# shanjiayao/PTT

Measured on AMD Instinct MI355X. Metric: tracklet frames/sec (hot path: PointNet++ SA stack + Point-Track-Transformer blocks), higher is better.
Workload: dtype f32

## Files before the change

include/ptt_hip.h:

```cpp
#ifndef PTT_HIP_H
#define PTT_HIP_H

#include <stddef.h>
#include <stdint.h>

#ifdef __cplusplus
extern "C" {
#endif

#define PTT_ABI_VERSION 28

enum {
    PTT_OK = 0,
    PTT_EINVAL = -1,
    PTT_EUNSUPPORTED = -2,
    PTT_ELAUNCH = -3,
    PTT_EWORKSPACE = -4
};

typedef void* ptt_stream_t;

int ptt_version(void);
const char* ptt_error_name(int code);
const char* ptt_last_error_string(void);

int ptt_fps_f32(const float* xyz, int B, int N, int npoint, int32_t* idx_out,
                ptt_stream_t stream);
int ptt_fps_ws_f32(const float* xyz, int B, int N, int npoint, int32_t* idx_out, float* workspace,
                   size_t workspace_elems, ptt_stream_t stream);

int ptt_gather_f32(const float* feat, const int32_t* idx, int B, int C, int N, int M,
                   float* out, ptt_stream_t stream);
int ptt_gather_grad_f32(const float* grad_out, const int32_t* idx, int B, int C, int N,
                        int M, float* grad_feat, ptt_stream_t stream);

int ptt_select_centres_f32(const float* xyz, const int32_t* idx, int B, int N, int M, float* new_xyz,
                           int64_t* idx64_out, ptt_stream_t stream);

int ptt_ball_query_f32(const float* new_xyz, const float* xyz, int B, int M, int N,
                       float radius, int nsample, int32_t* idx_out, ptt_stream_t stream);

int ptt_centres_ball_query_f32(const float* xyz, const int32_t* sel, int B, int N, int M, float radius, int nsample,
                               float* new_xyz, int64_t* idx64_out, int32_t* idx_out, ptt_stream_t stream);

int ptt_group_f32(const float* feat, const int32_t* idx, int B, int C, int N, int M,
                  int ns, float* out, ptt_stream_t stream);
int ptt_group_grad_f32(const float* grad_out, const int32_t* idx, int B, int C, int N,
                       int M, int ns, float* grad_feat, ptt_stream_t stream);

size_t ptt_scatter_add_det_workspace(int B, int N, int E);
int ptt_scatter_add_det_f32(const float* src, const int32_t* idx, int B, int C, int N, int E, float* out,
                            void* workspace, size_t workspace_bytes, ptt_stream_t stream);

int ptt_knn_f32(const float* xyz, int B, int N, int k, int32_t* idx_out,
                ptt_stream_t stream);
int ptt_knn_rel_f32(const float* xyz, int B, int N, int k, int32_t* idx_out, float* rel_out,
                    ptt_stream_t stream);

size_t ptt_packed_weight_elems(int Cout, int K);
int ptt_pack_weight_f32(const float* W, int Cout, int K, float* packed,
                        ptt_stream_t stream);
int ptt_pack_weight_rot_f32(const float* W, int Cout, int K, int rot, float* packed,
                            ptt_stream_t stream);

int ptt_linear_f32(const float* X, int rows, int K, int ldx, const float* Wpacked, int Cout,
                   const float* scale, const float* shift, int relu, const float* residual,
                   int ldr, float* out, int ldo, ptt_stream_t stream);

#define PTT_SA_MAX_LAYERS 4

typedef struct ptt_sa_layer {
    const float* Wpacked;
    const float* scale;
    const float* shift;
    int Cin;
    int Cout;
    int relu;
} ptt_sa_layer;

int ptt_rows_mlp_f32(const float* X, int rows, int K, int ldx, const ptt_sa_layer* layers, int n_layers,
                     const float* residual, int ldr, float* out, int ldo, ptt_stream_t stream);

size_t ptt_ball_query_grid_workspace(int B, int N);
int ptt_ball_query_grid_f32(const float* new_xyz, const float* xyz, int B, int M, int N, float radius, int nsample,
                            int32_t* idx_out, void* workspace, size_t workspace_bytes, ptt_stream_t stream);
int ptt_centres_ball_query_grid_f32(const float* xyz, const int32_t* sel, int B, int N, int M, float radius, int nsample,
                                    float* new_xyz, int64_t* idx64_out, int32_t* idx_out, void* workspace, size_t workspace_bytes,
                                    ptt_stream_t stream);
int ptt_fps_ball_knn_f32(const float* xyz, int B, int N, int M, float radius, int nsample, int k, int32_t* inds,
                         int64_t* inds64, float* new_xyz, int32_t* idx, int32_t* knn, float* rel, ptt_stream_t stream);
#define PTT_POINT_JOBS_MAX 4
typedef struct ptt_point_job {
    const float* xyz; const int32_t* centre_sel; const int32_t* point_sel;
    float* new_xyz; int64_t* idx64_out; int32_t* idx_out; float* rel_out;
    int32_t kind, sel_ld, B, Nraw, Npts, M, nsample;
    float radius;
} ptt_point_job;
int ptt_point_jobs_f32(const ptt_point_job* jobs, int n_jobs, ptt_stream_t stream);

#define PTT_ROW_JOBS_MAX 4
typedef struct ptt_row_job {
    const float* X; const float* X2;
    const float* Xmax;
    const float* Wpacked; const float* scale; const float* shift;
    const float* res; const float* res2;
    float* out; float* out2; float* raw;
    const float* rel; const float* w1;
    const float* qkv; const int32_t* knn; const float* pos;
    int32_t rows, K, K1, ldx, ldx2, Cout;
    int32_t act, res_split, ldr, ldr2, out_split, out_col0, ldo, ldo2, ldraw;
    int32_t prologue, epilogue, ldq, q_off, k_off, v_off, ldp, N;
    float sm_scale;
    int32_t col_tiles;
    const int32_t* idx; const float* xyz; const float* centres; const float* wx;
    float radius;
    int32_t ns, M, normalize_xyz, pro_relu;
} ptt_row_job;
int ptt_row_jobs_f32(const ptt_row_job* jobs, int n_jobs, ptt_stream_t stream);

typedef struct ptt_sa_desc {
    const float* xyz;
    const float* new_xyz;
    const int32_t* idx;
    const float* feat;
    int64_t feat_sb, feat_sc, feat_sn;
    float* out;
    int64_t out_sb, out_sc, out_sm;
    int B, N, M, nsample, C;
    float radius;
    int use_xyz;
    int normalize_xyz;
    int n_layers;
    ptt_sa_layer layers[PTT_SA_MAX_LAYERS];
    const float* l0_point_term;
    const float* l0_xyz_weight;
    int l0_channels;
    int l0_relu;
    void* compact_ws;
    size_t compact_ws_bytes;
} ptt_sa_desc;

int ptt_sa_fused_fwd_f32(const ptt_sa_desc* d, ptt_stream_t stream);
size_t ptt_sa_compact_workspace(int B, int M);

typedef struct ptt_xcorr_desc {
    const float* cos_t;
    const float* P;
    const float* w_sim;
    const float* scale0;
    const float* shift0;
    float* out;
    int64_t out_sb, out_sc, out_sn;
    float* sim_out;
    int B, Ns, Nt, C0;
    int n_layers;
    ptt_sa_layer layers[PTT_SA_MAX_LAYERS];
    int32_t split; int64_t out_sh;
    const float* search_feat; const float* templ_feat;
    int64_t s_sb, s_sn, t_sb, t_sn;
    int C; float eps;
} ptt_xcorr_desc;

int ptt_xcorr_fused_fwd_f32(const ptt_xcorr_desc* d, ptt_stream_t stream);

int ptt_cosine_map_f32(const float* search_feat, int64_t s_sb, int64_t s_sn, int64_t s_sc, const float* templ_feat,
                       int64_t t_sb, int64_t t_sn, int64_t t_sc, int B, int Ns, int Nt, int C, float eps,
                       float* cos_t, ptt_stream_t stream);

typedef struct ptt_attn_desc {
    const float* xyz;
    const float* rel;
    const int32_t* knn;
    const float* qkv;
    const float* Wd1p;
    const float* Wd2p;
    const float* bd2;
    const float* Wg1p;
    const float* bg1;
    const float* Wg2p;
    const float* bg2;
    float* res;
    float* attn;
    int B, N, k, D;
    const int32_t* order;
    int heads;
} ptt_attn_desc;

int ptt_pt_attn_pair_f32(const ptt_attn_desc* d, ptt_stream_t stream);
int ptt_spatial_order_f32(const float* xyz, int B, int N, int32_t* order, ptt_stream_t stream);

typedef struct ptt_crop_job {
    const float* points;
    int64_t ld;
    double lo1[3], hi1[3];
    double trans[3];
    double rot[9];
    double lo2[3], hi2[3];
    float* out;
    int32_t* count;
    int32_t n_points;
    int32_t capacity;
    uint8_t* label_out;
    double ltrans[3];
    double lrot[9];
    double llo[3], lhi[3];
    int32_t append;
    int32_t reserved;
} ptt_crop_job;

int ptt_crop_compact_f32(const ptt_crop_job* jobs_device, int n_jobs, ptt_stream_t stream);
#define PTT_CROP_JOBS_BY_VALUE_MAX 8
int ptt_crop_compact_host_f32(const ptt_crop_job* jobs_host, int n_jobs, ptt_stream_t stream);

#define PTT_MAX_SEGMENTS 4
typedef struct ptt_regularize_job {
    const float* seg[PTT_MAX_SEGMENTS];
    const int32_t* seg_count[PTT_MAX_SEGMENTS];
    int32_t seg_capacity[PTT_MAX_SEGMENTS];
    float* out;
    int32_t* info;
    int32_t n_seg;
    int32_t input_size;
// ... 297 lines not shown
```

ptt_amd/_lib.py:

```python
import ctypes
import os
import re
from ctypes import Structure, c_char_p, c_double, c_float, c_int, c_int32, c_int64, c_longlong, c_size_t, c_uint32, c_void_p

from .build import HEADER as HEADER_PATH, LIB as LIB_PATH


def _strip_comments(text):
    return re.sub(r"/\*.*?\*/|//[^\n]*", " ", text, flags=re.S)


def parse_defines(text):
    return {n: int(v) for n, v in re.findall(r"^[ \t]*#[ \t]*define[ \t]+(PTT_\w+)[ \t]+(-?\d+)[ \t]*$", _strip_comments(text), re.M)}


CTYPES = {"int": c_int, "int32_t": c_int32, "uint32_t": c_uint32, "int64_t": c_int64, "long long": c_longlong, "size_t": c_size_t,
          "float": c_float, "double": c_double, "ptt_stream_t": c_void_p}


def _ctype(decl, name, is_return=False):
    words = decl.replace("*", " * ").split()
    if not is_return and len(words) > 1 and words[-1] != "*":
        words.pop()
    if "*" in words:
# ... 67 lines not shown
                ("reg", c_float * 4), ("index", c_uint32), ("epoch", c_uint32), ("capacity", c_int32), ("reserved", c_int32)]


class TrainBatchDesc(Structure):
    _fields_ = [("search_points", c_void_p), ("template_points", c_void_p), ("cls_label", c_void_p), ("reg_label", c_void_p),
                ("src_out", c_void_p), ("idx_search_out", c_void_p), ("idx_template_out", c_void_p), ("info", c_void_p), ("totals", c_void_p),
                ("B", c_int32), ("n_cand", c_int32), ("search_size", c_int32), ("template_size", c_int32), ("min_points", c_int32),
                ("seed_lo", c_uint32), ("seed_hi", c_uint32), ("reserved", c_int32)]


class BnTrainTail(Structure):
    _fields_ = [("gamma", c_void_p), ("beta", c_void_p), ("act_a", c_void_p), ("act_b", c_void_p),
                ("running_mean", c_void_p), ("running_var", c_void_p), ("num_batches_tracked", c_void_p), ("momentum", c_float)]


class BnBwdInput(Structure):
    _fields_ = [("g", c_void_p), ("ldg", c_int), ("arg", c_void_p), ("ns", c_int), ("z", c_void_p), ("ldz", c_int),
                ("k1", c_void_p), ("c0", c_void_p), ("c1", c_void_p), ("mean", c_void_p), ("act_a", c_void_p), ("act_b", c_void_p),
                ("dz_out", c_void_p), ("ldd", c_int)]


class PackJob(Structure):
    _fields_ = [("W", c_void_p), ("out_offset", c_int64), ("stride_out", c_int64), ("stride_k", c_int64),
                ("Cout", c_int32), ("K", c_int32)]


class RowJob(Structure):
    _fields_ = [("X", c_void_p), ("X2", c_void_p), ("Xmax", c_void_p), ("Wpacked", c_void_p), ("scale", c_void_p), ("shift", c_void_p),
                ("res", c_void_p), ("res2", c_void_p), ("out", c_void_p), ("out2", c_void_p), ("raw", c_void_p),
                ("rel", c_void_p), ("w1", c_void_p), ("qkv", c_void_p), ("knn", c_void_p), ("pos", c_void_p),
                ("rows", c_int32), ("K", c_int32), ("K1", c_int32), ("ldx", c_int32), ("ldx2", c_int32), ("Cout", c_int32),
                ("act", c_int32), ("res_split", c_int32), ("ldr", c_int32), ("ldr2", c_int32), ("out_split", c_int32),
                ("out_col0", c_int32), ("ldo", c_int32), ("ldo2", c_int32), ("ldraw", c_int32),
                ("prologue", c_int32), ("epilogue", c_int32), ("ldq", c_int32), ("q_off", c_int32), ("k_off", c_int32),
                ("v_off", c_int32), ("ldp", c_int32), ("N", c_int32), ("sm_scale", c_float), ("col_tiles", c_int32),
                ("idx", c_void_p), ("xyz", c_void_p), ("centres", c_void_p), ("wx", c_void_p), ("radius", c_float),
                ("ns", c_int32), ("M", c_int32), ("normalize_xyz", c_int32), ("pro_relu", c_int32)]


class PointJob(Structure):
    _fields_ = [("xyz", c_void_p), ("centre_sel", c_void_p), ("point_sel", c_void_p), ("new_xyz", c_void_p), ("idx64_out", c_void_p),
                ("idx_out", c_void_p), ("rel_out", c_void_p), ("kind", c_int32), ("sel_ld", c_int32), ("B", c_int32),
                ("Nraw", c_int32), ("Npts", c_int32), ("M", c_int32), ("nsample", c_int32), ("radius", c_float)]


class TrackLossDesc(Structure):
    _fields_ = [("seed_cls", c_void_p), ("cls_label", c_void_p), ("search_inds", c_void_p), ("votes", c_void_p), ("reg_label", c_void_p),
                ("box_data", c_void_p), ("centres", c_void_p), ("pos_weight_seed", c_void_p), ("pos_weight_box", c_void_p),
                ("B", c_int32), ("N", c_int32), ("Ns", c_int32), ("M", c_int32), ("ld_reg", c_int32),
                ("w_seed_cls", c_float), ("w_seed_reg", c_float), ("w_box_cls", c_float), ("w_box_reg", c_float)]


class AdamTensor(Structure):
    _fields_ = [("param", c_void_p), ("grad", c_void_p), ("exp_avg", c_void_p), ("exp_avg_sq", c_void_p), ("n", c_int64)]


class GradJob(Structure):
    _fields_ = [("partial", c_void_p), ("nchunks", c_int32), ("reserved", c_int32)]


class GradSegment(Structure):
    _fields_ = [("dst", c_int64), ("n", c_int32), ("cols", c_int32), ("ld", c_int32), ("job0", c_int32), ("njobs", c_int32), ("out", c_int32),
                ("vec", c_int32), ("reserved", c_int32)]


class AdamHyper(Structure):
    _fields_ = [("beta1", c_float), ("beta2", c_float), ("one_minus_beta1", c_float), ("one_minus_beta2", c_float), ("eps", c_float), ("step_size", c_float), ("bias2_sqrt", c_float),
                ("weight_decay", c_float), ("max_norm", c_float), ("write_clipped", c_int32)]


class SaLayer(Structure):
    _fields_ = [("Wpacked", c_void_p), ("scale", c_void_p), ("shift", c_void_p),
                ("Cin", c_int), ("Cout", c_int), ("relu", c_int)]


class SaDesc(Structure):
    _fields_ = [("xyz", c_void_p), ("new_xyz", c_void_p), ("idx", c_void_p), ("feat", c_void_p),
                ("feat_sb", c_int64), ("feat_sc", c_int64), ("feat_sn", c_int64),
                ("out", c_void_p), ("out_sb", c_int64), ("out_sc", c_int64), ("out_sm", c_int64),
                ("B", c_int), ("N", c_int), ("M", c_int), ("nsample", c_int), ("C", c_int),
                ("radius", c_float), ("use_xyz", c_int), ("normalize_xyz", c_int), ("n_layers", c_int),
                ("layers", SaLayer * PTT_SA_MAX_LAYERS),
                ("l0_point_term", c_void_p), ("l0_xyz_weight", c_void_p), ("l0_channels", c_int), ("l0_relu", c_int),
                ("compact_ws", c_void_p), ("compact_ws_bytes", c_size_t)]


class XcorrDesc(Structure):
    _fields_ = [("cos_t", c_void_p), ("P", c_void_p), ("w_sim", c_void_p), ("scale0", c_void_p), ("shift0", c_void_p),
                ("out", c_void_p), ("out_sb", c_int64), ("out_sc", c_int64), ("out_sn", c_int64),
                ("sim_out", c_void_p),
                ("B", c_int), ("Ns", c_int), ("Nt", c_int), ("C0", c_int),
                ("n_layers", c_int), ("layers", SaLayer * PTT_SA_MAX_LAYERS),
                ("split", c_int32), ("out_sh", c_int64), ("search_feat", c_void_p), ("templ_feat", c_void_p),
                ("s_sb", c_int64), ("s_sn", c_int64), ("t_sb", c_int64), ("t_sn", c_int64), ("C", c_int), ("eps", c_float)]


class AttnDesc(Structure):
    _fields_ = [("xyz", c_void_p), ("rel", c_void_p), ("knn", c_void_p), ("qkv", c_void_p),
                ("Wd1p", c_void_p), ("Wd2p", c_void_p), ("bd2", c_void_p),
                ("Wg1p", c_void_p), ("bg1", c_void_p), ("Wg2p", c_void_p), ("bg2", c_void_p),
                ("res", c_void_p), ("attn", c_void_p),
                ("B", c_int), ("N", c_int), ("k", c_int), ("D", c_int), ("order", c_void_p), ("heads", c_int)]


_lib = None


def lib():
    global _lib
    if _lib is None:
        if not os.path.exists(LIB_PATH):
            raise RuntimeError(
                "ptt_amd: %s is missing — build it with `python -m ptt_amd.build` "
                "(hipcc --offload-arch=gfx950); there is no CPU fallback" % LIB_PATH)
        import torch
        try:
            loaded = ctypes.CDLL(LIB_PATH)
        except OSError as e:
            raise RuntimeError("ptt_amd: cannot load %s: %s" % (LIB_PATH, e))
        for name, (restype, argtypes) in PROTOTYPES.items():
            fn = getattr(loaded, name)
            fn.restype, fn.argtypes = restype, argtypes
        if loaded.ptt_version() != ABI_VERSION:
            raise RuntimeError("ptt_amd: %s has ABI version %d, this package expects %d — rebuild it with "
                               "`python -m ptt_amd.build`" % (LIB_PATH, loaded.ptt_version(), ABI_VERSION))
        _lib = loaded
    return _lib


def check(rc, what):
    if rc != 0:
        l = lib()
        raise RuntimeError("%s failed: %s (%s)" % (what, l.ptt_error_name(rc).decode(),
                                                   l.ptt_last_error_string().decode()))
```

ptt_amd/csrc/mfma_ops.hip:

```cpp
#include <math.h>
#include <stdlib.h>
#include <string.h>
#include "common.h"
#include "mfma_common.h"

#ifndef PTT_PAIR_PF
#define PTT_PAIR_PF 1
#endif
#ifndef PTT_GATHER_BATCH
#define PTT_GATHER_BATCH 16
#endif
#ifndef PTT_SA_WAVES
#define PTT_SA_WAVES 2
#endif

namespace ptt {

#ifdef PTT_DEV
#define PTT_STAMP(i) do { if (p.dbg && threadIdx.x == 0 && blockIdx.x < 4096) p.dbg[blockIdx.x * 8 + (i)] = __builtin_readcyclecounter(); } while (0)
#else
#define PTT_STAMP(i) do { } while (0)
#endif

__device__ __forceinline__ void stagger_second_slot(int first_wave_blocks, int quanta) {
// ... 341 lines not shown
                float y = acc[rt][u][r] * sc + sh;
                if (p.relu) y = fmaxf(y, 0.f);
                if (p.residual) y += p.residual[(size_t)gr * p.ldr + col];
                p.out[(size_t)gr * p.ldo + col] = y;
            }
    }
}

constexpr int LS_PD = 8;
__global__ __launch_bounds__(512, 1) void linear_small_kernel(LinearParams p) {
    extern __shared__ __attribute__((aligned(16))) float smem[];
    const int t = threadIdx.x, lane = t & 63, half = lane >> 5;
    const int w = __builtin_amdgcn_readfirstlane(t >> 6), ks = w >> 2, cw = w & 3;
    const int row0 = blockIdx.x * 32;
    const int ct = blockIdx.y * 4 + cw;
    const bool has_ct = ct < p.NT;
    const int hb = ((p.nkb + 1) / 2 + LS_PD - 1) / LS_PD * LS_PD;
    const int ldk = 2 * hb * 8 + 4;
    float* Xs = smem;
    float* Rs = smem + 32 * ldk;
    {
        const int qpr = 2 * hb * 2;
        for (int e = t; e < 32 * qpr; e += 512) {
            const int r = e / qpr, c = (e - r * qpr) << 2;
            f32x4 v = {0.f, 0.f, 0.f, 0.f};
            if (row0 + r < p.rows && c < p.K) v = *reinterpret_cast<const f32x4*>(p.X + (size_t)(row0 + r) * p.ldx + c);
            *reinterpret_cast<f32x4*>(Xs + r * ldk + c) = v;
        }
    }
    const __amdgpu_buffer_rsrc_t wr = weight_rsrc(p.Wp);
    const int wvoff = ((has_ct ? ct : 0) * 64 + lane) * 16;
    const int wkstep = p.NT * 1024;
    const int kb0 = ks * hb, last = p.nkb - 1;
    f32x4 b[LS_PD];
#pragma unroll
    for (int i = 0; i < LS_PD; ++i) b[i] = weight_load(wr, wvoff, min(kb0 + i, last) * wkstep);
    f32x16 acc;
#pragma unroll
    for (int r = 0; r < 16; ++r) acc[r] = 0.f;
    __syncthreads();
    const float* arow = Xs + (lane & 31) * ldk + 4 * half + kb0 * 8;
    for (int k = 0; k < hb; k += LS_PD) {
#pragma unroll
        for (int i = 0; i < LS_PD; ++i) {
            const f32x4 a = *reinterpret_cast<const f32x4*>(arow + (k + i) * 8);
#pragma unroll
            for (int j = 0; j < 4; ++j) acc = __builtin_amdgcn_mfma_f32_32x32x2f32(a[j], b[i][j], acc, 0, 0, 0);
            b[i] = weight_load(wr, wvoff, min(kb0 + k + i + LS_PD, last) * wkstep);
        }
    }
    if (ks == 1) {
#pragma unroll
        for (int r = 0; r < 16; ++r) Rs[(cw * 16 + r) * 64 + lane] = acc[r];
    }
    __syncthreads();
    if (ks == 1 || !has_ct) return;
    const int col = ct * 32 + (lane & 31);
    if (col >= p.Cout) return;
    const float sc = p.scale ? p.scale[col] : 1.f;
    const float sh = p.shift ? p.shift[col] : 0.f;
#pragma unroll
    for (int r = 0; r < 16; ++r) {
        const int gr = row0 + tile_row(r, half);
        if (gr >= p.rows) continue;
        float y = (acc[r] + Rs[(cw * 16 + r) * 64 + lane]) * sc + sh;
        if (p.relu) y = fmaxf(y, 0.f);
        if (p.residual) y += p.residual[(size_t)gr * p.ldr + col];
        p.out[(size_t)gr * p.ldo + col] = y;
    }
}

struct SaLayerDev { const float* Wp; const float* scale; const float* shift; int Cin, Cout, relu, nkb, NT; };
struct SaParams {
    const float* xyz; const float* new_xyz; const int32_t* idx; const float* feat; float* out;
    long long fsb, fsc, fsn, osb, osc, osm;
    int B, N, M, C, use_xyz, normalize, n_layers, ldk, K0, first_wave, stagger, vec_gather;
    int tiles, chunk;
    int hoist, l0_relu;
    const float* wx;
    float radius;
    long long* dbg;
    int32_t* cws;
    SaLayerDev L[PTT_SA_MAX_LAYERS];
};

struct RowsMlpParams {
    const float* X; const float* residual; float* out;
    int rows, K0, ldx, ldr, ldo, n_layers, ldk, vec_in;
    SaLayerDev L[PTT_SA_MAX_LAYERS];
};

__global__ __launch_bounds__(256, 2) void rows_mlp_kernel(RowsMlpParams p) {
    extern __shared__ __attribute__((aligned(16))) float smem[];
    float* Xs = smem;
    const int t = threadIdx.x, lane = t & 63, w = t >> 6, half = lane >> 5;
    const int row0 = blockIdx.x * 32;
    f32x4 pw[3];
    float psh[3];
    auto prefetch = [&](const SaLayerDev& L) {
        const f32x4* bp = reinterpret_cast<const f32x4*>(L.Wp) + (size_t)w * 64 + lane;
#pragma unroll
        for (int u = 0; u < 3; ++u) {
            psh[u] = 0.f;
            if (w + 4 * u < L.NT) {
                pw[u] = bp[(size_t)u * 4 * 64];
                const int col = (w + 4 * u) * 32 + (lane & 31);
                if (L.shift && !L.scale && col < L.Cout) psh[u] = L.shift[col];
            }
        }
    };
    prefetch(p.L[0]);
    {
        const int Kpad = p.L[0].nkb * 8;
        if (p.vec_in) {
            const int nq = Kpad >> 2;
            for (int e = t; e < 32 * nq; e += 256) {
                const int r = e / nq, c4 = (e - r * nq) * 4;
                f32x4 v = {0.f, 0.f, 0.f, 0.f};
                if (row0 + r < p.rows && c4 < p.K0) v = *reinterpret_cast<const f32x4*>(p.X + (size_t)(row0 + r) * p.ldx + c4);
                *reinterpret_cast<f32x4*>(Xs + r * p.ldk + c4) = v;
            }
        } else {
            for (int e = t; e < 32 * Kpad; e += 256) {
                const int r = e / Kpad, c = e - r * Kpad;
                Xs[r * p.ldk + c] = (row0 + r < p.rows && c < p.K0) ? p.X[(size_t)(row0 + r) * p.ldx + c] : 0.f;
            }
        }
    }
    lds_barrier();
    for (int l = 0; l < p.n_layers; ++l) {
        const SaLayerDev& L = p.L[l];
        const bool last = l == p.n_layers - 1, affine = L.scale != nullptr;
        f32x16 acc[1][3];
#pragma unroll
        for (int u = 0; u < 3; ++u)
#pragma unroll
            for (int r = 0; r < 16; ++r) acc[0][u][r] = psh[u];
        int nvalid = 0;
#pragma unroll
        for (int u = 0; u < 3; ++u)
            if (w + 4 * u < L.NT) nvalid = u + 1;
        if (nvalid) gemm_tiles<1, 3, 0>(Xs, p.ldk, L.nkb, reinterpret_cast<const f32x4*>(L.Wp), L.NT, w, nvalid, lane, acc, pw);
        if (!last) { prefetch(p.L[l + 1]); lds_barrier(); }
#pragma unroll
        for (int u = 0; u < 3; ++u) {
            if (u >= nvalid) break;
            const int col = (w + 4 * u) * 32 + (lane & 31);
            float sc = 1.f, sh = 0.f;
            if (affine && col < L.Cout) { sc = L.scale[col]; sh = L.shift ? L.shift[col] : 0.f; }
#pragma unroll
            for (int r = 0; r < 16; ++r) {
                float y = affine ? acc[0][u][r] * sc + sh : acc[0][u][r];
                if (L.relu) y = fmaxf(y, 0.f);
                const int row = tile_row(r, half);
                if (!last) {
                    Xs[row * p.ldk + col] = (col < L.Cout) ? y : 0.f;
                } else if (col < L.Cout && row0 + row < p.rows) {
                    if (p.residual) y += p.residual[(size_t)(row0 + row) * p.ldr + col];
                    p.out[(size_t)(row0 + row) * p.ldo + col] = y;
                }
            }
        }
        if (!last) lds_barrier();
    }
}

// ... 177 lines not shown
            } else {
                float m0 = y[0], m1 = y[8];
#pragma unroll
                for (int r = 1; r < 8; ++r) { m0 = fmaxf(m0, y[r]); m1 = fmaxf(m1, y[8 + r]); }
                m0 = max_halves(m0);
                m1 = max_halves(m1);
                if (L.relu) { m0 = fmaxf(m0, 0.f); m1 = fmaxf(m1, 0.f); }
                if (half == 0) {
                    const int ca = rt * 2, cb = rt * 2 + 1;
                    if (ca < ncentres) {
                        const int c = centre0 + ca; const int b = c / p.M, mm = c - b * p.M;
                        p.out[b * p.osb + col * p.osc + mm * p.osm] = m0;
                    }
                    if (cb < ncentres) {
                        const int c = centre0 + cb; const int b = c / p.M, mm = c - b * p.M;
                        p.out[b * p.osb + col * p.osc + mm * p.osm] = m1;
                    }
                }
            }
        }
    }
    if (!last) lds_barrier();
}

template <int NS, int RT>
__global__ __launch_bounds__(256, PTT_SA_WAVES) void sa_fused_kernel(SaParams p) {
    extern __shared__ __attribute__((aligned(16))) float smem[];
    float* Xs = smem;
    constexpr int CPW = 32 * RT / NS;
    const int t = threadIdx.x, lane = t & 63, w = t >> 6;
    const int total_centres = p.B * p.M;
    const int centre0 = logical_block() * CPW;
    const int ncentres = min(CPW, total_centres - centre0);
    stagger_second_slot(p.first_wave, p.stagger);
    PTT_STAMP(0);

    SaPre pre;
    pre.w[0] = pre.w[1] = f32x4{0.f, 0.f, 0.f, 0.f};
    prefetch_first_block(p.L[0].Wp, p.L[0].scale, p.L[0].shift, p.L[0].NT, w, lane, pre);

    sa_gather_rows<NS, 8 * RT>(p, Xs, w * 8 * RT, centre0, lane);
    lds_barrier();

    PTT_STAMP(1);
    for (int l = 0; l < p.n_layers; ++l) {
        const SaLayerDev& L = p.L[l];
        const bool last = (l == p.n_layers - 1);
        const int ctw = (L.NT + 3) >> 2;
        const SaLayerDev* Ln = last ? nullptr : &p.L[l + 1];
        if (ctw <= 1) sa_layer<NS, 1, RT>(p, L, last, Xs, lane, w, centre0, ncentres, pre, Ln);
        else sa_layer<NS, 2, RT>(p, L, last, Xs, lane, w, centre0, ncentres, pre, Ln);
        PTT_STAMP(2 + l);
    }
}

constexpr int SAS_LDK = 132;
constexpr int SAS_TILE = 64 * SAS_LDK;

__device__ __forceinline__ f32x4 sas_pair_load(const float* meta, __amdgpu_buffer_rsrc_t rf, int w, int i, int sub, int q,
                                               f32x4& m) {
    m = *reinterpret_cast<const f32x4*>(meta + (w * 16 + 2 * i + sub) * 4);
    return weight_load(rf, __builtin_bit_cast(int, m[0]) + q * 16, 0);
}
__device__ __forceinline__ void sas_pair_store(float* X, int w, int i, int sub, int q, f32x4 v, const f32x4& m, const f32x4& wx0,
                                               const f32x4& wx1, const f32x4& wx2, float floor) {
#pragma unroll
    for (int j = 0; j < 4; ++j) {
        float y = __builtin_fmaf(wx0[j], m[1], v[j]);
        y = __builtin_fmaf(wx1[j], m[2], y);
        y = __builtin_fmaf(wx2[j], m[3], y);
        v[j] = fmaxf(y, floor);
    }
    *reinterpret_cast<f32x4*>(X + (16 * w + 2 * i + sub) * SAS_LDK + q * 4) = v;
}

struct SasCentre {
    int c, b, m;
    __device__ __forceinline__ void advance(int k, int M) {
        c += k; m += k;
        while (m >= M) { m -= M; ++b; }
    }
};

__device__ __forceinline__ float sas_pool(const f32x16& a, float sh, int relu) {
    float mx = a[0];
#pragma unroll
    for (int r = 1; r < 16; ++r) mx = fmaxf(mx, a[r]);
    mx = max_halves(mx) + sh;
    return relu ? fmaxf(mx, 0.f) : mx;
}

#ifndef PTT_SAS_INTERLEAVE
#define PTT_SAS_INTERLEAVE 0
#endif
#ifndef PTT_SAS_EXP
#define PTT_SAS_EXP 0
#endif
template <int NS>
__global__ __launch_bounds__(256, 2) void sa_stream_kernel(SaParams p) {
    static_assert(NS == 32, "one centre per 32-row tile");
    extern __shared__ __attribute__((aligned(16))) float smem[];
    float* const P = smem;
    float* const Q = smem + SAS_TILE;
    float* const meta = smem + 2 * SAS_TILE;
    const int t = threadIdx.x, lane = t & 63, half = lane >> 5, sub = half, q = lane & 31;
    const int w = __builtin_amdgcn_readfirstlane(t >> 6);
    const int tile0 = logical_block() * p.chunk;
    const int ntiles = min(p.chunk, p.tiles - tile0);
    if (ntiles <= 0) return;
    stagger_second_slot(p.first_wave, p.stagger);
    const SaLayerDev& L1 = p.L[0];
    const SaLayerDev& L2 = p.L[1];
    const __amdgpu_buffer_rsrc_t rf = weight_rsrc(p.feat);
    const __amdgpu_buffer_rsrc_t wr1 = weight_rsrc(L1.Wp), wr2 = weight_rsrc(L2.Wp);
    const int wvoff = (w * 64 + lane) * 16;
    constexpr int WK1 = 4 * 1024, WK2 = 8 * 1024;
    const f32x4 wx0 = *reinterpret_cast<const f32x4*>(p.wx + q * 4);
    const f32x4 wx1 = *reinterpret_cast<const f32x4*>(p.wx + 128 + q * 4);
    const f32x4 wx2 = *reinterpret_cast<const f32x4*>(p.wx + 256 + q * 4);
    const int col = lane & 31;
    const float sh1 = L1.shift ? L1.shift[w * 32 + col] : 0.f;
    const float sh2a = L2.shift ? L2.shift[w * 32 + col] : 0.f;
    const float sh2b = L2.shift ? L2.shift[(w + 4) * 32 + col] : 0.f;
    f32x16 sh1v;
#pragma unroll
    for (int r = 0; r < 16; ++r) sh1v[r] = sh1;
    const int total_centres = p.B * p.M;
    const float floor0 = p.l0_relu ? 0.f : -__builtin_inff();
    const float rdiv = p.normalize ? p.radius : 1.0f;
    const int M = p.M, N = p.N;
    const int osb = (int)p.osb, osm = (int)p.osm;
    const int ocol0 = (w * 32 + col) * (int)p.osc, ocol1 = ((w + 4) * 32 + col) * (int)p.osc;

    SasCentre own, first;
    {
        const int c0 = tile0 * 2;
        first.c = c0; first.b = c0 / M; first.m = c0 - first.b * M;
        own = first;
        own.advance(w >> 1, M);
    }
    auto meta_index = [&](const SasCentre& ce) -> int {
        const int c = ce.c < total_centres ? ce.c : total_centres - 1;
        return p.idx[(size_t)c * 32 + 16 * (w & 1) + (lane & 15)];
    };
    struct MetaXyz { float x, y, z, cx, cy, cz; int flat; };
    auto meta_fetch = [&](const SasCentre& ce, int n) -> MetaXyz {
        const bool in = ce.c < total_centres;
        const int c = in ? ce.c : total_centres - 1;
        const int b = in ? ce.b : p.B - 1;
        MetaXyz r;
        r.flat = b * N + n;
        r.x = p.xyz[(size_t)r.flat * 3 + 0]; r.y = p.xyz[(size_t)r.flat * 3 + 1]; r.z = p.xyz[(size_t)r.flat * 3 + 2];
        r.cx = p.new_xyz[(size_t)c * 3 + 0]; r.cy = p.new_xyz[(size_t)c * 3 + 1]; r.cz = p.new_xyz[(size_t)c * 3 + 2];
        return r;
    };
    auto meta_store = [&](const MetaXyz& r) {
        const float dx = (r.x - r.cx) / rdiv, dy = (r.y - r.cy) / rdiv, dz = (r.z - r.cz) / rdiv;
        const int off = r.flat * (128 * (int)sizeof(float));
        *reinterpret_cast<f32x4*>(meta + (w * 16 + (lane & 15)) * 4) = f32x4{__builtin_bit_cast(float, off), dx, dy, dz};
    };

    f32x4 pre1[2] = {weight_load(wr1, wvoff, 0), weight_load(wr1, wvoff, WK1)};
    {
        const int n = meta_index(own);
        meta_store(meta_fetch(own, n));
#pragma unroll
        for (int i = 0; i < 8; ++i) {
            f32x4 m;
            const f32x4 v = sas_pair_load(meta, rf, w, i, sub, q, m);
            sas_pair_store(P, w, i, sub, q, v, m, wx0, wx1, wx2, floor0);
        }
    }

    f32x16 acc[2][2];
#pragma unroll
    for (int rt = 0; rt < 2; ++rt)
#pragma unroll
        for (int u = 0; u < 2; ++u)
#pragma unroll
            for (int r = 0; r < 16; ++r) acc[rt][u][r] = 0.f;
    float pv[2][2] = {{0.f, 0.f}, {0.f, 0.f}};
    SasCentre prev = first;
    const f32x16 zero16 = {0.f, 0.f, 0.f, 0.f, 0.f, 0.f, 0.f, 0.f, 0.f, 0.f, 0.f, 0.f, 0.f, 0.f, 0.f, 0.f};

    auto store_pooled = [&](const SasCentre& f) {
        SasCentre c1 = f;
        c1.advance(1, M);
        if (half == 0) {
            if (f.c < total_centres) {
                float* o = p.out + (f.b * osb + f.m * osm);
                o[ocol0] = pv[0][0]; o[ocol1] = pv[0][1];
            }
            if (c1.c < total_centres) {
                float* o = p.out + (c1.b * osb + c1.m * osm);
                o[ocol0] = pv[1][0]; o[ocol1] = pv[1][1];
            }
        }
    };

    for (int it = 0; it < ntiles; ++it) {
        const bool more = it + 1 < ntiles;
        SasCentre own_next = own;
        if (more) own_next.advance(2, M);
        if (!(PTT_SAS_EXP & 1)) lds_barrier();
        const int nn = meta_index(own_next);
        MetaXyz mx;

        f32x16 acc1[2];
        {
            const float* arow = P + (lane & 31) * SAS_LDK + 4 * half;
            f32x4 a0[2], a1[2], bc[2], bn[2];
#define SAS_A1(A, KB)                                                                           \
            {                                                                                   \
                A[0] = *reinterpret_cast<const f32x4*>(arow + (KB) * 8);                        \
                A[1] = *reinterpret_cast<const f32x4*>(arow + 32 * SAS_LDK + (KB) * 8);         \
            }
            bc[0] = pre1[0]; bc[1] = pre1[1];
            SAS_A1(a0, 0)
#pragma unroll
            for (int i = 0; i < 8; ++i) {
                if (i < 7) { bn[0] = weight_load(wr1, wvoff, (2 * i + 2) * WK1); bn[1] = weight_load(wr1, wvoff, (2 * i + 3) * WK1); }
                SAS_A1(a1, 2 * i + 1)
                if (i == 4 && !(PTT_SAS_EXP & 16)) mx = meta_fetch(own_next, nn);
                __builtin_amdgcn_sched_barrier(0);
                if (i == 0) {
#pragma unroll
                    for (int rt = 0; rt < 2; ++rt) acc1[rt] = __builtin_amdgcn_mfma_f32_32x32x2f32(a0[rt][0], bc[0][0], sh1v, 0, 0, 0);
#pragma unroll
                    for (int j = 1; j < 4; ++j)
#pragma unroll
                        for (int rt = 0; rt < 2; ++rt)
                            acc1[rt] = __builtin_amdgcn_mfma_f32_32x32x2f32(a0[rt][j], bc[0][j], acc1[rt], 0, 0, 0);
                } else {
#pragma unroll
                    for (int j = 0; j < 4; ++j)
#pragma unroll
                        for (int rt = 0; rt < 2; ++rt)
                            acc1[rt] = __builtin_amdgcn_mfma_f32_32x32x2f32(a0[rt][j], bc[0][j], acc1[rt], 0, 0, 0);
                }
                __builtin_amdgcn_sched_barrier(0);
                if (i < 7) SAS_A1(a0, 2 * i + 2)
                __builtin_amdgcn_sched_barrier(0);
#pragma unroll
                for (int j = 0; j < 4; ++j)
#pragma unroll
                    for (int rt = 0; rt < 2; ++rt)
                        acc1[rt] = __builtin_amdgcn_mfma_f32_32x32x2f32(a1[rt][j], bc[1][j], acc1[rt], 0, 0, 0);
                __builtin_amdgcn_sched_barrier(0);
                if (i < 4 && !(PTT_SAS_EXP & 8)) pv[i >> 1][i & 1] = sas_pool(acc[i >> 1][i & 1], (i & 1) ? sh2b : sh2a, L2.relu);
                if (i == 6 && !(PTT_SAS_EXP & 16)) meta_store(mx);
                __builtin_amdgcn_sched_barrier(0);
                bc[0] = bn[0]; bc[1] = bn[1];
            }
#undef SAS_A1
        }
        f32x4 pre2[2][2];
#pragma unroll
        for (int k = 0; k < 2; ++k) {
            pre2[k][0] = weight_load(wr2, wvoff, k * WK2);
            pre2[k][1] = weight_load(wr2, wvoff, k * WK2 + 4 * 1024);
        }
#pragma unroll
        for (int rt = 0; rt < 2; ++rt)
#pragma unroll
            for (int r = (PTT_SAS_EXP & 4) ? 15 : 0; r < 16; ++r)
                Q[(rt * 32 + tile_row(r, half)) * SAS_LDK + w * 32 + col] = fmaxf(acc1[rt][r], 0.f);
        if (it > 0) store_pooled(prev);
        if (!(PTT_SAS_EXP & 1)) lds_barrier();

        {
            const float* arow = Q + (lane & 31) * SAS_LDK + 4 * half;
            f32x4 a0[2], a1[2], bc[2][2], bn[2][2];
#define SAS_A2(A, KB)                                                                           \
            {                                                                                   \
                A[0] = *reinterpret_cast<const f32x4*>(arow + (KB) * 8);                        \
                A[1] = *reinterpret_cast<const f32x4*>(arow + 32 * SAS_LDK + (KB) * 8);         \
            }
#pragma unroll
            for (int k = 0; k < 2; ++k) { bc[k][0] = pre2[k][0]; bc[k][1] = pre2[k][1]; }
            SAS_A2(a0, 0)
            f32x4 mc = *reinterpret_cast<const f32x4*>(meta + (w * 16 + sub) * 4), mn = mc;
#pragma unroll
            for (int i = 0; i < 8; ++i) {
                if (i < 7) {
#pragma unroll
                    for (int k = 0; k < 2; ++k) {
                        bn[k][0] = weight_load(wr2, wvoff, (2 * i + 2 + k) * WK2);
                        bn[k][1] = weight_load(wr2, wvoff, (2 * i + 2 + k) * WK2 + 4 * 1024);
                    }
                } else {
                    pre1[0] = weight_load(wr1, wvoff, 0);
                    pre1[1] = weight_load(wr1, wvoff, WK1);
                }
                SAS_A2(a1, 2 * i + 1)
                f32x4 v = wx0;
                if (!(PTT_SAS_EXP & 2)) v = weight_load(rf, __builtin_bit_cast(int, mc[0]) + q * 16, 0);
                __builtin_amdgcn_sched_barrier(0);
                if (i == 0) {
#pragma unroll
                    for (int u = 0; u < 2; ++u)
#pragma unroll
                        for (int rt = 0; rt < 2; ++rt)
                            acc[rt][u] = __builtin_amdgcn_mfma_f32_32x32x2f32(a0[rt][0], bc[0][u][0], zero16, 0, 0, 0);
#pragma unroll
                    for (int j = 1; j < 4; ++j)
#pragma unroll
                        for (int u = 0; u < 2; ++u)
#pragma unroll
                            for (int rt = 0; rt < 2; ++rt)
                                acc[rt][u] = __builtin_amdgcn_mfma_f32_32x32x2f32(a0[rt][j], bc[0][u][j], acc[rt][u], 0, 0, 0);
                } else {
                    gemm_mfma_block<2, 2, 2>(a0, bc[0], acc);
                }
                __builtin_amdgcn_sched_barrier(0);
                if (i < 7) {
                    SAS_A2(a0, 2 * i + 2)
                    mn = *reinterpret_cast<const f32x4*>(meta + (w * 16 + 2 * (i + 1) + sub) * 4);
                }
                __builtin_amdgcn_sched_barrier(0);
                gemm_mfma_block<2, 2, 2>(a1, bc[1], acc);
                if (!(PTT_SAS_EXP & 2)) sas_pair_store(P, w, i, sub, q, v, mc, wx0, wx1, wx2, floor0);
#if PTT_SAS_INTERLEAVE
#pragma unroll
                for (int k = 0; k < 16; ++k) {
                    __builtin_amdgcn_sched_group_barrier(0x008, 1, 0);
                    __builtin_amdgcn_sched_group_barrier(0x002, 1, 0);
                }
                __builtin_amdgcn_sched_group_barrier(0x200, 1, 0);
#endif
                __builtin_amdgcn_sched_barrier(0);
                mc = mn;
#pragma unroll
                for (int k = 0; k < 2; ++k) { bc[k][0] = bn[k][0]; bc[k][1] = bn[k][1]; }
            }
#undef SAS_A2
        }
        prev = first;
        if (more) { first.advance(2, M); own = own_next; }
    }
#pragma unroll
    for (int i = 0; i < 4; ++i) pv[i >> 1][i & 1] = sas_pool(acc[i >> 1][i & 1], (i & 1) ? sh2b : sh2a, L2.relu);
    store_pooled(prev);
}

struct XcorrParams {
    const float* P; const float* wsim; const float* scale0; const float* shift0;
    float* sim_out;
    const float* cos_t;
    int C0, Nt;
    SaParams sa;
    const float* sfeat; const float* tfeat; long long s_sb, s_sn, t_sb, t_sn; int C; float eps;
    long long out_sh;
};

struct CosParams {
    const float* sfeat; const float* tfeat; float* cos_t;
    long long s_sb, s_sn, s_sc, t_sb, t_sn, t_sc;
    int B, Ns, Nt, C;
    float eps;
};
__global__ __launch_bounds__(256) void cos_map_kernel(CosParams q) {
    const int lane = threadIdx.x & 63;
    const int j = blockIdx.x * 4 + (threadIdx.x >> 6);
    if (j >= q.B * q.Ns) return;
    const int b = j / q.Ns, jj = j - b * q.Ns;
    const float* s = q.sfeat + (long long)b * q.s_sb + (long long)jj * q.s_sn;
    for (int i0 = 0; i0 < q.Nt; i0 += 64) {
        const int i = i0 + lane;
        const float* a = q.tfeat + (long long)b * q.t_sb + (long long)(i < q.Nt ? i : q.Nt - 1) * q.t_sn;
        float dot = 0.f, na = 0.f, ns = 0.f;
        if (q.t_sc == 1 && q.s_sc == 1 && (q.C & 3) == 0 && ((q.t_sn | q.t_sb | q.s_sn | q.s_sb) & 3) == 0 &&
            ((reinterpret_cast<uintptr_t>(q.tfeat) | reinterpret_cast<uintptr_t>(q.sfeat)) & 15) == 0) {
            for (int c = 0; c < q.C; c += 4) {
                const f32x4 av = *reinterpret_cast<const f32x4*>(a + c), sv = *reinterpret_cast<const f32x4*>(s + c);
#pragma unroll
                for (int k = 0; k < 4; ++k) { dot += av[k] * sv[k]; na += av[k] * av[k]; ns += sv[k] * sv[k]; }
            }
        } else {
            for (int c = 0; c < q.C; ++c) {
                const float av = a[(long long)c * q.t_sc], sv = s[(long long)c * q.s_sc];
                dot += av * sv; na += av * av; ns += sv * sv;
            }
        }
        if (i < q.Nt) q.cos_t[((long long)b * q.Ns + jj) * q.Nt + i] = dot / (fmaxf(sqrtf(na), q.eps) * fmaxf(sqrtf(ns), q.eps));
    }
}

template <int RT, bool SPLIT>
__global__ __launch_bounds__(256, 2) void xcorr_fused_kernel(XcorrParams q) {
    constexpr int ROWS = 32 * RT;
    extern __shared__ __attribute__((aligned(16))) float smem[];
    const SaParams& p = q.sa;
    float* Xs = smem;
    float* simv = smem + ROWS * p.ldk;
    const int t = threadIdx.x, lane = t & 63, w = t >> 6, half = lane >> 5;
    const int npts = p.B * p.M;
    const int j = SPLIT ? (int)blockIdx.x % npts : logical_block();
    const int hsel = SPLIT ? (int)blockIdx.x / npts : 0;
    const int b = j / p.M, jj = j - b * p.M;
    stagger_second_slot(p.first_wave, p.stagger);
    SaPre pre;
    pre.w[0] = pre.w[1] = f32x4{0.f, 0.f, 0.f, 0.f};
    float run[2] = {-__builtin_inff(), -__builtin_inff()};
    const int nlast = p.n_layers - 1;
    const SaLayerDev& LL = p.L[nlast];

    const int ibeg = SPLIT ? hsel * (q.Nt >> 1) : 0, iend = SPLIT ? ibeg + (q.Nt >> 1) : q.Nt;
    for (int i0 = ibeg; i0 < iend; i0 += ROWS) {
        prefetch_first_block(p.L[0].Wp, p.L[0].scale, p.L[0].shift, p.L[0].NT, w, lane, pre);
        if (i0 != ibeg) __syncthreads();
        if constexpr (SPLIT) {
            const int i = t >> 3, sub = t & 7;
            const float* a = q.tfeat + (long long)b * q.t_sb + (long long)(i0 + i) * q.t_sn;
            const float* sv_ = q.sfeat + (long long)b * q.s_sb + (long long)jj * q.s_sn;
            float dot = 0.f, na = 0.f, ns = 0.f;
            for (int c = sub * 4; c < q.C; c += 32) {
                const f32x4 av = *reinterpret_cast<const f32x4*>(a + c), sv = *reinterpret_cast<const f32x4*>(sv_ + c);
#pragma unroll
                for (int k = 0; k < 4; ++k) { dot += av[k] * sv[k]; na += av[k] * av[k]; ns += sv[k] * sv[k]; }
            }
#pragma unroll
// ... 80 lines not shown
            p.out[(SPLIT ? hsel * q.out_sh : 0) + b * p.osb + col * p.osc + jj * p.osm] = LL.relu ? fmaxf(run[u], 0.f) : run[u];
        }
    }
}

template <int NS, int CT, bool AFFINE, int RT>
__device__ __forceinline__ void sa_wave_layer(const SaParams& p, const SaLayerDev& L, bool last, float* Xw, int lane,
                                              int centre0, int ncentres) {
    f32x16 acc[RT][CT];
#pragma unroll
    for (int u = 0; u < CT; ++u) {
        const float s0 = (!AFFINE && L.shift) ? L.shift[u * 32 + (lane & 31)] : 0.f;
#pragma unroll
        for (int rt = 0; rt < RT; ++rt)
#pragma unroll
            for (int r = 0; r < 16; ++r) acc[rt][u][r] = s0;
    }
    gemm_core<RT, CT, CT, 1>(Xw, p.ldk, L.nkb, reinterpret_cast<const f32x4*>(L.Wp), L.NT, 0, lane, acc);
    __builtin_amdgcn_wave_barrier();
    const int half = lane >> 5;
#pragma unroll
    for (int u = 0; u < CT; ++u) {
        const int col = u * 32 + (lane & 31);
        float sc = 1.f, sv = 0.f;
        if constexpr (AFFINE) { sc = L.scale[col]; sv = L.shift ? L.shift[col] : 0.f; }
#pragma unroll
        for (int rt = 0; rt < RT; ++rt) {
            float y[16];
#pragma unroll
            for (int r = 0; r < 16; ++r) y[r] = AFFINE ? acc[rt][u][r] * sc + sv : acc[rt][u][r];
            if (!last) {
#pragma unroll
                for (int r = 0; r < 16; ++r)
                    Xw[(rt * 32 + tile_row(r, half)) * p.ldk + col] = L.relu ? fmaxf(y[r], 0.f) : y[r];
            } else if (NS == 32) {
                float m = y[0];
#pragma unroll
                for (int r = 1; r < 16; ++r) m = fmaxf(m, y[r]);
                m = max_halves(m);
                if (L.relu) m = fmaxf(m, 0.f);
                if (half == 0 && rt < ncentres) {
                    const int c = centre0 + rt; const int b = c / p.M, mm = c - b * p.M;
                    p.out[b * p.osb + col * p.osc + mm * p.osm] = m;
                }
            } else {
                float m0 = y[0], m1 = y[8];
#pragma unroll
                for (int r = 1; r < 8; ++r) { m0 = fmaxf(m0, y[r]); m1 = fmaxf(m1, y[8 + r]); }
                m0 = max_halves(m0);
                m1 = max_halves(m1);
                if (L.relu) { m0 = fmaxf(m0, 0.f); m1 = fmaxf(m1, 0.f); }
                if (half == 0) {
                    if (2 * rt < ncentres) {
                        const int c = centre0 + 2 * rt; const int b = c / p.M, mm = c - b * p.M;
                        p.out[b * p.osb + col * p.osc + mm * p.osm] = m0;
                    }
                    if (2 * rt + 1 < ncentres) {
                        const int c = centre0 + 2 * rt + 1; const int b = c / p.M, mm = c - b * p.M;
                        p.out[b * p.osb + col * p.osc + mm * p.osm] = m1;
                    }
                }
            }
        }
    }
    __builtin_amdgcn_wave_barrier();
}

constexpr int SAC_HDR = 16;
struct SacTable {
    int32_t* ws; int T;
    __host__ __device__ int32_t* ndist() const { return ws + SAC_HDR; }
    __host__ __device__ int32_t* list(int k) const { return ws + SAC_HDR + (size_t)(1 + k) * T; }
    __host__ __device__ int32_t* rows(int k) const { return ws + SAC_HDR + 5 * (size_t)T + (size_t)((4 << k) - 4) * T; }
    static size_t words(size_t T) { return SAC_HDR + 65 * T; }
};
constexpr int SAC_PASSES = 4;

__global__ __launch_bounds__(64) void sa_compact_zero_kernel(int32_t* ws) {
    if (threadIdx.x < 4) ws[threadIdx.x] = 0;
}

template <bool XYZ>
__global__ __launch_bounds__(256) void sa_compact_kernel(const float* __restrict__ xyz, const int32_t* __restrict__ idx, int N, int M,
                                                         SacTable tab) {
    __shared__ int s_cnt[4], s_base[4], s_cls[32], s_pos[32], s_nd[32];
    __shared__ int s_row[32][32];
    const int t = threadIdx.x, lane = t & 63, half = lane >> 5, s = lane & 31, w = t >> 6;
    const int g0 = blockIdx.x * 32, T = tab.T;
    if (t < 4) s_cnt[t] = 0;
    __syncthreads();
    int iv[SAC_PASSES];
    uint32_t x[SAC_PASSES], y[SAC_PASSES], z[SAC_PASSES];
#pragma unroll
    for (int q = 0; q < SAC_PASSES; ++q) iv[q] = idx[(size_t)min(g0 + q * 8 + w * 2 + half, T - 1) * 32 + s];
    if constexpr (XYZ) {
#pragma unroll
        for (int q = 0; q < SAC_PASSES; ++q) {
            const int b = min(g0 + q * 8 + w * 2 + half, T - 1) / M;
            const uint32_t* pt = reinterpret_cast<const uint32_t*>(xyz) + ((size_t)b * N + iv[q]) * 3;
            x[q] = pt[0]; y[q] = pt[1]; z[q] = pt[2];
        }
    }
#pragma unroll
    for (int q = 0; q < SAC_PASSES; ++q) {
        const int lc = q * 8 + w * 2 + half;
        const int i0a = __builtin_amdgcn_readlane(iv[q], 0), i0b = __builtin_amdgcn_readlane(iv[q], 32);
        const int i0 = half ? i0b : i0a;
        const bool real = s == 0 || iv[q] != i0;
        int dup = 0;
        if constexpr (XYZ) {
            const unsigned long long rm = __ballot(real);
            const int J = 31 - __builtin_clz((uint32_t)rm | (uint32_t)(rm >> 32));
            for (int j = 0; j < J; ++j) {
                const uint32_t xa = __builtin_amdgcn_readlane(x[q], j), xb = __builtin_amdgcn_readlane(x[q], 32 + j);
                const uint32_t ya = __builtin_amdgcn_readlane(y[q], j), yb = __builtin_amdgcn_readlane(y[q], 32 + j);
                const uint32_t za = __builtin_amdgcn_readlane(z[q], j), zb = __builtin_amdgcn_readlane(z[q], 32 + j);
                dup |= (int)(j < s) & (int)(x[q] == (half ? xb : xa)) & (int)(y[q] == (half ? yb : ya)) & (int)(z[q] == (half ? zb : za));
            }
        }
        const bool keep = real && !dup;
        const unsigned long long km = __ballot(keep);
        const uint32_t m = half ? (uint32_t)(km >> 32) : (uint32_t)km;
        const int nd = __popc(m);
        if (keep) s_row[lc][__popc(m & ((1u << s) - 1u))] = iv[q];
        if (s == 0) {
            const int k = nd <= 4 ? 0 : nd <= 8 ? 1 : nd <= 16 ? 2 : 3;
            const bool valid = g0 + lc < T;
            s_cls[lc] = valid ? k : -1;
            s_nd[lc] = nd;
            s_pos[lc] = valid ? atomicAdd(&s_cnt[k], 1) : 0;
            if (valid) tab.ndist()[g0 + lc] = nd;
        }
    }
    __syncthreads();
    if (t < 4) s_base[t] = s_cnt[t] ? atomicAdd(&tab.ws[t], s_cnt[t]) : 0;
    __syncthreads();
    for (int e = t; e < 32 * 32; e += 256) {
        const int lc = e >> 5, j = e & 31, k = s_cls[lc];
        if (k < 0 || j >= (4 << k)) continue;
        const int q = s_base[k] + s_pos[lc];
        tab.rows(k)[(size_t)q * (4 << k) + j] = s_row[lc][j < s_nd[lc] ? j : 0];
        if (j == 0) tab.list(k)[q] = g0 + lc;
    }
}

#ifndef PTT_SAL_WGS
#define PTT_SAL_WGS 1
#endif
#ifndef PTT_SAL_WAVES
#define PTT_SAL_WAVES 12
#endif

template <int ROWS>
struct SacTileT {
    static constexpr int LG = ROWS == 32 ? 3 : 4;
    static_assert(ROWS == 32 || ROWS == 64, "32- or 64-row tiles");
    int k, first, n;
    __device__ __forceinline__ static void count(const int32_t* ws, int total, int (&cnt)[4], int (&tiles)[4]) {
#pragma unroll
        for (int k = 0; k < 4; ++k) {
            cnt[k] = min(max(ws[k], 0), total);
            tiles[k] = (k ? tiles[k - 1] : 0) + ((cnt[k] + ((1 << LG) >> k) - 1) >> (LG - k));
        }
    }
    __device__ __forceinline__ void at(int j, const int (&tiles)[4], const int (&cnt)[4]) {
        k = j < tiles[0] ? 0 : j < tiles[1] ? 1 : j < tiles[2] ? 2 : 3;
        const int j0 = k == 0 ? 0 : k == 1 ? tiles[0] : k == 2 ? tiles[1] : tiles[2];
        const int nk = k == 0 ? cnt[0] : k == 1 ? cnt[1] : k == 2 ? cnt[2] : cnt[3];
        first = (j - j0) << (LG - k);
        n = min((1 << LG) >> k, nk - first);
    }
    __device__ __forceinline__ void row(const SacTable& tab, int s, int& n_out, int& ball) const {
        const int cl = s >> (2 + k), inb = cl < n;
        n_out = tab.rows(k)[(size_t)first * (4 << k) + (inb ? s : (s & ((4 << k) - 1)))];
        ball = tab.list(k)[first + (inb ? cl : 0)];
    }
};
using SacTile = SacTileT<32>;

template <int NU>
__device__ __forceinline__ void sac_store(int k, int n, int ball, int M, const f32x16 (&acc)[NU], const float (&sh)[NU],
                                          float* const (&o)[NU], int relu, int half, int osb, int osm) {
    int ob[8];
#pragma unroll
    for (int g = 0; g < 8; ++g) {
        if (g >= (8 >> k)) break;
        const int id = __builtin_amdgcn_readlane(ball, g << (2 + k)), b = id / M;
        ob[g] = b * osb + (id - b * M) * osm;
    }
#pragma unroll
    for (int u = 0; u < NU; ++u) {
        const f32x16& a = acc[u];
        if (k == 3) {
            const float mx = sas_pool(a, sh[u], relu);
            if (half == 0) o[u][ob[0]] = mx;
        } else if (k == 2) {
            float m0 = a[0], m1 = a[8];
#pragma unroll
            for (int r = 1; r < 8; ++r) { m0 = fmaxf(m0, a[r]); m1 = fmaxf(m1, a[8 + r]); }
            m0 = max_halves(m0) + sh[u]; m1 = max_halves(m1) + sh[u];
            if (relu) { m0 = fmaxf(m0, 0.f); m1 = fmaxf(m1, 0.f); }
            if (half < n) o[u][half ? ob[1] : ob[0]] = half ? m1 : m0;
        } else {
            float m[4];
#pragma unroll
            for (int q = 0; q < 4; ++q) m[q] = fmaxf(fmaxf(a[4 * q], a[4 * q + 1]), fmaxf(a[4 * q + 2], a[4 * q + 3]));
            if (k == 1) {
#pragma unroll
                for (int q = 0; q < 4; ++q) m[q] = max_halves(m[q]) + sh[u];
#pragma unroll
                for (int i = 0; i < 2; ++i) {
                    const int g = 2 * half + i;
                    float v = half ? m[2 + i] : m[i];
                    if (relu) v = fmaxf(v, 0.f);
                    if (g < n) o[u][half ? ob[2 + i] : ob[i]] = v;
                }
            } else {
#pragma unroll
                for (int q = 0; q < 4; ++q) {
                    const int g = 2 * q + half;
                    float v = m[q] + sh[u];
                    if (relu) v = fmaxf(v, 0.f);
                    if (g < n) o[u][half ? ob[2 * q + 1] : ob[2 * q]] = v;
                }
            }
        }
    }
}

template <bool COMPACT>
__global__ __launch_bounds__(64 * PTT_SAL_WAVES) __attribute__((amdgpu_waves_per_eu(PTT_SAL_WAVES * PTT_SAL_WGS / 4)))
void sa_lds_kernel(SaParams p) {
    extern __shared__ __attribute__((aligned(16))) float smem[];
    float* W1 = smem;
    float* W2 = smem + 4096;
    const int t = threadIdx.x, lane = t & 63, half = lane >> 5, col = lane & 31;
    const int w = __builtin_amdgcn_readfirstlane(t >> 6);
    const int total = p.B * p.M, M = p.M, N = p.N;
    const int nw = (int)blockDim.x >> 6;
    SacTable tab{p.cws, total};
    int cnt[4], tiles[4];
    if constexpr (COMPACT) {
        SacTile::count(p.cws, total, cnt, tiles);
        if (logical_block() >= tiles[3]) return;
    }
    {
        const f32x4* g1 = reinterpret_cast<const f32x4*>(p.L[1].Wp);
        const f32x4* g2 = reinterpret_cast<const f32x4*>(p.L[2].Wp);
        f32x4* s1 = reinterpret_cast<f32x4*>(W1);
        f32x4* s2 = reinterpret_cast<f32x4*>(W2);
        const int nthr = (int)blockDim.x;
        for (int i = t; i < 1024; i += nthr) s1[i] = g1[i];
        for (int i = t; i < 2048; i += nthr) s2[i] = g2[i];
    }
    float* cst = smem + 4096 + 8192 + w * 640 + lane;
#pragma unroll
    for (int u = 0; u < 2; ++u) {
        const f32x4 f = reinterpret_cast<const f32x4*>(p.L[0].Wp)[u * 64 + col];
        const float s0 = p.L[0].shift ? p.L[0].shift[u * 32 + col] : 0.f;
        cst[(0 + u) * 64] = half ? f[1] : f[0];
        cst[(2 + u) * 64] = half ? s0 : f[2];
        cst[(4 + u) * 64] = p.L[1].shift ? p.L[1].shift[u * 32 + col] : 0.f;
    }
#pragma unroll
    for (int u = 0; u < 4; ++u) cst[(6 + u) * 64] = p.L[2].shift ? p.L[2].shift[u * 32 + col] : 0.f;
    const float one_zero = half ? 0.f : 1.f, one_hi = 1.f;
    __syncthreads();
    int c0, c1, cstep;
    if constexpr (COMPACT) {
        c0 = logical_block() + (int)gridDim.x * w; c1 = tiles[3]; cstep = (int)gridDim.x * nw;
    } else {
        const int gw = logical_block() * nw + w;
        c0 = gw * p.chunk; c1 = min(total, c0 + p.chunk); cstep = 1;
    }
    if (c0 >= c1) return;
    const float rdiv = p.normalize ? p.radius : 1.0f;
    const int osb = (int)p.osb, osm = (int)p.osm, osc = (int)p.osc;
    const f32x16 zero16 = {0.f, 0.f, 0.f, 0.f, 0.f, 0.f, 0.f, 0.f, 0.f, 0.f, 0.f, 0.f, 0.f, 0.f, 0.f, 0.f};
    const float* a1p = W1 + lane * 4;
    const float* b2p = W2 + lane * 4;
    const __amdgpu_buffer_rsrc_t rx = weight_rsrc(p.xyz);

    SasCentre ce{0, 0, 0};
    SacTile tc{0, 0, 0};
    float px, py, pz, cx, cy, cz;
    int g_cur = 0;
    if constexpr (COMPACT) {
        tc.at(c0, tiles, cnt);
        int n_cur;
        tc.row(tab, col, n_cur, g_cur);
        const size_t flat = (size_t)(g_cur / M) * N + n_cur;
        px = p.xyz[flat * 3]; py = p.xyz[flat * 3 + 1]; pz = p.xyz[flat * 3 + 2];
        cx = p.new_xyz[(size_t)g_cur * 3]; cy = p.new_xyz[(size_t)g_cur * 3 + 1]; cz = p.new_xyz[(size_t)g_cur * 3 + 2];
    } else {
        ce.c = c0; ce.b = c0 / M; ce.m = c0 - ce.b * M;
        const int n_cur = p.idx[(size_t)c0 * 32 + col];
        const size_t flat = (size_t)ce.b * N + n_cur;
        px = p.xyz[flat * 3]; py = p.xyz[flat * 3 + 1]; pz = p.xyz[flat * 3 + 2];
        cx = p.new_xyz[(size_t)c0 * 3]; cy = p.new_xyz[(size_t)c0 * 3 + 1]; cz = p.new_xyz[(size_t)c0 * 3 + 2];
    }
    for (int c = c0; c < c1; c += cstep) {
        SasCentre nx = ce;
        SacTile tx = tc;
        int n_next, g_next;
        if constexpr (COMPACT) {
            if (c + cstep < c1) tx.at(c + cstep, tiles, cnt);
            tx.row(tab, col, n_next, g_next);
        } else {
            if (c + 1 < c1) nx.advance(1, M);
            n_next = p.idx[(size_t)nx.c * 32 + col];
        }
        f32x4 wa[2], wn[2];
#pragma unroll
        for (int u = 0; u < 2; ++u) wa[u] = *reinterpret_cast<const f32x4*>(a1p + u * 256);
        const float dx = (px - cx) / rdiv, dy = (py - cy) / rdiv, dz = (pz - cz) / rdiv;
        __builtin_amdgcn_sched_barrier(0);
        f32x16 h0[2];
        {
            const float k0 = half ? dy : dx, k1 = half ? one_hi : dz;
#pragma unroll
            for (int u = 0; u < 2; ++u) h0[u] = __builtin_amdgcn_mfma_f32_32x32x2f32(cst[(0 + u) * 64], k0, zero16, 0, 0, 0);
#pragma unroll
            for (int u = 0; u < 2; ++u) h0[u] = __builtin_amdgcn_mfma_f32_32x32x2f32(cst[(2 + u) * 64], k1, h0[u], 0, 0, 0);
#pragma unroll
            for (int u = 0; u < 2; ++u)
#pragma unroll
                for (int r = 0; r < 16; ++r) h0[u][r] = fmaxf(h0[u][r], 0.f);
        }
        f32x16 h1[2];
        f32x4 wb[4], wm[4];
        {
#pragma unroll
            for (int u = 0; u < 2; ++u) h1[u] = __builtin_amdgcn_mfma_f32_32x32x2f32(cst[(4 + u) * 64], one_zero, zero16, 0, 0, 0);
#pragma unroll
            for (int kb = 0; kb < 8; ++kb) {
                if (kb < 7) {
#pragma unroll
                    for (int u = 0; u < 2; ++u) wn[u] = *reinterpret_cast<const f32x4*>(a1p + ((kb + 1) * 2 + u) * 256);
                } else {
#pragma unroll
                    for (int u = 0; u < 4; ++u) wb[u] = *reinterpret_cast<const f32x4*>(b2p + u * 256);
                }
                __builtin_amdgcn_sched_barrier(0);
#pragma unroll
                for (int j = 0; j < 4; ++j)
#pragma unroll
                    for (int u = 0; u < 2; ++u)
                        h1[u] = __builtin_amdgcn_mfma_f32_32x32x2f32(wa[u][j], h0[kb >> 2][(kb & 3) * 4 + j], h1[u], 0, 0, 0);
                __builtin_amdgcn_sched_barrier(0);
#pragma unroll
                for (int u = 0; u < 2; ++u) wa[u] = wn[u];
            }
#pragma unroll
            for (int u = 0; u < 2; ++u)
#pragma unroll
                for (int r = 0; r < 16; ++r) h1[u][r] = fmaxf(h1[u][r], 0.f);
        }
        {
            const int g = COMPACT ? g_next : nx.c;
            const int off = ((COMPACT ? g_next / M : nx.b) * N + n_next) * 12;
            px = __builtin_bit_cast(float, __builtin_amdgcn_raw_buffer_load_b32(rx, off, 0, 0));
            py = __builtin_bit_cast(float, __builtin_amdgcn_raw_buffer_load_b32(rx, off + 4, 0, 0));
            pz = __builtin_bit_cast(float, __builtin_amdgcn_raw_buffer_load_b32(rx, off + 8, 0, 0));
            cx = p.new_xyz[(size_t)g * 3]; cy = p.new_xyz[(size_t)g * 3 + 1]; cz = p.new_xyz[(size_t)g * 3 + 2];
        }
        __builtin_amdgcn_sched_barrier(0);
        {
            f32x16 acc[4];
#pragma unroll
            for (int kb = 0; kb < 8; ++kb) {
                if (kb < 7) {
#pragma unroll
                    for (int u = 0; u < 4; ++u) wm[u] = *reinterpret_cast<const f32x4*>(b2p + ((kb + 1) * 4 + u) * 256);
                }
                __builtin_amdgcn_sched_barrier(0);
#pragma unroll
                for (int j = 0; j < 4; ++j)
#pragma unroll
                    for (int u = 0; u < 4; ++u)
                        acc[u] = __builtin_amdgcn_mfma_f32_32x32x2f32(h1[kb >> 2][(kb & 3) * 4 + j], wb[u][j],
                                                                       (kb == 0 && j == 0) ? zero16 : acc[u], 0, 0, 0);
                __builtin_amdgcn_sched_barrier(0);
#pragma unroll
                for (int u = 0; u < 4; ++u) wb[u] = wm[u];
            }
            if constexpr (COMPACT) {
                const float sh2[4] = {cst[6 * 64], cst[7 * 64], cst[8 * 64], cst[9 * 64]};
                float* const o[4] = {p.out + col * osc, p.out + (32 + col) * osc, p.out + (64 + col) * osc, p.out + (96 + col) * osc};
                sac_store<4>(tc.k, tc.n, g_cur, M, acc, sh2, o, p.L[2].relu, half, osb, osm);
            } else {
                float* o = p.out + (ce.b * osb + ce.m * osm);
#pragma unroll
                for (int u = 0; u < 4; ++u) {
                    const float mx = sas_pool(acc[u], cst[(6 + u) * 64], p.L[2].relu);
                    if (half == 0) o[(u * 32 + col) * osc] = mx;
                }
            }
        }
        if constexpr (COMPACT) { tc = tx; g_cur = g_next; } else ce = nx;
    }
}

__global__ __launch_bounds__(256, 2) void sa_stream_compact_kernel(SaParams p) {
    extern __shared__ __attribute__((aligned(16))) float smem[];
    float* const P = smem;
    float* const Q = smem + SAS_TILE;
    float* const meta = smem + 2 * SAS_TILE;
    int* const sball = reinterpret_cast<int*>(meta + 64 * 4);
    const int t = threadIdx.x, lane = t & 63, half = lane >> 5, sub = half, q = lane & 31, col = q;
    const int w = __builtin_amdgcn_readfirstlane(t >> 6);
    const int total = p.B * p.M, M = p.M, N = p.N;
    const SacTable tab{p.cws, total};
    int cnt[4], tiles[4];
    SacTileT<64>::count(p.cws, total, cnt, tiles);
    if ((int)blockIdx.x >= tiles[3]) return;
    const SaLayerDev& L1 = p.L[0];
    const SaLayerDev& L2 = p.L[1];
    const __amdgpu_buffer_rsrc_t rf = weight_rsrc(p.feat);
    const __amdgpu_buffer_rsrc_t wr1 = weight_rsrc(L1.Wp), wr2 = weight_rsrc(L2.Wp);
    const int wvoff = (w * 64 + lane) * 16;
    constexpr int WK1 = 4 * 1024, WK2 = 8 * 1024;
    const f32x4 wx0 = *reinterpret_cast<const f32x4*>(p.wx + q * 4);
    const f32x4 wx1 = *reinterpret_cast<const f32x4*>(p.wx + 128 + q * 4);
    const f32x4 wx2 = *reinterpret_cast<const f32x4*>(p.wx + 256 + q * 4);
    const float sh1 = L1.shift ? L1.shift[w * 32 + col] : 0.f;
    const float sh2[2] = {L2.shift ? L2.shift[w * 32 + col] : 0.f, L2.shift ? L2.shift[(w + 4) * 32 + col] : 0.f};
    f32x16 sh1v;
#pragma unroll
    for (int r = 0; r < 16; ++r) sh1v[r] = sh1;
    const f32x16 zero16 = {0.f, 0.f, 0.f, 0.f, 0.f, 0.f, 0.f, 0.f, 0.f, 0.f, 0.f, 0.f, 0.f, 0.f, 0.f, 0.f};
    const float floor0 = p.l0_relu ? 0.f : -__builtin_inff();
    const float rdiv = p.normalize ? p.radius : 1.0f;
    const int osb = (int)p.osb, osm = (int)p.osm;
    float* const o[2] = {p.out + (w * 32 + col) * (int)p.osc, p.out + ((w + 4) * 32 + col) * (int)p.osc};

    for (int j = blockIdx.x; j < tiles[3]; j += (int)gridDim.x) {
        SacTileT<64> tc;
        tc.at(j, tiles, cnt);
        if (t < 64) {
            int n, ball;
            tc.row(tab, t, n, ball);
            const int flat = (ball / M) * N + n;
            const float x = p.xyz[(size_t)flat * 3 + 0], y = p.xyz[(size_t)flat * 3 + 1], z = p.xyz[(size_t)flat * 3 + 2];
            const float cx = p.new_xyz[(size_t)ball * 3 + 0], cy = p.new_xyz[(size_t)ball * 3 + 1], cz = p.new_xyz[(size_t)ball * 3 + 2];
            const float dx = (x - cx) / rdiv, dy = (y - cy) / rdiv, dz = (z - cz) / rdiv;
            const int off = flat * (128 * (int)sizeof(float));
            *reinterpret_cast<f32x4*>(meta + t * 4) = f32x4{__builtin_bit_cast(float, off), dx, dy, dz};
            sball[t] = ball;
        }
        __syncthreads();
#pragma unroll
        for (int i = 0; i < 8; ++i) {
            f32x4 m;
            const f32x4 v = sas_pair_load(meta, rf, w, i, sub, q, m);
            sas_pair_store(P, w, i, sub, q, v, m, wx0, wx1, wx2, floor0);
        }
        const int ballr[2] = {sball[col], sball[32 + col]};
        __syncthreads();
        {
            f32x16 acc1[2] = {sh1v, sh1v};
            const float* arow = P + (lane & 31) * SAS_LDK + 4 * half;
#pragma unroll
            for (int kb = 0; kb < 16; ++kb) {
                const f32x4 b = weight_load(wr1, wvoff, kb * WK1);
                const f32x4 a[2] = {*reinterpret_cast<const f32x4*>(arow + kb * 8),
                                    *reinterpret_cast<const f32x4*>(arow + 32 * SAS_LDK + kb * 8)};
#pragma unroll
                for (int jj = 0; jj < 4; ++jj)
#pragma unroll
                    for (int rt = 0; rt < 2; ++rt) acc1[rt] = __builtin_amdgcn_mfma_f32_32x32x2f32(a[rt][jj], b[jj], acc1[rt], 0, 0, 0);
            }
#pragma unroll
            for (int rt = 0; rt < 2; ++rt)
#pragma unroll
                for (int r = 0; r < 16; ++r) Q[(rt * 32 + tile_row(r, half)) * SAS_LDK + w * 32 + col] = fmaxf(acc1[rt][r], 0.f);
        }
        __syncthreads();
        {
            f32x16 acc[2][2] = {{zero16, zero16}, {zero16, zero16}};
            const float* arow = Q + (lane & 31) * SAS_LDK + 4 * half;
#pragma unroll
            for (int kb = 0; kb < 16; ++kb) {
                const f32x4 b[2] = {weight_load(wr2, wvoff, kb * WK2), weight_load(wr2, wvoff, kb * WK2 + 4 * 1024)};
                const f32x4 a[2] = {*reinterpret_cast<const f32x4*>(arow + kb * 8),
                                    *reinterpret_cast<const f32x4*>(arow + 32 * SAS_LDK + kb * 8)};
                gemm_mfma_block<2, 2, 2>(a, b, acc);
            }
#pragma unroll
            for (int rt = 0; rt < 2; ++rt) {
                const int n = tc.n - rt * (8 >> tc.k);
                if (n <= 0) continue;
                sac_store<2>(tc.k, n, ballr[rt], M, acc[rt], sh2, o, L2.relu, half, osb, osm);
            }
        }
    }
}

template <int NS, int RT>
__global__ __launch_bounds__(256, 2) void sa_wave_kernel(SaParams p) {
    extern __shared__ __attribute__((aligned(16))) float smem[];
    constexpr int CPW = 32 * RT / NS;
    const int t = threadIdx.x, lane = t & 63, w = t >> 6;
    float* Xw = smem + w * 32 * RT * p.ldk;
    const int total_centres = p.B * p.M;
    const int centre0 = (logical_block() * 4 + w) * CPW;
    if (centre0 >= total_centres) return;
    const int ncentres = min(CPW, total_centres - centre0);

#pragma unroll
    for (int rt = 0; rt < RT; ++rt) sa_gather_rows<NS, 32>(p, Xw, rt * 32, centre0, lane);
    __builtin_amdgcn_wave_barrier();

    for (int l = 0; l < p.n_layers; ++l) {
        const SaLayerDev& L = p.L[l];
        const bool last = (l == p.n_layers - 1);
#define PTT_WAVE_LAYER(CTV)                                                                         \
        { if (L.scale) sa_wave_layer<NS, CTV, true, RT>(p, L, last, Xw, lane, centre0, ncentres);       \
          else sa_wave_layer<NS, CTV, false, RT>(p, L, last, Xw, lane, centre0, ncentres); }
        if (L.NT == 1) PTT_WAVE_LAYER(1)
        else if (L.NT == 2) PTT_WAVE_LAYER(2)
        else PTT_WAVE_LAYER(4)
#undef PTT_WAVE_LAYER
    }
}

struct AttnParams {
    const float* xyz; const float* rel; const int32_t* knn; const float* qkv; const float* Wd1p;
    const float* Wd2p; const float* bd2; const float* Wg1p; const float* bg1; const float* Wg2p; const float* bg2;
    float* res; float* attn;
    const int32_t* order;
    int BN, N, first_wave, stagger;
    long long* dbg;
};

template <int D, int HEADS>
__device__ __forceinline__ void gemm_heads(const float* Xs, int ldk, const float* Wp, int w, int lane, f32x16 (&acc)[1][4],
                                           const f32x4 (&pre)[4]) {
    static_assert(D == 512 && (HEADS == 2 || HEADS == 4 || HEADS == 8 || HEADS == 16), "4 waves x 4 column tiles of D = 512");
    constexpr int HD = D / HEADS, TPH = HD / 32, NKB = HD / 8;
    constexpr int NA = HEADS == 2 ? 2 : 4;
    constexpr int NB = HEADS == 2 ? 2 : 1;
    const int row = lane & 31, half = lane >> 5;
    const float* arow[NA];
#pragma unroll
    for (int i = 0; i < NA; ++i) arow[i] = Xs + row * ldk + 4 * half + ((w + 4 * i * (4 / NA)) / TPH) * HD;
    const __amdgpu_buffer_rsrc_t wr = weight_rsrc(Wp);
    int wvoff[NB];
#pragma unroll
    for (int i = 0; i < NB; ++i) wvoff[i] = (((w + 4 * i) % TPH) * 64 + lane) * 16;
    constexpr int wkstep = TPH * 1024;
    f32x4 bcur[NB], bnxt[NB];
#pragma unroll
    for (int i = 0; i < NB; ++i) { bcur[i] = pre[i]; bnxt[i] = bcur[i]; }
    auto block = [&](int kb) {
        f32x4 a[NA];
#pragma unroll
        for (int i = 0; i < NA; ++i) a[i] = *reinterpret_cast<const f32x4*>(arow[i] + kb * 8);
#pragma unroll
        for (int j = 0; j < 4; ++j)
#pragma unroll
            for (int u = 0; u < 4; ++u)
                acc[0][u] = __builtin_amdgcn_mfma_f32_32x32x2f32(a[u / (4 / NA)][j], bcur[u % NB][j], acc[0][u], 0, 0, 0);
    };
    for (int kb = 0; kb + 1 < NKB; ++kb) {
#pragma unroll
        for (int i = 0; i < NB; ++i) bnxt[i] = weight_load(wr, wvoff[i], (kb + 1) * wkstep);
        block(kb);
#pragma unroll
        for (int i = 0; i < NB; ++i) bcur[i] = bnxt[i];
    }
    block(NKB - 1);
}

template <int D, int HEADS>
__device__ __forceinline__ void prefetch_first_block_heads(const float* Wp, int w, int lane, f32x4 (&pre)[4]) {
// ... 248 lines not shown
        if (L.nkb * 8 > maxk) maxk = L.nkb * 8;
        if (!last && L.NT * 32 > maxk) maxk = L.NT * 32;
        cin = s.Cout;
    }
    if (ldo < cin || (residual && ldr < cin)) return fail(PTT_EINVAL, "ptt_rows_mlp_f32: ldo=%d ldr=%d Cout=%d", ldo, ldr, cin);
    p.ldk = maxk + 4;
    p.vec_in = ((K & 3) == 0 && (ldx & 3) == 0 && (reinterpret_cast<uintptr_t>(X) & 15) == 0) ? 1 : 0;
    const int lds = 32 * p.ldk * (int)sizeof(float);
    int rc = set_lds_limit(reinterpret_cast<const void*>(rows_mlp_kernel), lds);
    if (rc) return rc;
    hipLaunchKernelGGL(rows_mlp_kernel, dim3((rows + 31) / 32), dim3(256), lds, as_stream(stream), p);
    return check_launch("rows_mlp_kernel");
}

extern "C" size_t ptt_sa_compact_workspace(int B, int M) {
    const long long T = (long long)(B > 0 ? B : 0) * (M > 0 ? M : 0);
    return SacTable::words((size_t)T) * sizeof(int32_t);
}

extern "C" int ptt_sa_fused_fwd_f32(const ptt_sa_desc* d, ptt_stream_t stream) {
    if (!d) return fail(PTT_EINVAL, "ptt_sa_fused_fwd_f32: null descriptor");
    if (d->B < 0 || d->N <= 0 || d->M < 0 || d->C < 0 || d->n_layers < 1 || d->n_layers > PTT_SA_MAX_LAYERS)
        return fail(PTT_EINVAL, "ptt_sa_fused_fwd_f32: B=%d N=%d M=%d C=%d layers=%d", d->B, d->N, d->M, d->C,
                    d->n_layers);
    if (d->nsample != 16 && d->nsample != 32 && d->nsample != 64)
        return fail(PTT_EUNSUPPORTED, "ptt_sa_fused_fwd_f32: nsample=%d (16, 32 and 64 are instantiated)", d->nsample);
    if (d->B == 0 || d->M == 0) return PTT_OK;
    const bool hoist = d->l0_point_term != nullptr;
    if (!d->xyz || !d->new_xyz || !d->idx || !d->out || (!hoist && d->C > 0 && !d->feat))
        return fail(PTT_EINVAL, "ptt_sa_fused_fwd_f32: null pointer");
    if (!d->use_xyz && d->C == 0) return fail(PTT_EINVAL, "ptt_sa_fused_fwd_f32: no xyz and no features");
    if (hoist) {
        const int c0 = d->l0_channels;
        if (!d->use_xyz || !d->l0_xyz_weight || c0 <= 0 || (c0 % 32) != 0 || c0 > 256 ||
            (reinterpret_cast<uintptr_t>(d->l0_point_term) & 15) != 0 ||
            (reinterpret_cast<uintptr_t>(d->l0_xyz_weight) & 15) != 0)
            return fail(PTT_EINVAL, "ptt_sa_fused_fwd_f32: hoisted layer 0 needs use_xyz, 16-byte aligned (B,N,C0) and "
                        "(3,C0) arrays and C0 a multiple of 32 <= 256 (C0=%d)", c0);
    }

    SaParams p;
    p.xyz = d->xyz; p.new_xyz = d->new_xyz; p.idx = d->idx; p.feat = d->feat; p.out = d->out;
    p.fsb = d->feat_sb; p.fsc = d->feat_sc; p.fsn = d->feat_sn;
    p.osb = d->out_sb; p.osc = d->out_sc; p.osm = d->out_sm;
    p.B = d->B; p.N = d->N; p.M = d->M; p.C = d->C; p.use_xyz = d->use_xyz ? 1 : 0;
    p.normalize = d->normalize_xyz ? 1 : 0; p.n_layers = d->n_layers; p.radius = d->radius;
    p.K0 = (d->use_xyz ? 3 : 0) + d->C;
    p.hoist = hoist ? 1 : 0; p.l0_relu = d->l0_relu ? 1 : 0; p.wx = d->l0_xyz_weight;
    if (hoist && d->l0_channels == 128 && (unsigned long long)d->B * d->N * 128ull * sizeof(float) < 0x7fffffffull &&
        !dev_switches().sa_gather1)
        p.hoist = 2;
    if (hoist) {
        p.feat = d->l0_point_term; p.C = d->l0_channels; p.K0 = p.C;
        p.fsc = 1; p.fsn = p.C; p.fsb = (long long)d->N * p.C;
    }
    int maxk = 0, cin = p.K0;
    for (int l = 0; l < d->n_layers; ++l) {
        const ptt_sa_layer& s = d->layers[l];
        if (s.Cin != cin) return fail(PTT_EINVAL, "ptt_sa_fused_fwd_f32: layer %d Cin=%d, expected %d", l, s.Cin, cin);
        if (s.Cout <= 0 || (s.Cout % 32) != 0 || s.Cout > 256)
            return fail(PTT_EUNSUPPORTED, "ptt_sa_fused_fwd_f32: layer %d Cout=%d must be a multiple of 32 <= 256", l,
                        s.Cout);
        if (!s.Wpacked) return fail(PTT_EINVAL, "ptt_sa_fused_fwd_f32: layer %d has no weights", l);
        SaLayerDev& L = p.L[l];
        L.Wp = s.Wpacked; L.scale = s.scale; L.shift = s.shift; L.Cin = s.Cin; L.Cout = s.Cout; L.relu = s.relu;
        L.nkb = (s.Cin + 7) / 8; L.NT = s.Cout / 32;
        if (L.nkb * 8 > maxk) maxk = L.nkb * 8;
        if (l + 1 < d->n_layers && s.Cout > maxk) maxk = s.Cout;
        cin = s.Cout;
    }
    {
        const unsigned long long lim = 0x7fffffffull, B = (unsigned long long)d->B;
        if (B * d->N * 12ull >= lim || B * d->M * d->nsample * 4ull >= lim || B * d->M * (unsigned long long)cin * 4ull >= lim ||
            B * d->N * (unsigned long long)(p.C > 0 ? p.C : 1) * 4ull >= lim)
            return fail(PTT_EUNSUPPORTED, "ptt_sa_fused_fwd_f32: B=%d N=%d M=%d: an array of this launch exceeds 2 GiB "
                        "(32-bit offsets) — split the batch", d->B, d->N, d->M);
    }
    p.ldk = maxk + 4;
    p.vec_gather = (p.C > 0 && p.fsc == 1 && (p.C & 3) == 0 && p.C <= 256 && (p.fsn & 3) == 0 &&
                    (p.fsb & 3) == 0 && (reinterpret_cast<uintptr_t>(p.feat) & 15) == 0) ? 1 : 0;
    p.first_wave = 1024; p.stagger = dev_switches().sa_stagger;
    p.dbg = dev_switches().stamps;
    p.cws = nullptr;
    const int total_centres = d->B * d->M;
    hipStream_t s = as_stream(stream);
    int rc;
    if (d->C == 0 && d->use_xyz && !hoist && d->nsample == 32 && d->n_layers == 3 && p.L[0].Cout == 64 && p.L[1].Cout == 64 &&
        p.L[2].Cout == 128 && !p.L[0].scale && !p.L[1].scale && !p.L[2].scale && p.L[0].relu && p.L[1].relu &&
        dev_switches().sa_lds) {
        const int waves = 256 * PTT_SAL_WAVES * PTT_SAL_WGS;
        p.chunk = (total_centres + waves - 1) / waves;
        if (dev_switches().sa_lds_chunk > 0 && p.chunk > dev_switches().sa_lds_chunk) p.chunk = dev_switches().sa_lds_chunk;
        const int nw = total_centres * 3 <= 256 * PTT_SAL_WAVES ? 4 : PTT_SAL_WAVES;
        int wgs = (total_centres + p.chunk * nw - 1) / (p.chunk * nw);
        const int lds = (4096 + 8192 + PTT_SAL_WAVES * 640) * (int)sizeof(float);
        if (d->compact_ws) {
            if (d->compact_ws_bytes < ptt_sa_compact_workspace(d->B, d->M) || (reinterpret_cast<uintptr_t>(d->compact_ws) & 15))
                return fail(PTT_EWORKSPACE, "ptt_sa_fused_fwd_f32: compact_ws needs %zu bytes, 16-byte aligned (got %zu)",
                            ptt_sa_compact_workspace(d->B, d->M), d->compact_ws_bytes);
            p.cws = static_cast<int32_t*>(d->compact_ws);
            hipLaunchKernelGGL(sa_compact_zero_kernel, dim3(1), dim3(64), 0, s, p.cws);
            if ((rc = check_launch("sa_compact_zero_kernel"))) return rc;
            hipLaunchKernelGGL(sa_compact_kernel<true>, dim3((total_centres + 31) / 32), dim3(256), 0, s, d->xyz, d->idx, d->N, d->M,
                               SacTable{p.cws, total_centres});
            if ((rc = check_launch("sa_compact_kernel"))) return rc;
            if (wgs > 256 * PTT_SAL_WGS) wgs = 256 * PTT_SAL_WGS;
            if ((rc = set_lds_limit(reinterpret_cast<const void*>(sa_lds_kernel<true>), lds))) return rc;
            hipLaunchKernelGGL(sa_lds_kernel<true>, dim3(wgs), dim3(64 * nw), lds, s, p);
            return check_launch("sa_lds_kernel");
        }
        if ((rc = set_lds_limit(reinterpret_cast<const void*>(sa_lds_kernel<false>), lds))) return rc;
        hipLaunchKernelGGL(sa_lds_kernel<false>, dim3(wgs), dim3(64 * nw), lds, s, p);
        return check_launch("sa_lds_kernel");
    }
    size_t wbytes = 0;
    bool wave_ok = true;
    for (int l = 0; l < d->n_layers; ++l) {
        wbytes += (size_t)d->layers[l].Cin * d->layers[l].Cout * sizeof(float);
        const int nt = d->layers[l].Cout / 32;
        if (!(nt == 1 || nt == 2 || nt == 4)) wave_ok = false;
    }
    wave_ok = wave_ok && dev_switches().sa_wave;
    if (wave_ok && wbytes <= 64 * 1024 && d->nsample <= 32) {
        const int lds = 4 * 32 * p.ldk * (int)sizeof(float);
        const int cpw = 32 / d->nsample, per_wg = 4 * cpw;
        const dim3 grid((total_centres + per_wg - 1) / per_wg);
        if (d->nsample == 32) {
            if ((rc = set_lds_limit(reinterpret_cast<const void*>(sa_wave_kernel<32, 1>), lds))) return rc;
            hipLaunchKernelGGL((sa_wave_kernel<32, 1>), grid, dim3(256), lds, s, p);
        } else {
            if ((rc = set_lds_limit(reinterpret_cast<const void*>(sa_wave_kernel<16, 1>), lds))) return rc;
            hipLaunchKernelGGL((sa_wave_kernel<16, 1>), grid, dim3(256), lds, s, p);
        }
        return check_launch("sa_wave_kernel");
    }
    if (p.hoist == 2 && d->nsample == 32 && d->n_layers == 2 && p.L[0].Cin == 128 && p.L[0].Cout == 128 &&
        p.L[1].Cout == 256 && !p.L[0].scale && !p.L[1].scale && p.L[0].relu && dev_switches().sa_stream) {
        p.tiles = (total_centres + 1) / 2;
        int wgs = p.tiles < 512 ? p.tiles : 512;
        p.chunk = (p.tiles + wgs - 1) / wgs;
        if (dev_switches().sa_chunk > 0 && p.chunk > dev_switches().sa_chunk) p.chunk = dev_switches().sa_chunk;
        wgs = (p.tiles + p.chunk - 1) / p.chunk;
        if (d->compact_ws) {
            if (d->compact_ws_bytes < ptt_sa_compact_workspace(d->B, d->M) || (reinterpret_cast<uintptr_t>(d->compact_ws) & 15))
                return fail(PTT_EWORKSPACE, "ptt_sa_fused_fwd_f32: compact_ws needs %zu bytes, 16-byte aligned (got %zu)",
                            ptt_sa_compact_workspace(d->B, d->M), d->compact_ws_bytes);
            p.cws = static_cast<int32_t*>(d->compact_ws);
            hipLaunchKernelGGL(sa_compact_zero_kernel, dim3(1), dim3(64), 0, s, p.cws);
            if ((rc = check_launch("sa_compact_zero_kernel"))) return rc;
            hipLaunchKernelGGL(sa_compact_kernel<false>, dim3((total_centres + 31) / 32), dim3(256), 0, s, d->xyz, d->idx, d->N, d->M,
                               SacTable{p.cws, total_centres});
            if ((rc = check_launch("sa_compact_kernel"))) return rc;
            const int lds = (2 * SAS_TILE + 64 * 4 + 64) * (int)sizeof(float);
            if ((rc = set_lds_limit(reinterpret_cast<const void*>(sa_stream_compact_kernel), lds))) return rc;
            hipLaunchKernelGGL(sa_stream_compact_kernel, dim3(p.tiles < 512 ? p.tiles : 512), dim3(256), lds, s, p);
            return check_launch("sa_stream_compact_kernel");
        }
        const int lds = (2 * SAS_TILE + 4 * 16 * 4) * (int)sizeof(float);
        if ((rc = set_lds_limit(reinterpret_cast<const void*>(sa_stream_kernel<32>), lds))) return rc;
        hipLaunchKernelGGL((sa_stream_kernel<32>), dim3(wgs), dim3(256), lds, s, p);
        return check_launch("sa_stream_kernel");
    }
    int RT = dev_switches().sa_rt;
    if (d->nsample == 64) RT = 2;
    const int lds = 32 * RT * p.ldk * (int)sizeof(float);
    if (lds > 160 * 1024) return fail(PTT_EUNSUPPORTED, "ptt_sa_fused_fwd_f32: %d B of LDS per workgroup", lds);
    const int cpw = 32 * RT / d->nsample;
    const dim3 grid((total_centres + cpw - 1) / cpw);
#define PTT_SA_CASE(NSV, RTV)                                                                                   \
    if (d->nsample == NSV && RT == RTV) {                                                                       \
        if ((rc = set_lds_limit(reinterpret_cast<const void*>(sa_fused_kernel<NSV, RTV>), lds))) return rc;     \
        hipLaunchKernelGGL((sa_fused_kernel<NSV, RTV>), grid, dim3(256), lds, s, p);                            \
    }
    PTT_SA_CASE(32, 2) PTT_SA_CASE(32, 1) PTT_SA_CASE(16, 2) PTT_SA_CASE(16, 1) PTT_SA_CASE(64, 2)
#undef PTT_SA_CASE
    return check_launch("sa_fused_kernel");
}

extern "C" int ptt_xcorr_fused_fwd_f32(const ptt_xcorr_desc* d, ptt_stream_t stream) {
    if (!d) return fail(PTT_EINVAL, "ptt_xcorr_fused_fwd_f32: null descriptor");
    if (d->B < 0 || d->Ns <= 0 || d->C0 <= 0 || d->n_layers < 1 || d->n_layers > PTT_SA_MAX_LAYERS)
        return fail(PTT_EINVAL, "ptt_xcorr_fused_fwd_f32: B=%d Ns=%d C0=%d layers=%d", d->B, d->Ns, d->C0, d->n_layers);
    if (d->Nt <= 0 || (d->Nt % 64) != 0)
        return fail(PTT_EUNSUPPORTED, "ptt_xcorr_fused_fwd_f32: Nt=%d (the template seeds are walked in chunks of 64)", d->Nt);
    if (d->n_layers < 2) return fail(PTT_EUNSUPPORTED, "ptt_xcorr_fused_fwd_f32: needs at least two MFMA layers after layer 0");
    if ((d->C0 % 8) != 0 || d->C0 > 256) return fail(PTT_EUNSUPPORTED, "ptt_xcorr_fused_fwd_f32: C0=%d", d->C0);
    if (d->B == 0) return PTT_OK;
    if (!d->P || !d->w_sim || !d->out) return fail(PTT_EINVAL, "ptt_xcorr_fused_fwd_f32: null pointer");
    if ((unsigned long long)d->B * d->Ns * d->Nt >= 0x7fffffffull || (unsigned long long)d->B * d->Nt * d->C0 >= 0x7fffffffull)
        return fail(PTT_EUNSUPPORTED, "ptt_xcorr_fused_fwd_f32: B=%d Ns=%d Nt=%d: 32-bit element offsets — split the batch",
                    d->B, d->Ns, d->Nt);
    XcorrParams q;
    q.P = d->P; q.wsim = d->w_sim; q.scale0 = d->scale0;
    q.shift0 = d->shift0; q.sim_out = d->sim_out; q.cos_t = d->cos_t;
    q.C0 = d->C0; q.Nt = d->Nt;
    q.sfeat = q.tfeat = nullptr; q.s_sb = q.s_sn = q.t_sb = q.t_sn = 0; q.C = 0; q.eps = 0.f; q.out_sh = 0;
    SaParams& p = q.sa;
    memset(&p, 0, sizeof(p));
    p.out = d->out; p.osb = d->out_sb; p.osc = d->out_sc; p.osm = d->out_sn;
    p.B = d->B; p.M = d->Ns; p.n_layers = d->n_layers;
    int maxk = d->C0, cin = d->C0;
    for (int l = 0; l < d->n_layers; ++l) {
        const ptt_sa_layer& s = d->layers[l];
        if (s.Cin != cin) return fail(PTT_EINVAL, "ptt_xcorr_fused_fwd_f32: layer %d Cin=%d, expected %d", l, s.Cin, cin);
        if (s.Cout <= 0 || (s.Cout % 32) != 0 || s.Cout > 256)
            return fail(PTT_EUNSUPPORTED, "ptt_xcorr_fused_fwd_f32: layer %d Cout=%d", l, s.Cout);
        if (!s.Wpacked) return fail(PTT_EINVAL, "ptt_xcorr_fused_fwd_f32: layer %d has no weights", l);
        SaLayerDev& L = p.L[l];
        L.Wp = s.Wpacked; L.scale = s.scale; L.shift = s.shift; L.Cin = s.Cin; L.Cout = s.Cout; L.relu = s.relu;
        L.nkb = (s.Cin + 7) / 8; L.NT = s.Cout / 32;
        if (l + 1 < d->n_layers && s.Cout > maxk) maxk = s.Cout;
        cin = s.Cout;
    }
    p.ldk = ((maxk + 7) / 8) * 8 + 4;
    p.first_wave = 1024; p.stagger = 2;
    if (d->split) {
        if (!d->search_feat || !d->templ_feat || d->sim_out || (d->C & 3) || (d->s_sb & 3) || (d->s_sn & 3) ||
            (d->t_sb & 3) || (d->t_sn & 3) || ((reinterpret_cast<uintptr_t>(d->search_feat) | reinterpret_cast<uintptr_t>(d->templ_feat)) & 15) ||
            ((d->B * d->Ns) & 7) || d->C <= 0)
            return fail(PTT_EINVAL, "ptt_xcorr_fused_fwd_f32: the split form needs the features (unit channel stride, C %% 4 == 0, 16-byte "
                                    "aligned rows), B * Ns %% 8 == 0 and no sim_out");
        q.sfeat = d->search_feat; q.tfeat = d->templ_feat; q.s_sb = d->s_sb; q.s_sn = d->s_sn; q.t_sb = d->t_sb; q.t_sn = d->t_sn;
        q.C = d->C; q.eps = d->eps; q.out_sh = d->out_sh;
        const int lds = (32 * p.ldk + 32) * (int)sizeof(float);
        int rc = set_lds_limit(reinterpret_cast<const void*>(xcorr_fused_kernel<1, true>), lds);
        if (rc) return rc;
        hipLaunchKernelGGL((xcorr_fused_kernel<1, true>), dim3(2 * d->B * d->Ns), dim3(256), lds, as_stream(stream), q);
        return check_launch("xcorr_fused_kernel");
    }
    if (!d->cos_t) return fail(PTT_EINVAL, "ptt_xcorr_fused_fwd_f32: null pointer (cos_t comes from ptt_cosine_map_f32)");
    const int lds = (64 * p.ldk + 64) * (int)sizeof(float);
    int rc = set_lds_limit(reinterpret_cast<const void*>(xcorr_fused_kernel<2, false>), lds);
    if (rc) return rc;
    hipLaunchKernelGGL((xcorr_fused_kernel<2, false>), dim3(d->B * d->Ns), dim3(256), lds, as_stream(stream), q);
    return check_launch("xcorr_fused_kernel");
}

extern "C" int ptt_cosine_map_f32(const float* search_feat, int64_t s_sb, int64_t s_sn, int64_t s_sc, const float* templ_feat,
                                  int64_t t_sb, int64_t t_sn, int64_t t_sc, int B, int Ns, int Nt, int C, float eps,
                                  float* cos_t, ptt_stream_t stream) {
    if (B < 0 || Ns <= 0 || Nt <= 0 || C <= 0) return fail(PTT_EINVAL, "ptt_cosine_map_f32: B=%d Ns=%d Nt=%d C=%d", B, Ns, Nt, C);
    if (B == 0) return PTT_OK;
    if (!search_feat || !templ_feat || !cos_t) return fail(PTT_EINVAL, "ptt_cosine_map_f32: null pointer");
// ... 50 lines not shown
```

ptt_amd/csrc/point_ops.hip:

```cpp
#pragma clang fp contract(off)

#include <limits.h>
#include <stdlib.h>
#include "common.h"

namespace ptt {

__device__ __forceinline__ float sqdist3(float ax, float ay, float az, float bx, float by, float bz) {
    const float dx = ax - bx, dy = ay - by, dz = az - bz;
    return (dx * dx + dy * dy) + dz * dz;
}

__device__ __forceinline__ float knn_dist(float ax, float ay, float az, float bx, float by, float bz) {
    const float d = sqdist3(ax, ay, az, bx, by, bz);
    return d < __builtin_inff() ? d : 3.402823466e+38f;
}

__device__ __forceinline__ float lane_bcast(float v, int src_lane) {
    return __builtin_bit_cast(float, __builtin_amdgcn_readlane(__builtin_bit_cast(int, v), src_lane));
}

typedef float fps_f2 __attribute__((ext_vector_type(2)));


template <int T, int P, bool LX, int ABL = 0>
__global__ __launch_bounds__(T) void fps_kernel(const float* __restrict__ xyz, int N, int npoint,
                                               int32_t* __restrict__ idx_out) {
    constexpr int W = T / 64;
    const int b = blockIdx.x;
    const float* __restrict__ pts = xyz + (size_t)b * N * 3;
    int32_t* __restrict__ out = idx_out + (size_t)b * npoint;
    const int t = threadIdx.x;
    const int lane = t & 63;
    const int wv = t >> 6;

    extern __shared__ int sel_lds[];
    float* xyz_lds = reinterpret_cast<float*>(sel_lds + ((npoint + 3) & ~3));

    float px[P], py[P], pz[P], md[P];
#pragma unroll
    for (int i = 0; i < P; ++i) {
        const int k = t * P + i;
        float x = 0.f, y = 0.f, z = 0.f, m = -1.0f;
        if (k < N) {
            x = pts[3 * k + 0];
            y = pts[3 * k + 1];
            z = pts[3 * k + 2];
            const float mag = (x * x + y * y) + z * z;
            m = (mag > 1e-3f) ? 1e10f : -1.0f;
            if (LX) { xyz_lds[3 * k + 0] = x; xyz_lds[3 * k + 1] = y; xyz_lds[3 * k + 2] = z; }
        }
        px[i] = x; py[i] = y; pz[i] = z; md[i] = m;
    }

    __shared__ __attribute__((aligned(16))) float slots[2][W > 1 ? W : 1][8];

    float lx = pts[0], ly = pts[1], lz = pts[2];
    if (t == 0 && npoint > 0) sel_lds[0] = 0;
    if (LX) __syncthreads();

    for (int j = 1; j < npoint; ++j) {
        float best = -1.0f, bx = 0.f, by = 0.f, bz = 0.f;
        int besti = 0;
        if constexpr ((P % 2) == 0) {
            const fps_f2 lxv = {lx, lx}, lyv = {ly, ly}, lzv = {lz, lz};
#pragma unroll
            for (int i = 0; i < ((ABL & 32) ? 2 : P); i += 2) {
                const fps_f2 dx = fps_f2{px[i], px[i + 1]} - lxv, dy = fps_f2{py[i], py[i + 1]} - lyv,
                             dz = fps_f2{pz[i], pz[i + 1]} - lzv;
                const fps_f2 d = (dx * dx + dy * dy) + dz * dz;
#pragma unroll
                for (int h = 0; h < 2; ++h) {
                    const float m = fminf(md[i + h], d[h]);
                    md[i + h] = m;
                    const bool take = m > best;
                    best = take ? m : best;
                    besti = take ? t * P + i + h : besti;
                    if (!LX) {
                        bx = take ? px[i + h] : bx;
                        by = take ? py[i + h] : by;
                        bz = take ? pz[i + h] : bz;
                    }
                }
            }
        } else {
#pragma unroll
            for (int i = 0; i < P; ++i) {
                const float d = sqdist3(px[i], py[i], pz[i], lx, ly, lz);
                const float m = fminf(md[i], d);
                md[i] = m;
                const bool take = m > best;
                best = take ? m : best;
                besti = take ? t * P + i : besti;
                if (!LX) {
                    bx = take ? px[i] : bx;
                    by = take ? py[i] : by;
                    bz = take ? pz[i] : bz;
                }
            }
        }
        float wmax;
        if constexpr (ABL & 1) wmax = __builtin_amdgcn_readfirstlane(best); else wmax = wave_max_f32_fused(best);
        int src;
        if constexpr (ABL & 2) {
            src = (int)(__builtin_bit_cast(unsigned, wmax) & 63u);
        } else {
            const unsigned long long winners = __ballot(best == wmax);
            src = __ffsll((long long)winners) - 1;
            if constexpr (ABL & 1) src &= 63;
        }
// ... 2 lines not shown
            if (wmax < 0.f) widx = 0;
            if constexpr ((ABL & 8) != 0) {
                lx = (float)widx * 1e-3f; ly = lx; lz = lx;
            } else if constexpr (LX) {
                lx = xyz_lds[3 * widx + 0]; ly = xyz_lds[3 * widx + 1]; lz = xyz_lds[3 * widx + 2];
            } else if (wmax < 0.f) {
                lx = pts[0]; ly = pts[1]; lz = pts[2];
            } else {
                lx = lane_bcast(bx, src); ly = lane_bcast(by, src); lz = lane_bcast(bz, src);
            }
            if (lane == 0) sel_lds[j] = widx;
        } else if constexpr ((ABL & 4) != 0) {
            int gi = __builtin_amdgcn_readlane(besti, src);
            if (wmax < 0.f) gi = 0;
            if constexpr ((ABL & 8) != 0) { lx = (float)gi * 1e-3f; ly = lx; lz = lx; }
            else { lx = xyz_lds[3 * gi + 0]; ly = xyz_lds[3 * gi + 1]; lz = xyz_lds[3 * gi + 2]; }
            if (lane == 0 && wv == 0) sel_lds[j] = gi;
        } else {
            const int par = j & 1;
            if (lane == src) {
                if constexpr (LX) {
                    *reinterpret_cast<float2*>(slots[par][wv]) = make_float2(best, __builtin_bit_cast(float, besti));
                } else {
                    float4* s4 = reinterpret_cast<float4*>(slots[par][wv]);
                    s4[0] = make_float4(best, __builtin_bit_cast(float, besti), bx, by);
                    slots[par][wv][4] = bz;
                }
            }
            if constexpr ((ABL & 16) == 0) __syncthreads();
            float gd, gx = 0.f, gy = 0.f, gz = 0.f;
            int gi;
            if constexpr (W <= 4) {
                gd = -1.0f; gi = 0;
#pragma unroll
                for (int w = 0; w < W; ++w) {
                    if constexpr (LX) {
                        const float2 s2 = *reinterpret_cast<const float2*>(slots[par][w]);
                        const bool take = s2.x > gd;
                        gd = take ? s2.x : gd;
                        gi = take ? __builtin_bit_cast(int, s2.y) : gi;
                    } else {
                        const float4 s4 = *reinterpret_cast<const float4*>(slots[par][w]);
                        const float sz = slots[par][w][4];
                        const bool take = s4.x > gd;
                        gd = take ? s4.x : gd;
                        gi = take ? __builtin_bit_cast(int, s4.y) : gi;
                        gx = take ? s4.z : gx;
                        gy = take ? s4.w : gy;
                        gz = take ? sz : gz;
                    }
                }
            } else {
                if constexpr (LX) {
                    float2 s2 = make_float2(-1.0f, 0.f);
                    if (lane < W) s2 = *reinterpret_cast<const float2*>(slots[par][lane]);
                    gd = wave_max_f32_fused(s2.x);
                    const int sl = __ffsll((long long)__ballot(s2.x == gd)) - 1;
                    gi = __builtin_amdgcn_readlane(__builtin_bit_cast(int, s2.y), sl);
                } else {
                    float4 s4 = make_float4(-1.0f, 0.f, 0.f, 0.f);
                    float sz = 0.f;
                    if (lane < W) { s4 = *reinterpret_cast<const float4*>(slots[par][lane]); sz = slots[par][lane][4]; }
                    gd = wave_max_f32_fused(s4.x);
                    const int sl = __ffsll((long long)__ballot(s4.x == gd)) - 1;
                    gi = __builtin_amdgcn_readlane(__builtin_bit_cast(int, s4.y), sl);
                    gx = lane_bcast(s4.z, sl); gy = lane_bcast(s4.w, sl); gz = lane_bcast(sz, sl);
                }
            }
            if (gd < 0.f) gi = 0;
            if constexpr ((ABL & 16) != 0) gi &= 1023;
            if constexpr ((ABL & 8) != 0) {
                lx = (float)gi * 1e-3f; ly = lx; lz = lx;
            } else if constexpr (LX) {
                lx = xyz_lds[3 * gi + 0]; ly = xyz_lds[3 * gi + 1]; lz = xyz_lds[3 * gi + 2];
            } else {
                if (gd < 0.f) { gx = pts[0]; gy = pts[1]; gz = pts[2]; }
                lx = gx; ly = gy; lz = gz;
            }
            if (t == 0) sel_lds[j] = gi;
        }
    }
    __syncthreads();
    for (int j = t; j < npoint; j += T) out[j] = sel_lds[j];
}

template <int T, int P>
static int launch_fps(const float* xyz, int B, int N, int npoint, int32_t* idx, hipStream_t s) {
    const size_t sel_bytes = (size_t)((npoint + 3) & ~3) * sizeof(int);
    if (sel_bytes + (size_t)N * 12 + 1024 <= 65536 && !dev_switches().fps_plain) {
#ifdef PTT_DEV
        if (const char* e = getenv("PTT_FPS_ABL")) {
            const int abl = atoi(e);
#define PTT_FPS_ABL_CASE(A) if (abl == A) { hipLaunchKernelGGL((fps_kernel<T, P, true, A>), dim3(B), dim3(T), sel_bytes + (size_t)N * 12, s, xyz, N, npoint, idx); return check_launch("fps_kernel(abl)"); }
            PTT_FPS_ABL_CASE(1) PTT_FPS_ABL_CASE(2) PTT_FPS_ABL_CASE(3) PTT_FPS_ABL_CASE(4) PTT_FPS_ABL_CASE(8) PTT_FPS_ABL_CASE(12) PTT_FPS_ABL_CASE(15)
            PTT_FPS_ABL_CASE(16) PTT_FPS_ABL_CASE(32) PTT_FPS_ABL_CASE(47) PTT_FPS_ABL_CASE(7) PTT_FPS_ABL_CASE(24) PTT_FPS_ABL_CASE(40)
#undef PTT_FPS_ABL_CASE
        }
#endif
        hipLaunchKernelGGL((fps_kernel<T, P, true>), dim3(B), dim3(T), sel_bytes + (size_t)N * 12, s, xyz, N, npoint, idx);
        return check_launch("fps_kernel");
    }
    hipLaunchKernelGGL((fps_kernel<T, P, false>), dim3(B), dim3(T), sel_bytes, s, xyz, N, npoint, idx);
    return check_launch("fps_kernel");
}

template <int CPW>
__device__ __forceinline__ void ball_sweep(const float* __restrict__ pts, int N, float r2, int ns, const float (&cx)[CPW],
                                           const float (&cy)[CPW], const float (&cz)[CPW], int ncentres,
                                           int32_t* __restrict__ out0, int lane) {
    int cnt[CPW], first[CPW];
#pragma unroll
    for (int c = 0; c < CPW; ++c) { cnt[c] = (c < ncentres) ? 0 : ns; first[c] = 0; }
    for (int base = 0; base < N; base += 64) {
        const int k = base + lane;
        const bool in = k < N;
        float px = 0.f, py = 0.f, pz = 0.f;
        if (in) { px = pts[3 * k + 0]; py = pts[3 * k + 1]; pz = pts[3 * k + 2]; }
        bool active = false;
#pragma unroll
        for (int c = 0; c < CPW; ++c) {
            if (cnt[c] >= ns) continue;
            const float d = sqdist3(cx[c], cy[c], cz[c], px, py, pz);
            const bool hit = in && d < r2;
            const unsigned long long mask = __ballot(hit);
            if (mask != 0ull) {
                if (cnt[c] == 0) first[c] = base + (__ffsll((long long)mask) - 1);
                const int pos = cnt[c] + __popcll(mask & ((1ull << lane) - 1ull));
                if (hit && pos < ns) out0[(size_t)c * ns + pos] = k;
                cnt[c] += __popcll(mask);
            }
            active = active || cnt[c] < ns;
        }
        if (!active) break;
    }
#pragma unroll
    for (int c = 0; c < CPW; ++c) {
        if (c >= ncentres) break;
        const int fill = (cnt[c] > 0) ? first[c] : 0;
        for (int s = cnt[c] + lane; s < ns; s += 64) out0[(size_t)c * ns + s] = fill;
    }
}

template <int CPW>
__global__ __launch_bounds__(256) void ball_query_kernel(const float* __restrict__ new_xyz,
                                                         const float* __restrict__ xyz, int BM, int M, int N,
                                                         float r2, int ns, int32_t* __restrict__ idx_out) {
    const int centre = (blockIdx.x * 4 + (threadIdx.x >> 6)) * CPW;
    if (centre >= BM) return;
    const int lane = threadIdx.x & 63;
    const int b = centre / M;
    float cx[CPW], cy[CPW], cz[CPW];
    const int nc = min(CPW, BM - centre);
#pragma unroll
    for (int c = 0; c < CPW; ++c) {
        const int cc = centre + (c < nc ? c : 0);
        cx[c] = new_xyz[(size_t)cc * 3 + 0]; cy[c] = new_xyz[(size_t)cc * 3 + 1]; cz[c] = new_xyz[(size_t)cc * 3 + 2];
    }
    ball_sweep<CPW>(xyz + (size_t)b * N * 3, N, r2, ns, cx, cy, cz, nc, idx_out + (size_t)centre * ns, lane);
}

template <int CPW>
__global__ __launch_bounds__(256) void centres_ball_query_kernel(const float* __restrict__ xyz, const int32_t* __restrict__ sel,
                                                                 int BM, int M, int N, float r2, int ns,
                                                                 float* __restrict__ new_xyz, long long* __restrict__ idx64,
                                                                 int32_t* __restrict__ idx_out) {
    const int centre = (blockIdx.x * 4 + (threadIdx.x >> 6)) * CPW;
    if (centre >= BM) return;
    const int lane = threadIdx.x & 63;
    const int b = centre / M;
    const float* __restrict__ pts = xyz + (size_t)b * N * 3;
    float cx[CPW], cy[CPW], cz[CPW];
    const int nc = min(CPW, BM - centre);
#pragma unroll
    for (int c = 0; c < CPW; ++c) {
        const int cc = centre + (c < nc ? c : 0);
        const int n = sel ? sel[cc] : cc - b * M;
        cx[c] = pts[3 * n + 0]; cy[c] = pts[3 * n + 1]; cz[c] = pts[3 * n + 2];
        if (lane == 0 && c < nc) {
            new_xyz[(size_t)cc * 3 + 0] = cx[c]; new_xyz[(size_t)cc * 3 + 1] = cy[c]; new_xyz[(size_t)cc * 3 + 2] = cz[c];
            if (idx64) idx64[cc] = n;
        }
    }
    ball_sweep<CPW>(pts, N, r2, ns, cx, cy, cz, nc, idx_out + (size_t)centre * ns, lane);
}

// ... 635 lines not shown
__global__ __launch_bounds__(256) void ball_query_grid_kernel(const float* __restrict__ xyz, const float* __restrict__ centres,
                                                              const int32_t* __restrict__ sel, int sel_mode, int BM, int M, int N,
                                                              float r2, int ns, const int32_t* __restrict__ ws,
                                                              float* __restrict__ new_xyz_out, long long* __restrict__ idx64,
                                                              int32_t* __restrict__ idx_out) {
    extern __shared__ unsigned bq_bits[];
    const int lane = threadIdx.x & 63, wv = threadIdx.x >> 6;
    const int centre = blockIdx.x * 4 + wv;
    if (centre >= BM) return;
    const int words = (N + 31) >> 5;
    unsigned* __restrict__ bits = bq_bits + (size_t)wv * words;
    const int b = centre / M;
    const float* __restrict__ pts = xyz + (size_t)b * N * 3;
    const int32_t* __restrict__ slice = ws + (size_t)b * grid_slice_ints(N);
    const GridHead g = *reinterpret_cast<const GridHead*>(slice);
    const int32_t* __restrict__ cstart = slice + 8;
    const int32_t* __restrict__ cpts = slice + 8 + GRID_MAX_CELLS + 1;
    float cx, cy, cz;
    if (sel_mode) {
        const int n = sel ? sel[centre] : centre - b * M;
        cx = pts[3 * n]; cy = pts[3 * n + 1]; cz = pts[3 * n + 2];
        if (lane == 0) {
            new_xyz_out[(size_t)centre * 3] = cx; new_xyz_out[(size_t)centre * 3 + 1] = cy; new_xyz_out[(size_t)centre * 3 + 2] = cz;
            if (idx64) idx64[centre] = n;
        }
    } else {
        cx = centres[(size_t)centre * 3]; cy = centres[(size_t)centre * 3 + 1]; cz = centres[(size_t)centre * 3 + 2];
    }
    for (int w = lane; w < words; w += 64) bits[w] = 0u;
    __builtin_amdgcn_wave_barrier();
    const int ix = grid_cell_coord(cx, g.ox, g.inv, g.nx), iy = grid_cell_coord(cy, g.oy, g.inv, g.ny), iz = grid_cell_coord(cz, g.oz, g.inv, g.nz);
    for (int dz = -1; dz <= 1; ++dz) {
        const int z = iz + dz;
        if (z < 0 || z >= g.nz) continue;
        for (int dy = -1; dy <= 1; ++dy) {
            const int y = iy + dy;
            if (y < 0 || y >= g.ny) continue;
            const int x0 = ix > 0 ? ix - 1 : 0, x1 = ix + 1 < g.nx ? ix + 1 : g.nx - 1;
            const int c0 = (z * g.ny + y) * g.nx + x0;
            const int s0 = cstart[c0], s1 = cstart[c0 + (x1 - x0) + 1];
            for (int e = s0 + lane; e < s1; e += 64) {
                const int k = cpts[e];
                const float d = sqdist3(cx, cy, cz, pts[3 * k], pts[3 * k + 1], pts[3 * k + 2]);
                if (d < r2) atomicOr(&bits[k >> 5], 1u << (k & 31));
            }
        }
    }
    __builtin_amdgcn_wave_barrier();
    asm volatile("s_waitcnt lgkmcnt(0)" ::: "memory");
    int32_t* __restrict__ out = idx_out + (size_t)centre * ns;
    int cnt = 0, first = 0;
    for (int w0 = 0; w0 < words && cnt < ns; w0 += 64) {
        const int w = w0 + lane;
        unsigned v = w < words ? bits[w] : 0u;
        const int mine = __popc(v);
        int incl = mine;
#pragma unroll
        for (int off = 1; off < 64; off <<= 1) { const int u = __shfl_up(incl, off, 64); if (lane >= off) incl += u; }
        const int total = __shfl(incl, 63, 64);
        if (total == 0) continue;
        if (cnt == 0) {
            const unsigned long long any = __ballot(mine > 0);
            const int fl = __ffsll((long long)any) - 1;
            const unsigned fv = __shfl(v, fl, 64);
            first = ((w0 + fl) << 5) + (__ffs(fv) - 1);
        }
        int pos = cnt + incl - mine;
        while (v != 0u && pos < ns) {
            const int bit = __ffs(v) - 1;
            out[pos++] = (w << 5) + bit;
            v &= v - 1u;
        }
        cnt += total;
    }
    const int have = cnt < ns ? cnt : ns;
    const int fill = cnt > 0 ? first : 0;
    for (int s2 = have + lane; s2 < ns; s2 += 64) out[s2] = fill;
}

}

using namespace ptt;

extern "C" int ptt_fps_f32(const float* xyz, int B, int N, int npoint, int32_t* idx_out, ptt_stream_t stream) {
    if (B < 0 || N <= 0 || npoint < 0) return fail(PTT_EINVAL, "ptt_fps_f32: B=%d N=%d npoint=%d", B, N, npoint);
    if (B == 0 || npoint == 0) return PTT_OK;
    if (!xyz || !idx_out) return fail(PTT_EINVAL, "ptt_fps_f32: null pointer");
    if (npoint > 15360) return fail(PTT_EUNSUPPORTED, "ptt_fps_f32: npoint=%d exceeds the LDS index buffer (15360)", npoint);
    hipStream_t s = as_stream(stream);
    if (N <= 64) return launch_fps<64, 1>(xyz, B, N, npoint, idx_out, s);
    if (N <= 128) return launch_fps<64, 2>(xyz, B, N, npoint, idx_out, s);
    if (N <= 256) return launch_fps<64, 4>(xyz, B, N, npoint, idx_out, s);
    if (N <= 512) {
        if (const int T = dev_switches().fps_t) {
            if (T == 256) return launch_fps<256, 2>(xyz, B, N, npoint, idx_out, s);
            if (T == 128) return launch_fps<128, 4>(xyz, B, N, npoint, idx_out, s);
            if (T == 512) return launch_fps<512, 1>(xyz, B, N, npoint, idx_out, s);
        }
        return launch_fps<64, 8>(xyz, B, N, npoint, idx_out, s);
    }
    if (N <= 1024) {
        if (const int T = dev_switches().fps_t) {
            if (T == 64) return launch_fps<64, 16>(xyz, B, N, npoint, idx_out, s);
            if (T == 128) return launch_fps<128, 8>(xyz, B, N, npoint, idx_out, s);
            if (T == 512) return launch_fps<512, 2>(xyz, B, N, npoint, idx_out, s);
        }
        return launch_fps<256, 4>(xyz, B, N, npoint, idx_out, s);
    }
    if (N <= 2048) {
        if (const int T = dev_switches().fps_t) {
            if (T == 512) return launch_fps<512, 4>(xyz, B, N, npoint, idx_out, s);
            if (T == 1024) return launch_fps<1024, 2>(xyz, B, N, npoint, idx_out, s);
            if (T == 128) return launch_fps<128, 16>(xyz, B, N, npoint, idx_out, s);
        }
        return launch_fps<256, 8>(xyz, B, N, npoint, idx_out, s);
    }
    if (N <= 4096) return launch_fps<512, 8>(xyz, B, N, npoint, idx_out, s);
    if (N <= 8192) return launch_fps<1024, 8>(xyz, B, N, npoint, idx_out, s);
    if (N <= 16384) return launch_fps<1024, 16>(xyz, B, N, npoint, idx_out, s);
    return fail(PTT_EUNSUPPORTED, "ptt_fps_f32: N=%d exceeds the register-resident limit 16384 (use ptt_fps_ws_f32)", N);
}

extern "C" int ptt_spatial_order_f32(const float* xyz, int B, int N, int32_t* order, ptt_stream_t stream) {
    if (B < 0 || N <= 0) return fail(PTT_EINVAL, "ptt_spatial_order_f32: B=%d N=%d", B, N);
    if (B == 0) return PTT_OK;
    if (!xyz || !order) return fail(PTT_EINVAL, "ptt_spatial_order_f32: null pointer");
    if (N > 8192 || (long long)B * N > INT_MAX) return fail(PTT_EUNSUPPORTED, "ptt_spatial_order_f32: N=%d (at most 8192 points per cloud are sorted in LDS)", N);
    int P = 2;
    while (P < N) P <<= 1;
    const int lds = P * (int)sizeof(unsigned long long);
    if (int rc = set_lds_limit(reinterpret_cast<const void*>(spatial_order_kernel), lds)) return rc;
    hipLaunchKernelGGL(spatial_order_kernel, dim3(B), dim3(1024), lds, as_stream(stream), xyz, N, P, order);
    return check_launch("spatial_order_kernel");
}

extern "C" int ptt_fps_ws_f32(const float* xyz, int B, int N, int npoint, int32_t* idx_out, float* workspace, size_t workspace_elems,
                              ptt_stream_t stream) {
    if (B < 0 || N <= 0 || npoint < 0) return fail(PTT_EINVAL, "ptt_fps_ws_f32: B=%d N=%d npoint=%d", B, N, npoint);
    if (B == 0 || npoint == 0) return PTT_OK;
    if (!xyz || !idx_out) return fail(PTT_EINVAL, "ptt_fps_ws_f32: null pointer");
    if ((long long)N * 3 > INT_MAX) return fail(PTT_EUNSUPPORTED, "ptt_fps_ws_f32: N=%d", N);
    if (!workspace || workspace_elems < (size_t)B * N)
        return fail(PTT_EWORKSPACE, "ptt_fps_ws_f32: %zu floats of workspace needed", (size_t)B * N);
    hipLaunchKernelGGL(fps_ws_kernel, dim3(B), dim3(1024), 0, as_stream(stream), xyz, N, npoint, workspace, idx_out);
    return check_launch("fps_ws_kernel");
}

static int ball_cpw(int BM, int M) {
    const int force = dev_switches().ball_cpw;
    if (force == 1 || (M & 3) != 0) return 1;
    if (force == 8 && (M & 7) == 0) return 8;
    if (force == 4) return 4;
    return BM >= 4 * 256 * 8 ? 4 : 1;
}

extern "C" int ptt_ball_query_f32(const float* new_xyz, const float* xyz, int B, int M, int N, float radius,
                                  int nsample, int32_t* idx_out, ptt_stream_t stream) {
    if (B < 0 || M < 0 || N <= 0 || nsample <= 0)
        return fail(PTT_EINVAL, "ptt_ball_query_f32: B=%d M=%d N=%d nsample=%d", B, M, N, nsample);
    if (B == 0 || M == 0) return PTT_OK;
    if (!new_xyz || !xyz || !idx_out) return fail(PTT_EINVAL, "ptt_ball_query_f32: null pointer");
    const float r2 = radius * radius;
    const int BM = B * M;
    const int cpw = ball_cpw(BM, M);
    if (cpw == 8)
        hipLaunchKernelGGL((ball_query_kernel<8>), dim3((BM / 8 + 3) / 4), dim3(256), 0, as_stream(stream), new_xyz, xyz, BM, M,
                           N, r2, nsample, idx_out);
    else if (cpw == 4)
        hipLaunchKernelGGL((ball_query_kernel<4>), dim3((BM / 4 + 3) / 4), dim3(256), 0, as_stream(stream), new_xyz, xyz, BM, M,
                           N, r2, nsample, idx_out);
    else
        hipLaunchKernelGGL((ball_query_kernel<1>), dim3((BM + 3) / 4), dim3(256), 0, as_stream(stream), new_xyz, xyz, BM, M,
                           N, r2, nsample, idx_out);
    return check_launch("ball_query_kernel");
}

extern "C" int ptt_gather_f32(const float* feat, const int32_t* idx, int B, int C, int N, int M, float* out,
                              ptt_stream_t stream) {
    if (B < 0 || C < 0 || N <= 0 || M < 0) return fail(PTT_EINVAL, "ptt_gather_f32: bad sizes");
    const size_t total = (size_t)B * C * M;
    if (total == 0) return PTT_OK;
    if (!feat || !idx || !out) return fail(PTT_EINVAL, "ptt_gather_f32: null pointer");
    hipLaunchKernelGGL(gather_kernel, dim3(grid_for(total, 256)), dim3(256), 0, as_stream(stream), feat, idx, C, N, M,
                       out, total);
    return check_launch("gather_kernel");
}

extern "C" int ptt_select_centres_f32(const float* xyz, const int32_t* idx, int B, int N, int M, float* new_xyz,
                                      int64_t* idx64_out, ptt_stream_t stream) {
    if (B < 0 || N <= 0 || M < 0 || (!idx && M > N)) return fail(PTT_EINVAL, "ptt_select_centres_f32: B=%d N=%d M=%d", B, N, M);
    const size_t total = (size_t)B * M;
    if (total == 0) return PTT_OK;
    if (!xyz || !new_xyz) return fail(PTT_EINVAL, "ptt_select_centres_f32: null pointer");
    hipLaunchKernelGGL(select_centres_kernel, dim3(grid_for(total, 256)), dim3(256), 0, as_stream(stream), xyz, idx, N, M,
                       new_xyz, reinterpret_cast<long long*>(idx64_out), total);
    return check_launch("select_centres_kernel");
}

extern "C" int ptt_gather_grad_f32(const float* grad_out, const int32_t* idx, int B, int C, int N, int M,
                                   float* grad_feat, ptt_stream_t stream) {
    if (B < 0 || C < 0 || N <= 0 || M < 0) return fail(PTT_EINVAL, "ptt_gather_grad_f32: bad sizes");
    const size_t nout = (size_t)B * C * N;
    if (nout == 0) return PTT_OK;
// ... 218 lines not shown
```

ptt_amd/models/backbones_3d/pointnet2/pointnet2_modules.py:

```python
import os
from typing import List

import torch
import torch.nn as nn
import torch.nn.functional as F

from .... import ops, train_ops
from ....param_cache import (DropsCachesOnModeChange, FoldedLayer, ParamCache, conv_bn_tensors, fold_conv_bn,
                             index_table)
from . import pointnet2_utils
from . import pytorch_utils as pt_utils

STREAM_COMPACT_MIN_BALLS = 2048
STREAM_COMPACT_MAX_POINTS = 1024


class PointnetSAModuleVotes(DropsCachesOnModeChange, nn.Module):
    def __init__(self, *, mlp: List[int], radius: float = None, nsample: int = None, bn: bool = True,
                 use_xyz: bool = True, normalize_xyz: bool = False, sample_uniformly: bool = False,
                 sample_method='fps'):
        super().__init__()
        self.radius = radius
        self.nsample = nsample
        self.mlp_module = None
        self.use_xyz = use_xyz
        self.normalize_xyz = normalize_xyz
        self.sample_uniformly = sample_uniformly
        self.grouper = pointnet2_utils.QueryAndGroup(radius, nsample, use_xyz=use_xyz, ret_grouped_xyz=True,
                                                     normalize_xyz=normalize_xyz, sample_uniformly=sample_uniformly,
                                                     ret_unique_cnt=False)
        mlp_spec = mlp
        if use_xyz and len(mlp_spec) > 0:
            mlp_spec[0] += 3
        self.mlp_module = pt_utils.SharedMLP(mlp_spec, bn=bn)
        self.sample_method = sample_method
        self._fused_cache = ParamCache()
        self.centres_knn_k = 0
        self.centres_knn = None

    def _sample(self, xyz, features, npoint):
        if self.sample_method == 'fps':
            return pointnet2_utils.furthest_point_sample(xyz, npoint)
        if self.sample_method in ('rs', 'sequence'):
            return index_table(xyz.size(0), npoint, xyz.device, torch.int32)
        if self.sample_method == 'ffps':
            raise NotImplementedError("sample_method 'ffps' needs furthest_point_sampling_with_dist, which the "
                                      "reference's extension never provided (tools/cfgs/kitti_models/ptt.yaml:42)")
        raise NotImplementedError(self.sample_method)

    def _fusable(self, xyz, features):
        if self.training or not xyz.is_cuda:
            return False
        name = 'PointnetSAModuleVotes(nsample=%s, mlp=%s)' % (self.nsample, [u.conv.weight.shape[0] for u in self.mlp_module
                                                                              if hasattr(u, 'conv')])
        if ops.autograd_recording(self, xyz, features):
            return ops.note_unfused(name, 'autograd is recording (wrap inference in torch.no_grad())')
        if self.sample_uniformly or self.nsample not in (16, 32, 64):
            return ops.note_unfused(name, 'nsample must be 16, 32 or 64 and sample_uniformly off')
        if xyz.dtype != torch.float32 or (features is not None and features.dtype != torch.float32):
            return ops.note_unfused(name, 'inputs must be float32')
        if len(self.mlp_module) > 4:
            return ops.note_unfused(name, 'more than 4 SharedMLP layers')
        for unit in self.mlp_module:
            conv = getattr(unit, 'conv', None)
            if conv is None or conv.kernel_size != (1, 1) or conv.weight.shape[0] % 32 != 0 or conv.weight.shape[0] > 256:
                return ops.note_unfused(name, 'layer widths must be multiples of 32, at most 256, 1x1 convolutions')
            if list(unit._modules.keys())[0] != 'conv':
                return ops.note_unfused(name, 'pre-activation units')
        return True

    def _fused_params(self, device):
        return self._fused_cache.get(conv_bn_tensors(self.mlp_module), device, self._fold)

    def _fold(self):
        layers, scale0 = [], None
        for li, unit in enumerate(self.mlp_module):
            w = unit.conv.weight
            cout, cin = w.shape[0], w.shape[1]
            rot = 3 if (li == 0 and self.use_xyz and cin > 3) else 0
            scale, shift = fold_conv_bn(unit)
            scale0 = scale if li == 0 else scale0
            wq = w if scale is None else w * scale.view(-1, 1, 1, 1)
            layers.append(FoldedLayer(ops.pack_weight(wq, rot), None, shift, cin, cout, hasattr(unit, 'activation')))
        hoist = None
        w0 = self.mlp_module[0].conv.weight
        if (self.use_xyz and len(layers) >= 2 and w0.shape[1] > 3 and layers[0].cout <= 256
                and os.environ.get('PTT_SA_HOIST', '1') != '0'):
            w2 = w0.reshape(w0.shape[0], w0.shape[1]).float()
            wx = w2[:, 0:3] if scale0 is None else w2[:, 0:3] * scale0[:, None]
            wf = w2[:, 3:] if scale0 is None else w2[:, 3:] * scale0[:, None]
            hoist = (ops.pack_weight(wf.contiguous()), wx.t().contiguous(), layers[0].cout, layers[0].relu)
        return layers, hoist

    def forward(self, xyz: torch.Tensor, features: torch.Tensor, npoint: int, inds: torch.Tensor = None, pre=None,
                compact: bool = False):
        self.centres_knn = None
        if self._fusable(xyz, features):
            return self._forward_fused(xyz, features, npoint, inds, pre, compact)
        return self._forward_train(xyz, features, npoint, inds)

    def _forward_fused(self, xyz, features, npoint, inds, pre, compact):
        if (pre is None and inds is None and self.sample_method == 'fps' and xyz.shape[1] <= 256 and npoint <= 128
                and xyz.shape[0] * npoint * self.nsample <= ops.ONE_FRAME_MAX_SA_ROWS and self.centres_knn_k <= npoint):
            xyz = xyz.contiguous()
            inds, inds64, new_xyz, idx, self.centres_knn = ops.fps_ball_knn(xyz, npoint, self.radius, self.nsample, self.centres_knn_k)
            pre = (new_xyz, idx, inds64)
        prefix = inds is None and self.sample_method in ('rs', 'sequence')
        if pre is not None:
            pass
        elif prefix:
            inds64 = index_table(xyz.size(0), npoint, xyz.device, torch.int64)
        elif inds is None:
            inds = self._sample(xyz, features, npoint)
        else:
            assert inds.shape[1] == npoint
            inds = inds.to(torch.int32)

        xyz = xyz.contiguous()
        if pre is not None:
            new_xyz, idx, inds64 = pre
        elif prefix:
            new_xyz, _, idx = ops.centres_ball_query(xyz, None, npoint, self.radius, self.nsample)
        else:
            new_xyz, inds64, idx = ops.centres_ball_query(xyz, inds.contiguous(), npoint, self.radius, self.nsample)
        layers, hoist = self._fused_params(xyz.device)
        if hoist is not None and features is not None:
            wf_packed, wx, c0, relu0 = hoist
            rows = features.transpose(1, 2)
            uniform = rows.stride(2) == 1 and rows.stride(0) == rows.shape[1] * rows.stride(1)
            term = ops.linear(rows if uniform else rows.contiguous(), wf_packed, c0, None, layers[0].shift, relu=False)
            B, M, ns = xyz.shape[0], npoint, self.nsample
            if (B * M * ns <= ops.ONE_FRAME_MAX_SA_ROWS and ns in (16, 32) and len(layers) == 3 and c0 % 4 == 0 and c0 >= 192):
                L1, L2 = layers[1], layers[2]
                h = torch.empty((B * M * ns, L1.cout), dtype=torch.float32, device=xyz.device)
                ops.row_jobs([pt_utils.layer_job(L1, prologue=3, x=term, idx=idx, xyz=xyz, centres=new_xyz, wx=wx,
                                                 radius=self.radius, ns=ns, M=M, N=xyz.shape[1], normalize_xyz=self.normalize_xyz,
                                                 pro_relu=relu0, out=h)])
                pooled = torch.empty((B, M, L2.cout), dtype=torch.float32, device=xyz.device)
                ops.row_jobs([pt_utils.layer_job(L2, x=h, epilogue=2, ns=ns, M=M, out=pooled)])
                return new_xyz, pooled.transpose(1, 2), inds64
            new_features = ops.sa_fused_forward(xyz, new_xyz, idx, None, layers[1:], self.radius, True,
                                                self.normalize_xyz, point_major_out=True, l0=(term, wx, relu0),
                                                compact=(bool(compact) and B * M >= STREAM_COMPACT_MIN_BALLS
                                                         and xyz.shape[1] <= STREAM_COMPACT_MAX_POINTS))
        else:
            new_features = ops.sa_fused_forward(xyz, new_xyz, idx, features, layers, self.radius,
                                                self.use_xyz, self.normalize_xyz, point_major_out=True,
                                                compact=features is None)
        return new_xyz, new_features, inds64

    def _forward_train(self, xyz, features, npoint, inds):
        if inds is None:
            inds = self._sample(xyz, features, npoint)
        else:
            assert inds.shape[1] == npoint
            inds = inds.to(torch.int32)
        hoist = (self.use_xyz and not self.sample_uniformly and self.nsample * npoint <= 16384
                 and train_ops.usable(self.mlp_module, xyz if features is None else features)
                 and self.mlp_module[0].conv.weight.shape[0] % 4 == 0)
        if hoist and not xyz.requires_grad and inds.dtype == torch.int32:
            new_xyz, inds64, idx = ops.centres_ball_query(xyz.contiguous(), inds.contiguous(), npoint, self.radius, self.nsample)
            y = train_ops.sa_level_hoisted(xyz, new_xyz, features, idx, self.mlp_module, self.radius, self.normalize_xyz)
            return new_xyz, y, inds64
        xyz_flipped = xyz.transpose(1, 2).contiguous()
        new_xyz = pointnet2_utils.gather_operation(xyz_flipped, inds).transpose(1, 2).contiguous()
        if hoist and features is not None:
            idx = pointnet2_utils.ball_query(self.radius, self.nsample, xyz, new_xyz)
            y = train_ops.sa_level_hoisted(xyz, new_xyz, features, idx, self.mlp_module, self.radius, self.normalize_xyz)
            return new_xyz, y, inds.to(torch.int64)
        grouped_features, grouped_xyz = self.grouper(xyz, new_xyz, features)
        if train_ops.usable(self.mlp_module, grouped_features):
            return new_xyz, train_ops.shared_mlp_pool(grouped_features, self.mlp_module, pool_dim=3), inds.to(torch.int64)
        y = self.mlp_module(grouped_features)
        y = y.max(dim=3)[0]
        return new_xyz, y, inds.to(torch.int64)
```

ptt_amd/models/backbones_3d/pointnet2_backbone.py:

```python
from typing import List

import torch
import torch.nn as nn

from ... import graph_policy, ops, train_ops
from ...param_cache import ParamCache, index_table
from .pointnet2 import pointnet2_modules


class PointNet2BackboneLight(nn.Module):
    def __init__(self, model_cfg, input_channels, **kwargs):
        super().__init__()
        self.model_cfg = model_cfg
        input_channels -= 3
        self.num_points_each_layer = []
        self.SA_modules = nn.ModuleList()
        sa = self.model_cfg.SA_CONFIG
        for k in range(len(sa.RADIUS)):
            mlps = list(sa.MLPS[k])
            if k == 0:
                mlps[0] = input_channels
            self.SA_modules.append(pointnet2_modules.PointnetSAModuleVotes(
                radius=sa.RADIUS[k], nsample=sa.NSAMPLE[k], mlp=mlps,
                use_xyz=sa.get('USE_XYZ', True), normalize_xyz=sa.get('NORMALIZE_XYZ', True),
                sample_method=sa.SAMPLE_METHOD[k]))
        self.cov_final = nn.Conv1d(256, 256, kernel_size=1)
        self.num_point_features = sa.MLPS[-1][-1]
        self._cov_cache = ParamCache()
        self.seed_knn = 16
        self.overlap_branches = True
        self._side_stream = None

    @staticmethod
    def _break_up_pc(pc):
        xyz = pc[..., 0:3].contiguous()
        features = pc[..., 3:].contiguous() if pc.size(-1) > 3 else None
        return xyz, features

    def _cov_final(self, features):
        if not features.is_cuda:
            return self.cov_final(features)
        if self.training:
            if features.dtype != torch.float32:
                return self.cov_final(features)
            return train_ops.rows_linear(self.cov_final, features.transpose(1, 2)).transpose(1, 2)
        if ops.autograd_recording(self.cov_final, features) or features.dtype != torch.float32:
            ops.note_unfused('PointNet2BackboneLight.cov_final', 'autograd is recording or input is not float32')
            return self.cov_final(features)
        w, b = self.cov_final.weight, self.cov_final.bias
        wpacked, bias = self._cov_cache.get([w, b], w.device, lambda: (ops.pack_weight(w), b.detach().float().contiguous()))
        rows = features.transpose(1, 2)
        out = ops.linear(rows, wpacked, w.shape[0], None, bias)
        return out.transpose(1, 2)

    def branch_forward(self, pts, npoints: List, inds0=None, want_knn=0, compact_levels=()):
        xyz, features = self._break_up_pc(pts)
        sa = self.model_cfg.SA_CONFIG
        one_frame = (not self.training and xyz.is_cuda and features is None and len(self.SA_modules) == 3
                     and xyz.shape[0] * npoints[0] <= 4 * ops.ONE_FRAME_MAX_POINTS
                     and self.SA_modules[0].sample_method == 'fps'
                     and all(m.sample_method in ('rs', 'sequence') for m in self.SA_modules[1:])
                     and npoints[0] >= npoints[1] >= npoints[2] and (not want_knn or npoints[2] <= 128)
                     and all(m._fusable(xyz, None) for m in self.SA_modules[:1]))
        knn = None
        if one_frame:
            from .pointnet2 import pointnet2_utils
            xyz = xyz.contiguous()
            if inds0 is None:
                inds0 = pointnet2_utils.furthest_point_sample(xyz, npoints[0])
            inds0 = inds0.to(torch.int32).contiguous()
            levels, inds64, knn = ops.sa_levels_point_jobs(xyz, inds0, list(npoints), list(sa.RADIUS), list(sa.NSAMPLE),
                                                           knn_k=want_knn)
            seq = [None] + [index_table(xyz.size(0), n, xyz.device, torch.int64) for n in npoints[1:3]]
            xyz, features, inds0 = self.SA_modules[0](xyz=xyz, features=features, npoint=npoints[0], inds=inds0,
                                                      pre=(levels[0][0], levels[0][1], inds64))
            xyz, features, inds1 = self.SA_modules[1](xyz=xyz, features=features, npoint=npoints[1],
                                                      pre=(levels[1][0], levels[1][1], seq[1]))
            xyz, features, inds2 = self.SA_modules[2](xyz=xyz, features=features, npoint=npoints[2],
                                                      pre=(levels[2][0], levels[2][1], seq[2]))
        else:
            xyz, features, inds0 = self.SA_modules[0](xyz=xyz, features=features, npoint=npoints[0], inds=inds0)
            xyz, features, inds1 = self.SA_modules[1](xyz=xyz, features=features, npoint=npoints[1], compact=1 in compact_levels)
            xyz, features, inds2 = self.SA_modules[2](xyz=xyz, features=features, npoint=npoints[2], compact=2 in compact_levels)
        point_features = self._cov_final(features)
        assert inds1.dtype == inds2.dtype == torch.int64, 'index type must be int64, not {}'.format(inds2.dtype)
        if all(m.sample_method in ('rs', 'sequence') for m in self.SA_modules[1:]) and inds0.shape[1] >= npoints[2]:
            inds = inds0[:, :npoints[2]]
        else:
            inds = inds0.gather(1, inds1).gather(1, inds2)
        if want_knn:
            return xyz, point_features, inds, knn
        return xyz, point_features, inds

    def sample(self, search_points, template_points):
        from .pointnet2 import pointnet2_utils
        sa = self.model_cfg.SA_CONFIG
        assert sa.SAMPLE_METHOD[0] == 'fps'
        return (pointnet2_utils.furthest_point_sample(search_points[..., 0:3].contiguous(), sa.NPOINTS_SEARCH[0]),
                pointnet2_utils.furthest_point_sample(template_points[..., 0:3].contiguous(), sa.NPOINTS_TEMPLATE[0]))

    def forward_branches(self, search_points, template_points, inds=None):
        sa = self.model_cfg.SA_CONFIG
        i_s, i_t = inds if inds is not None else (None, None)
        last = (len(self.SA_modules) - 1,) if (search_points.is_cuda and not self.training) else ()
        if not (self.overlap_branches and search_points.is_cuda and not self.training):
            r = self.branch_forward(search_points, sa.NPOINTS_SEARCH, i_s, want_knn=self.seed_knn, compact_levels=last)
            t_seeds, t_feats, t_inds = self.branch_forward(template_points, sa.NPOINTS_TEMPLATE, i_t)
        else:
            if self._side_stream is None or self._side_stream.device != search_points.device:
                self._side_stream = torch.cuda.Stream(device=search_points.device)
            main = torch.cuda.current_stream(search_points.device)
            side = graph_policy.branch(main, self._side_stream)
            with torch.cuda.stream(side):
                t_seeds, t_feats, t_inds = self.branch_forward(template_points, sa.NPOINTS_TEMPLATE, i_t)
            r = self.branch_forward(search_points, sa.NPOINTS_SEARCH, i_s, want_knn=self.seed_knn, compact_levels=last)
            graph_policy.join(main, side)
            if side is not main:
                for t in (t_seeds, t_feats, t_inds, template_points):
                    t.record_stream(main)
        s_seeds, s_feats, s_inds = r[:3]
        s_knn = r[3] if len(r) > 3 else None
        out = {'search_seeds': s_seeds, 'search_feats': s_feats, 'search_inds': s_inds,
               'template_seeds': t_seeds, 'template_feats': t_feats, 'template_inds': t_inds}
        if s_knn is not None:
            out['search_seeds_knn'] = s_knn
        return out

    def forward(self, batch_dict):
        batch_dict.update(self.forward_branches(batch_dict['search_points'], batch_dict['template_points'],
                                                batch_dict.pop('fps_inds', None)))
        batch_dict.pop('search_points')
        batch_dict.pop('template_points')
        return batch_dict
```

ptt_amd/ops.py:

```python
import contextlib
import ctypes
import os

import torch

from . import _lib
from ._lib import AttnDesc, SaDesc, SaLayer, XcorrDesc


def _stream():
    return ctypes.c_void_p(torch.cuda.current_stream().cuda_stream)


_timing = None


def start_kernel_timing(names):
    global _timing
    _timing = {n: [] for n in names}


def stop_kernel_timing():
    global _timing
    t, _timing = _timing, None
# ... 42 lines not shown

param_generation = 0


def publish_params(device, replaced=True):
    global param_generation
    if replaced:
        param_generation += 1
    if device.type == 'cuda' and not torch.cuda.is_current_stream_capturing():
        torch.cuda.current_stream(device).synchronize()


def drop_params():
    global param_generation
    param_generation += 1


class StateWatch(object):

    def __init__(self, module):
        self.tensors = list(module.parameters()) + list(module.buffers())
        self.mark()

    def _key(self):
        return list(map(torch.Tensor.data_ptr, self.tensors)), [t._version for t in self.tensors]

    def mark(self):
        self.generation, self.key = param_generation, self._key()

    def changed(self):
        return param_generation != self.generation or self._key() != self.key


def require_finite(*tensors):
    bad = [k for k, t in enumerate(tensors) if t is not None and t.is_floating_point() and not bool(torch.isfinite(t).all())]
    if bad:
        raise ValueError("non-finite values in tensor(s) %s" % ", ".join("#%d %s" % (k, tuple(tensors[k].shape)) for k in bad))


def _chk(t, name, dtype, ndim=None):
    if not isinstance(t, torch.Tensor):
        raise TypeError("%s must be a torch.Tensor" % name)
    if not t.is_cuda:
        raise RuntimeError("%s must be a device (HIP) tensor — CPU tensors are not supported" % name)
    if t.dtype != dtype:
        raise RuntimeError("%s must be %s, got %s" % (name, dtype, t.dtype))
    if not t.is_contiguous():
        raise RuntimeError("%s must be contiguous" % name)
    if ndim is not None and t.dim() != ndim:
        raise RuntimeError("%s must have %d dimensions, got %s" % (name, ndim, tuple(t.shape)))
    return t


def _ptr(t):
    return ctypes.c_void_p(t.data_ptr()) if t is not None else ctypes.c_void_p(0)


_UNTIMED = contextlib.nullcontext()


def _launch(name, device, *args, timed=None):
    with torch.cuda.device(device), (_timed(timed) if timed else _UNTIMED):
        rc = getattr(_lib.lib(), name)(*args, _stream())
    if rc:
        _lib.check(rc, name)


def _host(name, *args):
    return getattr(_lib.lib(), name)(*args)


def _host_checked(name, *args):
    _lib.check(_host(name, *args), name)


def _workspace(query, device, *dims):
    ws = _ws(_host(query, *dims), device)
    return ws, (_ptr(ws), ws.numel() * 8)


FPS_RESIDENT_MAX_N, FPS_RESIDENT_MAX_NPOINT = 16384, 15360


def furthest_point_sampling(xyz, npoint):
    _chk(xyz, "xyz", torch.float32, 3)
    B, N, _ = xyz.shape
    out = torch.empty((B, int(npoint)), dtype=torch.int32, device=xyz.device)
    if N <= FPS_RESIDENT_MAX_N and int(npoint) <= FPS_RESIDENT_MAX_NPOINT:
        _launch("ptt_fps_f32", xyz.device, _ptr(xyz), B, N, int(npoint), _ptr(out), timed='ptt_fps_f32')
    else:
        ws = torch.empty((B * N,), dtype=torch.float32, device=xyz.device)
        _launch("ptt_fps_ws_f32", xyz.device, _ptr(xyz), B, N, int(npoint), _ptr(out), _ptr(ws), ws.numel(), timed='ptt_fps_f32')
    return out


def gather_points(features, idx):
    _chk(features, "features", torch.float32, 3)
    _chk(idx, "idx", torch.int32, 2)
    B, C, N = features.shape
    M = idx.shape[1]
    out = torch.empty((B, C, M), dtype=torch.float32, device=features.device)
    _launch("ptt_gather_f32", features.device, _ptr(features), _ptr(idx), B, C, N, M, _ptr(out))
    return out


def scatter_add_det(src, idx, N):
    B, C, E = src.shape
    out = torch.empty((B, C, int(N)), dtype=torch.float32, device=src.device)
    nbytes = _host("ptt_scatter_add_det_workspace", B, int(N), E)
    ws = torch.empty((max(1, (nbytes + 3) // 4),), dtype=torch.int32, device=src.device)
    _launch("ptt_scatter_add_det_f32", src.device, _ptr(src), _ptr(idx), B, C, int(N), E, _ptr(out), _ptr(ws), ws.numel() * 4)
    return out


_ATOMIC_GRADS = os.environ.get("PTT_ATOMIC_GRADS", "0")


def set_atomic_grads(on):
    global _ATOMIC_GRADS
    prev = _ATOMIC_GRADS == "1"
    _ATOMIC_GRADS = "1" if on else "0"
    return prev


def _det_grads(entries, N):
    if int(N) * 16384 > 0xffffffff:
        return False
    return entries <= 16384 and _ATOMIC_GRADS != "1"


def gather_points_grad(grad_out, idx, N):
    _chk(grad_out, "grad_out", torch.float32, 3)
    _chk(idx, "idx", torch.int32, 2)
    B, C, M = grad_out.shape
    if M > 0 and _det_grads(M, N):
        return scatter_add_det(grad_out, idx, N)
    out = torch.empty((B, C, int(N)), dtype=torch.float32, device=grad_out.device)
    _launch("ptt_gather_grad_f32", grad_out.device, _ptr(grad_out), _ptr(idx), B, C, int(N), M, _ptr(out))
    return out


def select_centres(xyz, idx, npoint, want_idx64=True):
    _chk(xyz, "xyz", torch.float32, 3)
    B, N, _ = xyz.shape
    if idx is not None:
        _chk(idx, "idx", torch.int32, 2)
    new_xyz = torch.empty((B, int(npoint), 3), dtype=torch.float32, device=xyz.device)
    idx64 = torch.empty((B, int(npoint)), dtype=torch.int64, device=xyz.device) if (want_idx64 and idx is not None) else None
    _launch("ptt_select_centres_f32", xyz.device, _ptr(xyz), _ptr(idx), B, N, int(npoint), _ptr(new_xyz), _ptr(idx64))
    return new_xyz, idx64


GRID_BALL_QUERY_MIN_POINTS = 4096


def ball_query(new_xyz, xyz, radius, nsample):
    _chk(new_xyz, "new_xyz", torch.float32, 3)
    _chk(xyz, "xyz", torch.float32, 3)
    B, M, _ = new_xyz.shape
    N = xyz.shape[1]
    out = torch.empty((B, M, int(nsample)), dtype=torch.int32, device=xyz.device)
    if GRID_BALL_QUERY_MIN_POINTS <= N <= 131072:
        ws, ws_arg = _workspace("ptt_ball_query_grid_workspace", xyz.device, B, N)
        _launch("ptt_ball_query_grid_f32", xyz.device, _ptr(new_xyz), _ptr(xyz), B, M, N, float(radius), int(nsample), _ptr(out), *ws_arg,
                timed='ptt_ball_query_f32')
    else:
        _launch("ptt_ball_query_f32", xyz.device, _ptr(new_xyz), _ptr(xyz), B, M, N, float(radius), int(nsample), _ptr(out),
                timed='ptt_ball_query_f32')
    return out


def centres_ball_query(xyz, sel, npoint, radius, nsample, want_idx64=True):
    _chk(xyz, "xyz", torch.float32, 3)
    B, N, _ = xyz.shape
    if sel is not None:
        _chk(sel, "sel", torch.int32, 2)
# ... 21 lines not shown
    return out


def group_points_grad(grad_out, idx, N):
    _chk(grad_out, "grad_out", torch.float32, 4)
    _chk(idx, "idx", torch.int32, 3)
    B, C, M, ns = grad_out.shape
    if M * ns > 0 and _det_grads(M * ns, N):
        return scatter_add_det(grad_out.view(B, C, M * ns), idx.view(B, M * ns), N)
    out = torch.empty((B, C, int(N)), dtype=torch.float32, device=grad_out.device)
    _launch("ptt_group_grad_f32", grad_out.device, _ptr(grad_out), _ptr(idx), B, C, int(N), M, ns, _ptr(out))
    return out


def _unreached(name):
    def fn(*a, **k):
        raise NotImplementedError("%s is never reached by PTT (SURVEY.md §2.1) and is not provided" % name)
    fn.__name__ = name
    return fn


three_nn = _unreached("three_nn")
three_interpolate = _unreached("three_interpolate")
three_interpolate_grad = _unreached("three_interpolate_grad")
furthest_point_sampling_with_dist = _unreached("furthest_point_sampling_with_dist")


def knn(xyz, k, want_rel=False):
    _chk(xyz, "xyz", torch.float32, 3)
    B, N, _ = xyz.shape
    out = torch.empty((B, N, int(k)), dtype=torch.int32, device=xyz.device)
    rel = torch.empty((B, N, int(k), 3), dtype=torch.float32, device=xyz.device) if want_rel else None
    _launch("ptt_knn_rel_f32", xyz.device, _ptr(xyz), B, N, int(k), _ptr(out), _ptr(rel), timed='ptt_knn_f32')
    return (out, rel) if want_rel else out


def pack_weight(weight, rot=0):
    w = weight.detach()
    w = w.reshape(w.shape[0], -1).contiguous().float()
    _chk(w, "weight", torch.float32, 2)
    Cout, K = w.shape
    n = _host("ptt_packed_weight_elems", Cout, K)
    out = torch.empty((n,), dtype=torch.float32, device=w.device)
    _launch("ptt_pack_weight_rot_f32", w.device, _ptr(w), Cout, K, int(rot), _ptr(out))
    return out


ONE_FRAME_MAX_SA_ROWS = 4096
ROW_JOB_MAX_ROWS = 1024
ONE_FRAME_MAX_POINTS = int(os.environ.get("PTT_PT_PER_LAYER_MAX", "512"))


def linear(x, wpacked, cout, scale=None, shift=None, relu=False, residual=None, out=None):
    if not x.is_cuda or x.dtype != torch.float32:
        raise RuntimeError("x must be a float32 device tensor")
    K = x.shape[-1]
    x2 = x.reshape(-1, K)
    if x2.stride(1) != 1:
        x2 = x2.contiguous()
    rows = x2.shape[0]
    if out is None:
        out = torch.empty(tuple(x.shape[:-1]) + (int(cout),), dtype=torch.float32, device=x.device)
    o2 = out.view(-1, int(cout))
    r2 = None
    if residual is not None:
        r2 = residual.reshape(-1, int(cout))
        if r2.stride(1) != 1:
            r2 = r2.contiguous()
    if (scale is None and (rows > 8192 or (rows >= 6144 and int(cout) == 256)) and x2.data_ptr() % 16 == 0 and o2.is_contiguous()
            and _host("ptt_rows_gemm_supported", rows, K, int(cout), x2.stride(0), int(cout))):
        _launch("ptt_rows_gemm_f32", x.device, _ptr(x2), rows, K, x2.stride(0), None, None, _ptr(wpacked), int(cout), _ptr(shift), 1 if relu else 0,
                _ptr(r2), r2.stride(0) if r2 is not None else int(cout), _ptr(o2), int(cout), None, 0, timed='ptt_linear_f32')
        return out
    if rows <= ROW_JOB_MAX_ROWS and 192 <= K <= 1024 and o2.stride(1) == 1:
        row_jobs([row_job(wpacked, cout, x=x2, scale=scale, shift=shift, act=1 if relu else 0, res=r2, out=o2)])
        return out
    _launch("ptt_linear_f32", x.device, _ptr(x2), rows, K, x2.stride(0) if rows > 1 else K, _ptr(wpacked), int(cout), _ptr(scale), _ptr(shift),
            1 if relu else 0, _ptr(r2), (r2.stride(0) if (r2 is not None and rows > 1) else int(cout)), _ptr(o2),
            o2.stride(0) if rows > 1 else int(cout), timed='ptt_linear_f32')
    return out


def sa_fused_forward(xyz, new_xyz, idx, features, layers, radius, use_xyz=True, normalize_xyz=False,
                     point_major_out=True, l0=None, compact=False):
    _chk(xyz, "xyz", torch.float32, 3)
    _chk(new_xyz, "new_xyz", torch.float32, 3)
    _chk(idx, "idx", torch.int32, 3)
    B, N, _ = xyz.shape
    _, M, ns = idx.shape
    d = SaDesc()
    d.xyz, d.new_xyz, d.idx = xyz.data_ptr(), new_xyz.data_ptr(), idx.data_ptr()
    if features is not None:
        if not features.is_cuda or features.dtype != torch.float32 or features.dim() != 3:
            raise RuntimeError("features must be a (B,C,N) float32 device tensor")
        d.feat = features.data_ptr()
        d.feat_sb, d.feat_sc, d.feat_sn = features.stride()
        d.C = features.shape[1]
    else:
        d.feat, d.C = None, 0
    cout = layers[-1][4]
    if point_major_out:
        store = torch.empty((B, M, cout), dtype=torch.float32, device=xyz.device)
        out = store.transpose(1, 2)
    else:
        out = torch.empty((B, cout, M), dtype=torch.float32, device=xyz.device)
    d.out = out.data_ptr()
    d.out_sb, d.out_sc, d.out_sm = out.stride()
    d.B, d.N, d.M, d.nsample = B, N, M, ns
    d.radius, d.use_xyz, d.normalize_xyz = float(radius), int(bool(use_xyz)), int(bool(normalize_xyz))
    d.n_layers = len(layers)
    for i, (wp, sc, sh, cin, co, relu) in enumerate(layers):
        L = d.layers[i]
        L.Wpacked = wp.data_ptr()
        L.scale = sc.data_ptr() if sc is not None else None
        L.shift = sh.data_ptr() if sh is not None else None
        L.Cin, L.Cout, L.relu = int(cin), int(co), int(bool(relu))
    if l0 is not None:
        term, wx, l0_relu = l0
        if features is not None:
            raise RuntimeError("with a hoisted layer 0 the point features are already inside l0[0]")
        _chk(term, "l0 point term", torch.float32, 3)
        _chk(wx, "l0 xyz weight", torch.float32, 2)
        if term.shape[0] != B or term.shape[1] != N or wx.shape[0] != 3 or wx.shape[1] != term.shape[2]:
            raise RuntimeError("l0 point term must be (B,N,C0) and the xyz weight (3,C0)")
        d.l0_point_term, d.l0_xyz_weight = term.data_ptr(), wx.data_ptr()
        d.l0_channels, d.l0_relu = term.shape[2], int(bool(l0_relu))
    if isinstance(compact, torch.Tensor):
        if not compact.is_cuda or compact.device != xyz.device or not compact.is_contiguous():
            raise RuntimeError("compact workspace must be a contiguous tensor on %s" % xyz.device)
        d.compact_ws, d.compact_ws_bytes = compact.data_ptr(), compact.numel() * compact.element_size()
    elif compact:
        ws, (_, d.compact_ws_bytes) = _workspace("ptt_sa_compact_workspace", xyz.device, B, M)
        d.compact_ws = ws.data_ptr()
    _launch("ptt_sa_fused_fwd_f32", xyz.device, ctypes.byref(d), timed='ptt_sa_fused_fwd_f32')
    return out


def cosine_map(search_feats, templ_feats, eps=1e-8):
    for t_, n_ in ((search_feats, "search_feats"), (templ_feats, "templ_feats")):
        if not isinstance(t_, torch.Tensor) or not t_.is_cuda or t_.dtype != torch.float32 or t_.dim() != 3:
            raise RuntimeError("%s must be a (B,C,N) float32 device tensor" % n_)
    if search_feats.shape[:2] != templ_feats.shape[:2] or search_feats.device != templ_feats.device:
        raise RuntimeError("search_feats and templ_feats must share batch size, channel count and device")
    B, C, Ns = search_feats.shape
    Nt = templ_feats.shape[2]
    out = torch.empty((B, Ns, Nt), dtype=torch.float32, device=search_feats.device)
    ssb, ssc, ssn = search_feats.stride()
    tsb, tsc, tsn = templ_feats.stride()
    _launch("ptt_cosine_map_f32", out.device, search_feats.data_ptr(), ssb, ssn, ssc, templ_feats.data_ptr(), tsb, tsn, tsc, B, Ns, Nt, C, float(eps),
            out.data_ptr(), timed='ptt_cosine_map_f32')
    return out


def rows_mlp(x, layers, residual=None):
    if not x.is_cuda or x.dtype != torch.float32 or x.stride(-1) != 1:
        raise RuntimeError("rows_mlp: x must be a float32 device tensor with contiguous rows")
    K = x.shape[-1]
    x2 = x.reshape(-1, K)
    rows = x2.shape[0]
    cout = int(layers[-1][4])
    out = torch.empty((rows, cout), dtype=torch.float32, device=x.device)
    res2 = None
    if residual is not None:
        res2 = residual.reshape(-1, cout)
        _chk(res2 if res2.is_contiguous() else res2.contiguous(), "residual", torch.float32, 2)
        res2 = res2 if res2.stride(1) == 1 else res2.contiguous()
    arr = (SaLayer * len(layers))()
    for i, (wp, sc, sh, cin, co, relu) in enumerate(layers):
        arr[i].Wpacked = wp.data_ptr()
        arr[i].scale = sc.data_ptr() if sc is not None else None
        arr[i].shift = sh.data_ptr() if sh is not None else None
        arr[i].Cin, arr[i].Cout, arr[i].relu = int(cin), int(co), int(bool(relu))
    _launch("ptt_rows_mlp_f32", x.device, _ptr(x2), rows, K, x2.stride(0), arr, len(layers), _ptr(res2), res2.stride(0) if res2 is not None else 0,
            _ptr(out), cout, timed='ptt_rows_mlp_f32')
    return out.view(*x.shape[:-1], cout)


def xcorr_fused(search_feats, templ_feats, P, w_sim, scale0, shift0, layers, eps=1e-8, want_sim=False, cos_t=None, split=False):
    for t_, n_ in ((search_feats, "search_feats"), (templ_feats, "templ_feats")):
        if not t_.is_cuda or t_.dtype != torch.float32 or t_.dim() != 3:
            raise RuntimeError("%s must be a (B,C,N) float32 device tensor" % n_)
    _chk(P, "P", torch.float32, 3)
    _chk(w_sim, "w_sim", torch.float32, 1)
    B, C, Ns = search_feats.shape
    Nt = templ_feats.shape[2]
    C0 = P.shape[2]
    if Nt <= 0 or Nt % 64:
        raise RuntimeError("xcorr_fused: Nt=%d (ptt_xcorr_fused_fwd_f32 walks the template seeds in chunks of 64)" % Nt)
    if P.shape[0] != B or P.shape[1] != Nt or w_sim.shape[0] != C0 or templ_feats.shape[:2] != search_feats.shape[:2]:
        raise RuntimeError("xcorr_fused: inconsistent shapes")
    cout = layers[-1][4]
    split = (split and not want_sim and search_feats.stride(1) == 1 and templ_feats.stride(1) == 1 and C % 4 == 0 and (B * Ns) % 8 == 0
             and all(st % 4 == 0 for st in (search_feats.stride(0), search_feats.stride(2), templ_feats.stride(0), templ_feats.stride(2)))
             and search_feats.data_ptr() % 16 == 0 and templ_feats.data_ptr() % 16 == 0 and bool(layers[-1][5]))
    if not split:
        if cos_t is None:
            cos_t = cosine_map(search_feats, templ_feats, eps=eps)
        _chk(cos_t, "cos_t", torch.float32, 3)
        if tuple(cos_t.shape) != (B, Ns, Nt):
            raise RuntimeError("xcorr_fused: cos_t must be (B,Ns,Nt)")
    store = torch.empty(((2, B, Ns, cout) if split else (B, Ns, cout)), dtype=torch.float32, device=P.device)
    out = store.transpose(-1, -2)
    sim = torch.empty((B, Nt, Ns), dtype=torch.float32, device=P.device) if want_sim else None
    d = XcorrDesc()
    if split:
        d.split, d.out_sh = 1, store.stride(0)
        d.search_feat, d.templ_feat = search_feats.data_ptr(), templ_feats.data_ptr()
        d.s_sb, d.s_sn, d.t_sb, d.t_sn = search_feats.stride(0), search_feats.stride(2), templ_feats.stride(0), templ_feats.stride(2)
        d.C, d.eps = int(C), float(eps)
    else:
        d.cos_t = cos_t.data_ptr()
    d.P, d.w_sim = P.data_ptr(), w_sim.data_ptr()
    d.scale0 = scale0.data_ptr() if scale0 is not None else None
    d.shift0 = shift0.data_ptr() if shift0 is not None else None
    d.out = out.data_ptr()
    d.out_sb, d.out_sc, d.out_sn = out.stride()[-3:]
# ... 1260 lines not shown
```

Before: 17430.

## Skip duplicate FPS tail centres in fused SA kernels via per-batch live counts

```diff
diff --git a/include/ptt_hip.h b/include/ptt_hip.h
--- a/include/ptt_hip.h
+++ b/include/ptt_hip.h
@@ -8,7 +8,7 @@
 extern "C" {
 #endif
 
-#define PTT_ABI_VERSION 28
+#define PTT_ABI_VERSION 29
 
 enum {
     PTT_OK = 0,
@@ -26,6 +26,8 @@
 
 int ptt_fps_f32(const float* xyz, int B, int N, int npoint, int32_t* idx_out,
                 ptt_stream_t stream);
+int ptt_fps_live_f32(const float* xyz, int B, int N, int npoint, int32_t* idx_out, int32_t* live_out,
+                     ptt_stream_t stream);
 int ptt_fps_ws_f32(const float* xyz, int B, int N, int npoint, int32_t* idx_out, float* workspace,
                    size_t workspace_elems, ptt_stream_t stream);
 
@@ -138,6 +140,7 @@
     int l0_relu;
     void* compact_ws;
     size_t compact_ws_bytes;
+    const int32_t* live;
 } ptt_sa_desc;
 
 int ptt_sa_fused_fwd_f32(const ptt_sa_desc* d, ptt_stream_t stream);
diff --git a/ptt_amd/_lib.py b/ptt_amd/_lib.py
--- a/ptt_amd/_lib.py
+++ b/ptt_amd/_lib.py
@@ -173,7 +173,7 @@
                 ("radius", c_float), ("use_xyz", c_int), ("normalize_xyz", c_int), ("n_layers", c_int),
                 ("layers", SaLayer * PTT_SA_MAX_LAYERS),
                 ("l0_point_term", c_void_p), ("l0_xyz_weight", c_void_p), ("l0_channels", c_int), ("l0_relu", c_int),
-                ("compact_ws", c_void_p), ("compact_ws_bytes", c_size_t)]
+                ("compact_ws", c_void_p), ("compact_ws_bytes", c_size_t), ("live", c_void_p)]
 
 
 class XcorrDesc(Structure):
diff --git a/ptt_amd/csrc/mfma_ops.hip b/ptt_amd/csrc/mfma_ops.hip
--- a/ptt_amd/csrc/mfma_ops.hip
+++ b/ptt_amd/csrc/mfma_ops.hip
@@ -447,6 +447,7 @@
     long long* dbg;
     int32_t* cws;
     SaLayerDev L[PTT_SA_MAX_LAYERS];
+    const int32_t* live;
 };
 
 struct RowsMlpParams {
@@ -790,6 +791,9 @@
     }
 };
 
+__device__ __forceinline__ int sa_live_lim(const int32_t* live, int b, int M) { return min(max(live[b], 1), M); }
+__device__ __forceinline__ int sas_even_lim(const int32_t* live, int b, int M) { return (sa_live_lim(live, b, M) + 1) & ~1; }
+
 __device__ __forceinline__ float sas_pool(const f32x16& a, float sh, int relu) {
     float mx = a[0];
 #pragma unroll
@@ -804,7 +808,7 @@
 #ifndef PTT_SAS_EXP
 #define PTT_SAS_EXP 0
 #endif
-template <int NS>
+template <int NS, bool LIVE>
 __global__ __launch_bounds__(256, 2) void sa_stream_kernel(SaParams p) {
     static_assert(NS == 32, "one centre per 32-row tile");
     extern __shared__ __attribute__((aligned(16))) float smem[];
@@ -813,9 +817,51 @@
     float* const meta = smem + 2 * SAS_TILE;
     const int t = threadIdx.x, lane = t & 63, half = lane >> 5, sub = half, q = lane & 31;
     const int w = __builtin_amdgcn_readfirstlane(t >> 6);
-    const int tile0 = logical_block() * p.chunk;
-    const int ntiles = min(p.chunk, p.tiles - tile0);
-    if (ntiles <= 0) return;
+    int tile0, ntiles, live_b0 = 0, live_m0 = 0, elim = 0;
+    if constexpr (LIVE) {
+        auto scan = [&](int b0) {
+            int v = b0 + lane < p.B ? sas_even_lim(p.live, b0 + lane, p.M) >> 1 : 0;
+#pragma unroll
+            for (int d = 1; d < 64; d <<= 1) { const int u = __shfl_up(v, d, 64); v += lane >= d ? u : 0; }
+            return v;
+        };
+        if (p.B <= 64) {
+            const int sc = scan(0), total = __builtin_amdgcn_readfirstlane(__shfl(sc, 63, 64));
+            const int chunk = (total + (int)gridDim.x - 1) / (int)gridDim.x;
+            tile0 = logical_block() * chunk;
+            ntiles = min(chunk, total - tile0);
+            if (ntiles <= 0) return;
+            const int k = __popcll(__ballot(sc <= tile0));
+            const int before = __builtin_amdgcn_readfirstlane(k ? __shfl(sc, k - 1, 64) : 0);
+            live_b0 = k;
+            live_m0 = 2 * (tile0 - before);
+            elim = 2 * (__builtin_amdgcn_readfirstlane(__shfl(sc, k, 64)) - before);
+        } else {
+            int total = 0;
+            for (int b0 = 0; b0 < p.B; b0 += 64) total += __shfl(scan(b0), 63, 64);
+            total = __builtin_amdgcn_readfirstlane(total);
+            const int chunk = (total + (int)gridDim.x - 1) / (int)gridDim.x;
+            tile0 = logical_block() * chunk;
+            ntiles = min(chunk, total - tile0);
+            if (ntiles <= 0) return;
+            for (int b0 = 0, base = 0; b0 < p.B; b0 += 64) {
+                const int sc = scan(b0), tot = __builtin_amdgcn_readfirstlane(__shfl(sc, 63, 64));
+                if (tile0 < base + tot) {
+                    const int k = __popcll(__ballot(base + sc <= tile0));
+                    const int before = __builtin_amdgcn_readfirstlane(k ? __shfl(sc, k - 1, 64) : 0);
+                    live_b0 = b0 + k;
+                    live_m0 = 2 * (tile0 - base - before);
+                    break;
+                }
+                base += tot;
+            }
+            elim = sas_even_lim(p.live, live_b0, p.M);
+        }
+    } else {
+        tile0 = logical_block() * p.chunk;
+        ntiles = min(p.chunk, p.tiles - tile0);
+        if (ntiles <= 0) return;
+    }
     stagger_second_slot(p.first_wave, p.stagger);
     const SaLayerDev& L1 = p.L[0];
     const SaLayerDev& L2 = p.L[1];
@@ -842,11 +888,23 @@
 
     SasCentre own, first;
     {
-        const int c0 = tile0 * 2;
-        first.c = c0; first.b = c0 / M; first.m = c0 - first.b * M;
+        if constexpr (LIVE) {
+            first.c = live_b0 * M + live_m0; first.b = live_b0; first.m = live_m0;
+        } else {
+            const int c0 = tile0 * 2;
+            first.c = c0; first.b = c0 / M; first.m = c0 - first.b * M;
+        }
         own = first;
         own.advance(w >> 1, M);
     }
+    auto live_step = [&](SasCentre& ce, int el) -> int {
+        ce.c += 2; ce.m += 2;
+        if (ce.m >= el) {
+            ce.c += M - el; ce.m -= el; ++ce.b;
+            el = sas_even_lim(p.live, min(ce.b, p.B - 1), M);
+        }
+        return el;
+    };
     auto meta_index = [&](const SasCentre& ce) -> int {
         const int c = ce.c < total_centres ? ce.c : total_centres - 1;
         return p.idx[(size_t)c * 32 + 16 * (w & 1) + (lane & 15)];
@@ -891,17 +949,30 @@
     SasCentre prev = first;
     const f32x16 zero16 = {0.f, 0.f, 0.f, 0.f, 0.f, 0.f, 0.f, 0.f, 0.f, 0.f, 0.f, 0.f, 0.f, 0.f, 0.f, 0.f};
 
+    bool prev_last = false;
     auto store_pooled = [&](const SasCentre& f) {
         SasCentre c1 = f;
         c1.advance(1, M);
+        int lim = M;
+        if constexpr (LIVE) {
+            if (prev_last) lim = sa_live_lim(p.live, f.b, M);
+        }
+        const bool alias = LIVE && lim < M && lim - 1 == f.m;
         if (half == 0) {
             if (f.c < total_centres) {
                 float* o = p.out + (f.b * osb + f.m * osm);
                 o[ocol0] = pv[0][0]; o[ocol1] = pv[0][1];
             }
-            if (c1.c < total_centres) {
+            if (c1.c < total_centres && !alias) {
                 float* o = p.out + (c1.b * osb + c1.m * osm);
                 o[ocol0] = pv[1][0]; o[ocol1] = pv[1][1];
+            }
+        }
+        if constexpr (LIVE) {
+            if (lim < M) {
+                const float v0 = alias ? pv[0][0] : pv[1][0], v1 = alias ? pv[0][1] : pv[1][1];
+                float* o = p.out + f.b * osb;
+                for (int mm = lim + half; mm < M; mm += 2) { o[mm * osm + ocol0] = v0; o[mm * osm + ocol1] = v1; }
             }
         }
     };
@@ -909,7 +980,10 @@
     for (int it = 0; it < ntiles; ++it) {
         const bool more = it + 1 < ntiles;
         SasCentre own_next = own;
-        if (more) own_next.advance(2, M);
+        int elim_next = elim;
+        if (more) {
+            if constexpr (LIVE) elim_next = live_step(own_next, elim); else own_next.advance(2, M);
+        }
         if (!(PTT_SAS_EXP & 1)) lds_barrier();
         const int nn = meta_index(own_next);
         MetaXyz mx;
@@ -1044,7 +1118,12 @@
 #undef SAS_A2
         }
         prev = first;
-        if (more) { first.advance(2, M); own = own_next; }
+        if constexpr (LIVE) {
+            prev_last = first.m + 2 >= elim;
+            if (more) { live_step(first, elim); elim = elim_next; own = own_next; }
+        } else {
+            if (more) { first.advance(2, M); own = own_next; }
+        }
     }
 #pragma unroll
     for (int i = 0; i < 4; ++i) pv[i >> 1][i & 1] = sas_pool(acc[i >> 1][i & 1], (i & 1) ? sh2b : sh2a, L2.relu);
@@ -1291,7 +1370,7 @@
 
 template <bool XYZ>
 __global__ __launch_bounds__(256) void sa_compact_kernel(const float* __restrict__ xyz, const int32_t* __restrict__ idx, int N, int M,
-                                                         SacTable tab) {
+                                                         SacTable tab, const int32_t* __restrict__ live) {
     __shared__ int s_cnt[4], s_base[4], s_cls[32], s_pos[32], s_nd[32];
     __shared__ int s_row[32][32];
     const int t = threadIdx.x, lane = t & 63, half = lane >> 5, s = lane & 31, w = t >> 6;
@@ -1334,7 +1413,11 @@
         if (keep) s_row[lc][__popc(m & ((1u << s) - 1u))] = iv[q];
         if (s == 0) {
             const int k = nd <= 4 ? 0 : nd <= 8 ? 1 : nd <= 16 ? 2 : 3;
-            const bool valid = g0 + lc < T;
+            bool valid = g0 + lc < T;
+            if (live && valid) {
+                const int b = (g0 + lc) / M;
+                valid = g0 + lc - b * M < sa_live_lim(live, b, M);
+            }
             s_cls[lc] = valid ? k : -1;
             s_nd[lc] = nd;
             s_pos[lc] = valid ? atomicAdd(&s_cnt[k], 1) : 0;
@@ -1387,15 +1470,35 @@
 };
 using SacTile = SacTileT<32>;
 
+
+__device__ __forceinline__ float sac_ball_pool(const f32x16& a, int k, int g, float sh, int relu) {
+    if (k == 3) return sas_pool(a, sh, relu);
+    float v;
+    if (k == 2) {
+        const int r0 = 8 * (g & 1);
+        float m = a[r0];
+#pragma unroll
+        for (int r = 1; r < 8; ++r) m = fmaxf(m, a[r0 + r]);
+        v = max_halves(m) + sh;
+    } else {
+        const int q = (k == 1 ? g : g >> 1) & 3;
+        const float m = fmaxf(fmaxf(a[4 * q], a[4 * q + 1]), fmaxf(a[4 * q + 2], a[4 * q + 3]));
+        v = (k == 1 ? max_halves(m) : m) + sh;
+    }
+    return relu ? fmaxf(v, 0.f) : v;
+}
+
 template <int NU>
-__device__ __forceinline__ void sac_store(int k, int n, int ball, int M, const f32x16 (&acc)[NU], const float (&sh)[NU],
-                                          float* const (&o)[NU], int relu, int half, int osb, int osm) {
+__device__ __forceinline__ void sac_store(int k, int n, int ball, int M, const int32_t* live, const f32x16 (&acc)[NU],
+                                          const float (&sh)[NU], float* const (&o)[NU], int relu, int half, int osb, int osm) {
     int ob[8];
+    unsigned last = 0;
 #pragma unroll
     for (int g = 0; g < 8; ++g) {
         if (g >= (8 >> k)) break;
         const int id = __builtin_amdgcn_readlane(ball, g << (2 + k)), b = id / M;
         ob[g] = b * osb + (id - b * M) * osm;
+        if (live && g < n && id - b * M == sa_live_lim(live, b, M) - 1) last |= 1u << g;
     }
 #pragma unroll
     for (int u = 0; u < NU; ++u) {
@@ -1432,6 +1535,23 @@
                     if (relu) v = fmaxf(v, 0.f);
                     if (g < n) o[u][half ? ob[2 * q + 1] : ob[2 * q]] = v;
                 }
+            }
+        }
+    }
+    if (last) {
+#pragma unroll
+        for (int g = 0; g < 8; ++g) {
+            if (g >= (8 >> k)) break;
+            if (!(last >> g & 1)) continue;
+            const int b = __builtin_amdgcn_readlane(ball, g << (2 + k)) / M, lim = sa_live_lim(live, b, M);
+            if (lim >= M) continue;
+            const int row0 = b * osb;
+#pragma unroll
+            for (int u = 0; u < NU; ++u) {
+                const float v = sac_ball_pool(acc[u], k, g, sh[u], relu);
+                const int step = k ? 2 : 1;
+                if (k || half == (g & 1))
+                    for (int mm = lim + (k ? half : 0); mm < M; mm += step) o[u][row0 + mm * osm] = v;
             }
         }
     }
@@ -1596,7 +1716,7 @@
             if constexpr (COMPACT) {
                 const float sh2[4] = {cst[6 * 64], cst[7 * 64], cst[8 * 64], cst[9 * 64]};
                 float* const o[4] = {p.out + col * osc, p.out + (32 + col) * osc, p.out + (64 + col) * osc, p.out + (96 + col) * osc};
-                sac_store<4>(tc.k, tc.n, g_cur, M, acc, sh2, o, p.L[2].relu, half, osb, osm);
+                sac_store<4>(tc.k, tc.n, g_cur, M, p.live, acc, sh2, o, p.L[2].relu, half, osb, osm);
             } else {
                 float* o = p.out + (ce.b * osb + ce.m * osm);
 #pragma unroll
@@ -1699,7 +1819,7 @@
             for (int rt = 0; rt < 2; ++rt) {
                 const int n = tc.n - rt * (8 >> tc.k);
                 if (n <= 0) continue;
-                sac_store<2>(tc.k, n, ballr[rt], M, acc[rt], sh2, o, L2.relu, half, osb, osm);
+                sac_store<2>(tc.k, n, ballr[rt], M, p.live, acc[rt], sh2, o, L2.relu, half, osb, osm);
             }
         }
     }
@@ -2114,6 +2234,7 @@
     p.first_wave = 1024; p.stagger = dev_switches().sa_stagger;
     p.dbg = dev_switches().stamps;
     p.cws = nullptr;
+    p.live = d->live;
     const int total_centres = d->B * d->M;
     hipStream_t s = as_stream(stream);
     int rc;
@@ -2134,7 +2255,7 @@
             hipLaunchKernelGGL(sa_compact_zero_kernel, dim3(1), dim3(64), 0, s, p.cws);
             if ((rc = check_launch("sa_compact_zero_kernel"))) return rc;
             hipLaunchKernelGGL(sa_compact_kernel<true>, dim3((total_centres + 31) / 32), dim3(256), 0, s, d->xyz, d->idx, d->N, d->M,
-                               SacTable{p.cws, total_centres});
+                               SacTable{p.cws, total_centres}, p.live);
             if ((rc = check_launch("sa_compact_kernel"))) return rc;
             if (wgs > 256 * PTT_SAL_WGS) wgs = 256 * PTT_SAL_WGS;
             if ((rc = set_lds_limit(reinterpret_cast<const void*>(sa_lds_kernel<true>), lds))) return rc;
@@ -2181,7 +2302,7 @@
             hipLaunchKernelGGL(sa_compact_zero_kernel, dim3(1), dim3(64), 0, s, p.cws);
             if ((rc = check_launch("sa_compact_zero_kernel"))) return rc;
             hipLaunchKernelGGL(sa_compact_kernel<false>, dim3((total_centres + 31) / 32), dim3(256), 0, s, d->xyz, d->idx, d->N, d->M,
-                               SacTable{p.cws, total_centres});
+                               SacTable{p.cws, total_centres}, p.live);
             if ((rc = check_launch("sa_compact_kernel"))) return rc;
             const int lds = (2 * SAS_TILE + 64 * 4 + 64) * (int)sizeof(float);
             if ((rc = set_lds_limit(reinterpret_cast<const void*>(sa_stream_compact_kernel), lds))) return rc;
@@ -2189,8 +2310,13 @@
             return check_launch("sa_stream_compact_kernel");
         }
         const int lds = (2 * SAS_TILE + 4 * 16 * 4) * (int)sizeof(float);
-        if ((rc = set_lds_limit(reinterpret_cast<const void*>(sa_stream_kernel<32>), lds))) return rc;
-        hipLaunchKernelGGL((sa_stream_kernel<32>), dim3(wgs), dim3(256), lds, s, p);
+        if (p.live && (d->M & 1) == 0) {
+            if ((rc = set_lds_limit(reinterpret_cast<const void*>(sa_stream_kernel<32, true>), lds))) return rc;
+            hipLaunchKernelGGL((sa_stream_kernel<32, true>), dim3(wgs), dim3(256), lds, s, p);
+            return check_launch("sa_stream_kernel");
+        }
+        if ((rc = set_lds_limit(reinterpret_cast<const void*>(sa_stream_kernel<32, false>), lds))) return rc;
+        hipLaunchKernelGGL((sa_stream_kernel<32, false>), dim3(wgs), dim3(256), lds, s, p);
         return check_launch("sa_stream_kernel");
     }
     int RT = dev_switches().sa_rt;
diff --git a/ptt_amd/csrc/point_ops.hip b/ptt_amd/csrc/point_ops.hip
--- a/ptt_amd/csrc/point_ops.hip
+++ b/ptt_amd/csrc/point_ops.hip
@@ -25,7 +25,7 @@
 
 template <int T, int P, bool LX, int ABL = 0>
 __global__ __launch_bounds__(T) void fps_kernel(const float* __restrict__ xyz, int N, int npoint,
-                                               int32_t* __restrict__ idx_out) {
+                                               int32_t* __restrict__ idx_out, int32_t* __restrict__ live_out) {
     constexpr int W = T / 64;
     const int b = blockIdx.x;
     const float* __restrict__ pts = xyz + (size_t)b * N * 3;
@@ -194,25 +194,39 @@
     }
     __syncthreads();
     for (int j = t; j < npoint; j += T) out[j] = sel_lds[j];
+    if (live_out) {
+        const int last = sel_lds[npoint - 1];
+        int h = 0;
+        for (int j = t; j < npoint; j += T)
+            if (sel_lds[j] != last) h = j + 1;
+        const float hw = wave_max_f32_fused((float)h);
+        if (lane == 0) slots[0][wv][0] = hw;
+        __syncthreads();
+        if (t == 0) {
+            float hm = 0.f;
+            for (int w = 0; w < W; ++w) hm = fmaxf(hm, slots[0][w][0]);
+            live_out[b] = (int)hm + 1;
+        }
+    }
 }
 
 template <int T, int P>
-static int launch_fps(const float* xyz, int B, int N, int npoint, int32_t* idx, hipStream_t s) {
+static int launch_fps(const float* xyz, int B, int N, int npoint, int32_t* idx, int32_t* live, hipStream_t s) {
     const size_t sel_bytes = (size_t)((npoint + 3) & ~3) * sizeof(int);
     if (sel_bytes + (size_t)N * 12 + 1024 <= 65536 && !dev_switches().fps_plain) {
 #ifdef PTT_DEV
         if (const char* e = getenv("PTT_FPS_ABL")) {
             const int abl = atoi(e);
-#define PTT_FPS_ABL_CASE(A) if (abl == A) { hipLaunchKernelGGL((fps_kernel<T, P, true, A>), dim3(B), dim3(T), sel_bytes + (size_t)N * 12, s, xyz, N, npoint, idx); return check_launch("fps_kernel(abl)"); }
+#define PTT_FPS_ABL_CASE(A) if (abl == A) { hipLaunchKernelGGL((fps_kernel<T, P, true, A>), dim3(B), dim3(T), sel_bytes + (size_t)N * 12, s, xyz, N, npoint, idx, live); return check_launch("fps_kernel(abl)"); }
             PTT_FPS_ABL_CASE(1) PTT_FPS_ABL_CASE(2) PTT_FPS_ABL_CASE(3) PTT_FPS_ABL_CASE(4) PTT_FPS_ABL_CASE(8) PTT_FPS_ABL_CASE(12) PTT_FPS_ABL_CASE(15)
             PTT_FPS_ABL_CASE(16) PTT_FPS_ABL_CASE(32) PTT_FPS_ABL_CASE(47) PTT_FPS_ABL_CASE(7) PTT_FPS_ABL_CASE(24) PTT_FPS_ABL_CASE(40)
 #undef PTT_FPS_ABL_CASE
         }
 #endif
-        hipLaunchKernelGGL((fps_kernel<T, P, true>), dim3(B), dim3(T), sel_bytes + (size_t)N * 12, s, xyz, N, npoint, idx);
+        hipLaunchKernelGGL((fps_kernel<T, P, true>), dim3(B), dim3(T), sel_bytes + (size_t)N * 12, s, xyz, N, npoint, idx, live);
         return check_launch("fps_kernel");
     }
-    hipLaunchKernelGGL((fps_kernel<T, P, false>), dim3(B), dim3(T), sel_bytes, s, xyz, N, npoint, idx);
+    hipLaunchKernelGGL((fps_kernel<T, P, false>), dim3(B), dim3(T), sel_bytes, s, xyz, N, npoint, idx, live);
     return check_launch("fps_kernel");
 }
 
@@ -1014,43 +1028,52 @@
 
 using namespace ptt;
 
-extern "C" int ptt_fps_f32(const float* xyz, int B, int N, int npoint, int32_t* idx_out, ptt_stream_t stream) {
+static int fps_dispatch(const float* xyz, int B, int N, int npoint, int32_t* idx_out, int32_t* live_out, ptt_stream_t stream) {
     if (B < 0 || N <= 0 || npoint < 0) return fail(PTT_EINVAL, "ptt_fps_f32: B=%d N=%d npoint=%d", B, N, npoint);
     if (B == 0 || npoint == 0) return PTT_OK;
     if (!xyz || !idx_out) return fail(PTT_EINVAL, "ptt_fps_f32: null pointer");
     if (npoint > 15360) return fail(PTT_EUNSUPPORTED, "ptt_fps_f32: npoint=%d exceeds the LDS index buffer (15360)", npoint);
     hipStream_t s = as_stream(stream);
-    if (N <= 64) return launch_fps<64, 1>(xyz, B, N, npoint, idx_out, s);
-    if (N <= 128) return launch_fps<64, 2>(xyz, B, N, npoint, idx_out, s);
-    if (N <= 256) return launch_fps<64, 4>(xyz, B, N, npoint, idx_out, s);
+    if (N <= 64) return launch_fps<64, 1>(xyz, B, N, npoint, idx_out, live_out, s);
+    if (N <= 128) return launch_fps<64, 2>(xyz, B, N, npoint, idx_out, live_out, s);
+    if (N <= 256) return launch_fps<64, 4>(xyz, B, N, npoint, idx_out, live_out, s);
     if (N <= 512) {
         if (const int T = dev_switches().fps_t) {
-            if (T == 256) return launch_fps<256, 2>(xyz, B, N, npoint, idx_out, s);
-            if (T == 128) return launch_fps<128, 4>(xyz, B, N, npoint, idx_out, s);
-            if (T == 512) return launch_fps<512, 1>(xyz, B, N, npoint, idx_out, s);
-        }
-        return launch_fps<64, 8>(xyz, B, N, npoint, idx_out, s);
+            if (T == 256) return launch_fps<256, 2>(xyz, B, N, npoint, idx_out, live_out, s);
+            if (T == 128) return launch_fps<128, 4>(xyz, B, N, npoint, idx_out, live_out, s);
+            if (T == 512) return launch_fps<512, 1>(xyz, B, N, npoint, idx_out, live_out, s);
+        }
+        return launch_fps<64, 8>(xyz, B, N, npoint, idx_out, live_out, s);
     }
     if (N <= 1024) {
         if (const int T = dev_switches().fps_t) {
-            if (T == 64) return launch_fps<64, 16>(xyz, B, N, npoint, idx_out, s);
-            if (T == 128) return launch_fps<128, 8>(xyz, B, N, npoint, idx_out, s);
-            if (T == 512) return launch_fps<512, 2>(xyz, B, N, npoint, idx_out, s);
-        }
-        return launch_fps<256, 4>(xyz, B, N, npoint, idx_out, s);
+            if (T == 64) return launch_fps<64, 16>(xyz, B, N, npoint, idx_out, live_out, s);
+            if (T == 128) return launch_fps<128, 8>(xyz, B, N, npoint, idx_out, live_out, s);
+            if (T == 512) return launch_fps<512, 2>(xyz, B, N, npoint, idx_out, live_out, s);
+        }
+        return launch_fps<256, 4>(xyz, B, N, npoint, idx_out, live_out, s);
     }
     if (N <= 2048) {
         if (const int T = dev_switches().fps_t) {
-            if (T == 512) return launch_fps<512, 4>(xyz, B, N, npoint, idx_out, s);
-            if (T == 1024) return launch_fps<1024, 2>(xyz, B, N, npoint, idx_out, s);
-            if (T == 128) return launch_fps<128, 16>(xyz, B, N, npoint, idx_out, s);
-        }
-        return launch_fps<256, 8>(xyz, B, N, npoint, idx_out, s);
-    }
-    if (N <= 4096) return launch_fps<512, 8>(xyz, B, N, npoint, idx_out, s);
-    if (N <= 8192) return launch_fps<1024, 8>(xyz, B, N, npoint, idx_out, s);
-    if (N <= 16384) return launch_fps<1024, 16>(xyz, B, N, npoint, idx_out, s);
+            if (T == 512) return launch_fps<512, 4>(xyz, B, N, npoint, idx_out, live_out, s);
+            if (T == 1024) return launch_fps<1024, 2>(xyz, B, N, npoint, idx_out, live_out, s);
+            if (T == 128) return launch_fps<128, 16>(xyz, B, N, npoint, idx_out, live_out, s);
+        }
+        return launch_fps<256, 8>(xyz, B, N, npoint, idx_out, live_out, s);
+    }
+    if (N <= 4096) return launch_fps<512, 8>(xyz, B, N, npoint, idx_out, live_out, s);
+    if (N <= 8192) return launch_fps<1024, 8>(xyz, B, N, npoint, idx_out, live_out, s);
+    if (N <= 16384) return launch_fps<1024, 16>(xyz, B, N, npoint, idx_out, live_out, s);
     return fail(PTT_EUNSUPPORTED, "ptt_fps_f32: N=%d exceeds the register-resident limit 16384 (use ptt_fps_ws_f32)", N);
+}
+
+extern "C" int ptt_fps_f32(const float* xyz, int B, int N, int npoint, int32_t* idx_out, ptt_stream_t stream) {
+    return fps_dispatch(xyz, B, N, npoint, idx_out, nullptr, stream);
+}
+
+extern "C" int ptt_fps_live_f32(const float* xyz, int B, int N, int npoint, int32_t* idx_out, int32_t* live_out, ptt_stream_t stream) {
+    if (!live_out && B > 0 && npoint > 0) return fail(PTT_EINVAL, "ptt_fps_live_f32: null live_out");
+    return fps_dispatch(xyz, B, N, npoint, idx_out, live_out, stream);
 }
 
 extern "C" int ptt_spatial_order_f32(const float* xyz, int B, int N, int32_t* order, ptt_stream_t stream) {
diff --git a/ptt_amd/models/backbones_3d/pointnet2/pointnet2_modules.py b/ptt_amd/models/backbones_3d/pointnet2/pointnet2_modules.py
--- a/ptt_amd/models/backbones_3d/pointnet2/pointnet2_modules.py
+++ b/ptt_amd/models/backbones_3d/pointnet2/pointnet2_modules.py
@@ -93,13 +93,13 @@
         return layers, hoist
 
     def forward(self, xyz: torch.Tensor, features: torch.Tensor, npoint: int, inds: torch.Tensor = None, pre=None,
-                compact: bool = False):
+                compact: bool = False, live: torch.Tensor = None):
         self.centres_knn = None
         if self._fusable(xyz, features):
-            return self._forward_fused(xyz, features, npoint, inds, pre, compact)
+            return self._forward_fused(xyz, features, npoint, inds, pre, compact, live)
         return self._forward_train(xyz, features, npoint, inds)
 
-    def _forward_fused(self, xyz, features, npoint, inds, pre, compact):
+    def _forward_fused(self, xyz, features, npoint, inds, pre, compact, live=None):
         if (pre is None and inds is None and self.sample_method == 'fps' and xyz.shape[1] <= 256 and npoint <= 128
                 and xyz.shape[0] * npoint * self.nsample <= ops.ONE_FRAME_MAX_SA_ROWS and self.centres_knn_k <= npoint):
             xyz = xyz.contiguous()
@@ -142,11 +142,11 @@
             new_features = ops.sa_fused_forward(xyz, new_xyz, idx, None, layers[1:], self.radius, True,
                                                 self.normalize_xyz, point_major_out=True, l0=(term, wx, relu0),
                                                 compact=(bool(compact) and B * M >= STREAM_COMPACT_MIN_BALLS
-                                                         and xyz.shape[1] <= STREAM_COMPACT_MAX_POINTS))
+                                                         and xyz.shape[1] <= STREAM_COMPACT_MAX_POINTS), live=live)
         else:
             new_features = ops.sa_fused_forward(xyz, new_xyz, idx, features, layers, self.radius,
                                                 self.use_xyz, self.normalize_xyz, point_major_out=True,
-                                                compact=features is None)
+                                                compact=features is None, live=live)
         return new_xyz, new_features, inds64
 
     def _forward_train(self, xyz, features, npoint, inds):
diff --git a/ptt_amd/models/backbones_3d/pointnet2_backbone.py b/ptt_amd/models/backbones_3d/pointnet2_backbone.py
--- a/ptt_amd/models/backbones_3d/pointnet2_backbone.py
+++ b/ptt_amd/models/backbones_3d/pointnet2_backbone.py
@@ -56,6 +56,9 @@
     def branch_forward(self, pts, npoints: List, inds0=None, want_knn=0, compact_levels=()):
         xyz, features = self._break_up_pc(pts)
         sa = self.model_cfg.SA_CONFIG
+        live = None
+        if isinstance(inds0, (tuple, list)):
+            inds0, live = inds0
         one_frame = (not self.training and xyz.is_cuda and features is None and len(self.SA_modules) == 3
                      and xyz.shape[0] * npoints[0] <= 4 * ops.ONE_FRAME_MAX_POINTS
                      and self.SA_modules[0].sample_method == 'fps'
@@ -79,9 +82,16 @@
             xyz, features, inds2 = self.SA_modules[2](xyz=xyz, features=features, npoint=npoints[2],
                                                       pre=(levels[2][0], levels[2][1], seq[2]))
         else:
-            xyz, features, inds0 = self.SA_modules[0](xyz=xyz, features=features, npoint=npoints[0], inds=inds0)
-            xyz, features, inds1 = self.SA_modules[1](xyz=xyz, features=features, npoint=npoints[1], compact=1 in compact_levels)
-            xyz, features, inds2 = self.SA_modules[2](xyz=xyz, features=features, npoint=npoints[2], compact=2 in compact_levels)
+            m0 = self.SA_modules[0]
+            if inds0 is None and xyz.is_cuda and not self.training and m0.sample_method == 'fps' and m0._fusable(xyz, features):
+                inds0, live = ops.fps(xyz, npoints[0], want_live=True)
+            prefix1 = self.SA_modules[1].sample_method in ('rs', 'sequence')
+            prefix2 = prefix1 and self.SA_modules[2].sample_method in ('rs', 'sequence')
+            xyz, features, inds0 = m0(xyz=xyz, features=features, npoint=npoints[0], inds=inds0, live=live)
+            xyz, features, inds1 = self.SA_modules[1](xyz=xyz, features=features, npoint=npoints[1], compact=1 in compact_levels,
+                                                      live=live if prefix1 else None)
+            xyz, features, inds2 = self.SA_modules[2](xyz=xyz, features=features, npoint=npoints[2], compact=2 in compact_levels,
+                                                      live=live if prefix2 else None)
         point_features = self._cov_final(features)
         assert inds1.dtype == inds2.dtype == torch.int64, 'index type must be int64, not {}'.format(inds2.dtype)
         if all(m.sample_method in ('rs', 'sequence') for m in self.SA_modules[1:]) and inds0.shape[1] >= npoints[2]:
@@ -96,12 +106,22 @@
         from .pointnet2 import pointnet2_utils
         sa = self.model_cfg.SA_CONFIG
         assert sa.SAMPLE_METHOD[0] == 'fps'
-        return (pointnet2_utils.furthest_point_sample(search_points[..., 0:3].contiguous(), sa.NPOINTS_SEARCH[0]),
-                pointnet2_utils.furthest_point_sample(template_points[..., 0:3].contiguous(), sa.NPOINTS_TEMPLATE[0]))
+        s_xyz, t_xyz = search_points[..., 0:3].contiguous(), template_points[..., 0:3].contiguous()
+        if s_xyz.is_cuda and not self.training and s_xyz.dtype == torch.float32 and t_xyz.dtype == torch.float32:
+            i_s, l_s = ops.fps(s_xyz, sa.NPOINTS_SEARCH[0], want_live=True)
+            i_t, l_t = ops.fps(t_xyz, sa.NPOINTS_TEMPLATE[0], want_live=True)
+            if l_s is not None and l_t is not None:
+                return i_s, i_t, l_s, l_t
+            return i_s, i_t
+        return (pointnet2_utils.furthest_point_sample(s_xyz, sa.NPOINTS_SEARCH[0]),
+                pointnet2_utils.furthest_point_sample(t_xyz, sa.NPOINTS_TEMPLATE[0]))
 
     def forward_branches(self, search_points, template_points, inds=None):
         sa = self.model_cfg.SA_CONFIG
-        i_s, i_t = inds if inds is not None else (None, None)
+        if inds is not None and len(inds) == 4:
+            i_s, i_t = (inds[0], inds[2]), (inds[1], inds[3])
+        else:
+            i_s, i_t = inds if inds is not None else (None, None)
         last = (len(self.SA_modules) - 1,) if (search_points.is_cuda and not self.training) else ()
         if not (self.overlap_branches and search_points.is_cuda and not self.training):
             r = self.branch_forward(search_points, sa.NPOINTS_SEARCH, i_s, want_knn=self.seed_knn, compact_levels=last)
diff --git a/ptt_amd/ops.py b/ptt_amd/ops.py
--- a/ptt_amd/ops.py
+++ b/ptt_amd/ops.py
@@ -148,16 +148,23 @@
 FPS_RESIDENT_MAX_N, FPS_RESIDENT_MAX_NPOINT = 16384, 15360
 
 
-def furthest_point_sampling(xyz, npoint):
+def furthest_point_sampling(xyz, npoint, want_live=False):
     _chk(xyz, "xyz", torch.float32, 3)
     B, N, _ = xyz.shape
     out = torch.empty((B, int(npoint)), dtype=torch.int32, device=xyz.device)
     if N <= FPS_RESIDENT_MAX_N and int(npoint) <= FPS_RESIDENT_MAX_NPOINT:
+        if want_live:
+            live = torch.empty((B,), dtype=torch.int32, device=xyz.device)
+            _launch("ptt_fps_live_f32", xyz.device, _ptr(xyz), B, N, int(npoint), _ptr(out), _ptr(live), timed='ptt_fps_f32')
+            return out, live
         _launch("ptt_fps_f32", xyz.device, _ptr(xyz), B, N, int(npoint), _ptr(out), timed='ptt_fps_f32')
     else:
         ws = torch.empty((B * N,), dtype=torch.float32, device=xyz.device)
         _launch("ptt_fps_ws_f32", xyz.device, _ptr(xyz), B, N, int(npoint), _ptr(out), _ptr(ws), ws.numel(), timed='ptt_fps_f32')
-    return out
+    return (out, None) if want_live else out
+
+
+fps = furthest_point_sampling
 
 
 def gather_points(features, idx):
@@ -345,7 +352,7 @@
 
 
 def sa_fused_forward(xyz, new_xyz, idx, features, layers, radius, use_xyz=True, normalize_xyz=False,
-                     point_major_out=True, l0=None, compact=False):
+                     point_major_out=True, l0=None, compact=False, live=None, out=None):
     _chk(xyz, "xyz", torch.float32, 3)
     _chk(new_xyz, "new_xyz", torch.float32, 3)
     _chk(idx, "idx", torch.int32, 3)
@@ -362,7 +369,10 @@
     else:
         d.feat, d.C = None, 0
     cout = layers[-1][4]
-    if point_major_out:
+    if out is not None:
+        if not out.is_cuda or out.dtype != torch.float32 or tuple(out.shape) != (B, cout, M):
+            raise RuntimeError("out must be a (B,Cout,M) = %s float32 device tensor" % ((B, cout, M),))
+    elif point_major_out:
         store = torch.empty((B, M, cout), dtype=torch.float32, device=xyz.device)
         out = store.transpose(1, 2)
     else:
@@ -395,6 +405,11 @@
     elif compact:
         ws, (_, d.compact_ws_bytes) = _workspace("ptt_sa_compact_workspace", xyz.device, B, M)
         d.compact_ws = ws.data_ptr()
+    if live is not None:
+        _chk(live, "live", torch.int32, 1)
+        if live.shape[0] != B or not live.is_contiguous():
+            raise RuntimeError("live must be a contiguous (B,) int32 tensor")
+        d.live = live.data_ptr()
     _launch("ptt_sa_fused_fwd_f32", xyz.device, ctypes.byref(d), timed='ptt_sa_fused_fwd_f32')
     return out
 
```

Result: no change. 17280 (-0.8%).
